# NVlabs/InstantSplat

Measured on AMD Instinct MI355X. Metric: train_iters_per_sec, higher is better.
Workload: dtype f32

## Files before the change

### include/mi355gs.h

```cpp
#ifndef MI355GS_H
#define MI355GS_H

#include <stddef.h>
#include <stdint.h>

#ifdef __cplusplus
extern "C" {
#endif

#define MI355GS_ABI_VERSION 10

#define MI355GS_OK 0
#define MI355GS_EINVAL (-1)
#define MI355GS_ELAUNCH (-2)
#define MI355GS_EOVERFLOW (-3)

int mi355gs_abi_version(void);
const char* mi355gs_error_string(int code);

size_t mi355gs_raster_geom_bytes(int P);
size_t mi355gs_raster_tiles_bytes(int W, int H);
size_t mi355gs_raster_binning_bytes(int64_t num_instances, int W, int H);

int mi355gs_raster_forward_preprocess(
    void* stream, int P, int D, int M, int W, int H,
    const float* means3D, const float* shs, const float* shs_rest, const float* colors_precomp, const float* opacities,
    const float* scales, float scale_modifier, const float* rotations, const float* cov3D_precomp,
    const float* viewmatrix, const float* projmatrix, const float* campos,
    float tanfovx, float tanfovy, int prefiltered,
    int32_t* radii, void* geom, void* tiles, int32_t* num_rendered, uint8_t* visible, void* grad_scratch, int debug);

int mi355gs_raster_forward_render(
    void* stream, int P, int W, int H, int64_t capacity, const float* bg,
    const void* geom, void* tiles, void* binning, float* out_color, int debug);

size_t mi355gs_raster_binning_bytes_render_only(int64_t num_instances, int W, int H);
int mi355gs_raster_forward_render_only(
    void* stream, int P, int W, int H, int64_t capacity, const float* bg,
    const void* geom, void* tiles, void* binning, float* out_color, int debug);

size_t mi355gs_raster_grad_scratch_bytes(int P);
size_t mi355gs_raster_grad_gate_offset(int P);
int mi355gs_raster_backward(
    void* stream, int P, int D, int M, int W, int H, const float* bg,
    const float* means3D, const float* shs, const float* shs_rest, const float* colors_precomp, const float* opacities,
    const float* scales, float scale_modifier, const float* rotations, const float* cov3D_precomp,
    const float* viewmatrix, const float* projmatrix, const float* campos,
    float tanfovx, float tanfovy,
    const void* geom, void* tiles, const void* binning, int64_t capacity, const int32_t* radii,
    const float* out_color, const float* dL_dpix, void* grad_scratch,
    float* dL_dmeans3D, float* dL_dmeans2D, float* dL_dshs, float* dL_dshs_rest, float* dL_dcolors, float* dL_dopacities,
    float* dL_dscales, float* dL_drotations, float* dL_dcov3D, int grad_scratch_is_clear, int debug);

int mi355gs_raster_mark_visible(void* stream, int P, const float* means3D, const float* viewmatrix,
                                const float* projmatrix, uint8_t* present);

int mi355gs_raster_frame_stats(void* stream, int W, int H, const void* tiles, int64_t* stats);

int mi355gs_tune_min_units(int min_units);

int mi355gs_tune_deterministic(int on);

int mi355gs_tune_scale_grad(int mode);

int mi355gs_profile_begin(void);
int mi355gs_profile_set_period(int every);
int mi355gs_profile_work_counters(void* counters);
int mi355gs_profile_read(int kind, double* total_ms, int* launches);
int mi355gs_profile_end(void);
int mi355gs_profile_ranges(int on);

size_t mi355gs_ssim_scratch_bytes(int B, int C, int H, int W);
int mi355gs_ssim_forward(void* stream, int B, int C, int H, int W, const float* img1, const float* img2,
                         float* dm_dmu1, float* dm_dsigma1_sq, float* dm_dsigma12,
                         void* scratch, float* ssim_mean, float* l1_mean, int padding_valid);
int mi355gs_ssim_backward(void* stream, int B, int C, int H, int W, const float* img1, const float* img2,
                          const float* dm_dmu1, const float* dm_dsigma1_sq, const float* dm_dsigma12,
                          const float* ssim_grad_scale, const float* l1_grad_scale, float* dL_dimg1, int padding_valid);
int mi355gs_l1_ssim_loss_fused(void* stream, int B, int C, int H, int W, const float* img1, const float* img2, void* scratch,
                               float lambda_dssim, float* ssim_mean, float* l1_mean, float* loss, float* dloss_dimg1);

size_t mi355gs_l1_scratch_bytes(int64_t n);
int mi355gs_l1_loss_forward(void* stream, int64_t n, const float* a, const float* b, void* scratch, float* mean_out);
int mi355gs_l1_loss_backward(void* stream, int64_t n, const float* a, const float* b, const float* grad_scale, float* d_a);
#define MI355GS_LOSS_PROGRAM_MAX 16
#define MI355GS_LOSS_OP_L1 0
#define MI355GS_LOSS_OP_SSIM 1
#define MI355GS_LOSS_OP_MULK 2
#define MI355GS_LOSS_OP_ADDK 3
#define MI355GS_LOSS_OP_RSUBK 4
#define MI355GS_LOSS_OP_DIVK 5
#define MI355GS_LOSS_OP_NEG 6
#define MI355GS_LOSS_OP_ADD 7
#define MI355GS_LOSS_OP_SUB 8
int mi355gs_l1_ssim_pair_forward(void* stream, int B, int C, int H, int W, const float* img1, const float* img2, void* scratch,
                                 float* dssim_dimg1);
int mi355gs_l1_ssim_pair_backward(void* stream, int64_t n, const float* img1, const float* img2, const float* dssim_dimg1,
                                  const float* g_l1, float c_l1, const float* g_ssim, float c_ssim, float* d_img1);
int mi355gs_loss_program_eval(void* stream, int n_ops, const int32_t* ops, const float* consts, int B, int C, int H, int W,
                              const void* scratch, float* ssim_mean, float* l1_mean, float* out, float* host_out, float ticket);
int mi355gs_loss_program_eval_grad(void* stream, int n_ops, const int32_t* ops, const float* consts, int B, int C, int H, int W,
                                   const void* scratch, float* ssim_mean, float* l1_mean, float* out, float* host_out, float ticket,
                                   const float* img1, const float* img2, const float* dssim_dimg1, float c_l1, float c_ssim, float* d_img1);

size_t mi355gs_knn_scratch_bytes(int N);
int mi355gs_knn_dist2(void* stream, int N, const float* points, float* mean_dist2, void* scratch);

int mi355gs_adam_step(void* stream, int64_t n, int row, float* param, const float* grad, float* exp_avg,
                      float* exp_avg_sq, const float* per_point_lr, const float* grad_sumsq,
                      float lr, float beta1, float beta2, float eps, int step);

int mi355gs_adam_multi_step(void* stream, int ntensors, const int64_t* numel, const int32_t* row, float* const* params,
                            const float* const* grads, float* const* exp_avg, float* const* exp_avg_sq,
                            const float* const* per_point_lr, const float* lr, float beta1, float beta2, float eps,
                            const int32_t* step, float* scratch, const float* gate, const int32_t* gate_index,
                            uint32_t* live, uint32_t seq);

int mi355gs_pose_forward(void* stream, int P, const float* xyz, const float* rot, const float* scaling,
                         const float* opacity_logit, const float* pose, float* means_cam, float* rot_cam, float* scales,
                         float* opac);
int mi355gs_pose_backward(void* stream, int P, const float* xyz, const float* rot, const float* scales, const float* opac,
                          const float* pose, const float* g_means, const float* g_rot, const float* g_scales,
                          const float* g_opac, float* d_xyz, float* d_rot, float* d_scaling, float* d_opacity_logit,
                          float* d_pose, float* scratch);

int mi355gs_posed_forward_preprocess(void* stream, int P, int D, int W, int H, const float* xyz, const float* f_dc,
                                     const float* f_rest, const float* opacity_logit, const float* log_scales, float scale_modifier,
                                     const float* rotation, const float* pose, const float* view_identity, const float* projmatrix,
                                     const float* origin, float tanfovx, float tanfovy, int32_t* radii, void* geom, void* tiles,
                                     int32_t* num_rendered, uint8_t* visible, void* grad_scratch, int debug);
int mi355gs_posed_backward(void* stream, int P, int D, int W, int H, const float* bg, const float* xyz, const float* f_dc,
                           const float* f_rest, const float* opacity_logit, const float* log_scales, float scale_modifier,
                           const float* rotation, const float* pose, const float* view_identity, const float* projmatrix,
                           const float* origin, float tanfovx, float tanfovy, const void* geom, void* tiles, const void* binning,
                           int64_t capacity, const int32_t* radii, const float* out_color, const float* dL_dpix,
                           void* grad_scratch, float* pose_scratch, float* d_xyz, float* d_means2D, float* d_f_dc, float* d_f_rest,
                           float* d_opacity_logit, float* d_log_scales, float* d_rotation, float* d_pose, int pose_rows, int pose_row,
                           int grad_scratch_is_clear, int debug);

size_t mi355gs_trainer_workspace_bytes(int P, int W, int H, int V, int64_t capacity);
void* mi355gs_trainer_create(int P, int W, int H, int V, int64_t capacity, float* xyz, float* f_dc, float* f_rest, float* opacity,
                             float* scaling, float* rotation, float* poses, float* const* exp_avg, float* const* exp_avg_sq,
                             const float* per_point_lr, void* workspace);
int mi355gs_trainer_step(void* trainer, void* stream, int view, int sh_degree, const float* gt_image, const float* projmatrix,
                         float tanfovx, float tanfovy, const float* bg, const float* lr, const int32_t* step, float beta1, float beta2, float eps,
                         float lambda_dssim, int do_optimizer_step, float* loss_out, int32_t* num_rendered_out);
int mi355gs_trainer_optimizer_step(void* trainer, void* stream, const float* lr, const int32_t* step, float beta1, float beta2,
                                   float eps, int commit_gate);
void mi355gs_trainer_destroy(void* trainer);
const float* mi355gs_trainer_grad(void* trainer, int k);

#define MI355GS_TRACKER_STATE_FLOATS 40
#define MI355GS_TRACKER_POSE 0
#define MI355GS_TRACKER_EXP_AVG 8
#define MI355GS_TRACKER_EXP_AVG_SQ 16
#define MI355GS_TRACKER_BEST 24
#define MI355GS_TRACKER_INITIAL 25
#define MI355GS_TRACKER_FLAG 26
#define MI355GS_TRACKER_COUNT 27
#define MI355GS_TRACKER_CAND 32
size_t mi355gs_tracker_workspace_bytes(int P, int W, int H, int64_t capacity);
void* mi355gs_tracker_create(int P, int M, int W, int H, int64_t capacity, const float* xyz, const float* f_dc, const float* f_rest,
                             const float* opacity, const float* scaling, const float* rotation, void* workspace);
int mi355gs_tracker_count(void* tracker, void* stream, int sh_degree, const float* projmatrix, float tanfovx, float tanfovy,
                          const float* pose, int32_t* count_out);
int mi355gs_tracker_run(void* tracker, void* stream, int sh_degree, const float* gt_image, const float* projmatrix, float tanfovx,
                        float tanfovy, const float* bg, const float* sched, int num_iter, int first_iter, int n_iters, float* state,
                        float* pose_trace, float* loss_trace, float* grad_trace);
void mi355gs_tracker_destroy(void* tracker);

int mi355gs_rgb8_from_planar(void* stream, int H, int W, const float* img, uint8_t* out);
size_t mi355gs_path_workspace_bytes(int P, int W, int H, int64_t capacity);
void* mi355gs_path_create(int P, int M, int W, int H, int64_t capacity, const float* xyz, const float* f_dc, const float* f_rest,
                          const float* opacity, const float* scaling, const float* rotation, void* workspace);
int mi355gs_path_render(void* path, void* stream, int sh_degree, const float* projmatrix, float tanfovx, float tanfovy,
                        const float* bg, const float* poses, int first, int n, uint8_t* frames, int32_t* counts);
void mi355gs_path_destroy(void* path);

#ifdef __cplusplus
}
#endif
#endif
```

### instantsplat_amd/_lib.py

```python
from __future__ import annotations

import ctypes
import os
from ctypes import c_float, c_int, c_int64, c_size_t, c_void_p

import torch

_HERE = os.path.dirname(os.path.abspath(__file__))
LIB_PATH = os.path.join(_HERE, "lib", "libmi355gs.so")
_LIB = None
_TEST_MODE = False

_P = c_void_p
_SIGNATURES = {
    "mi355gs_abi_version": (c_int, []),
    "mi355gs_error_string": (ctypes.c_char_p, [c_int]),
    "mi355gs_raster_geom_bytes": (c_size_t, [c_int]),
    "mi355gs_raster_tiles_bytes": (c_size_t, [c_int, c_int]),
    "mi355gs_raster_binning_bytes": (c_size_t, [c_int64, c_int, c_int]),
    "mi355gs_raster_grad_scratch_bytes": (c_size_t, [c_int]),
    "mi355gs_raster_grad_gate_offset": (c_size_t, [c_int]),
    "mi355gs_raster_forward_preprocess": (c_int, [_P, c_int, c_int, c_int, c_int, c_int, _P, _P, _P, _P, _P, _P, c_float, _P, _P,
                                                  _P, _P, _P, c_float, c_float, c_int, _P, _P, _P, _P, _P, _P, c_int]),
    "mi355gs_raster_forward_render": (c_int, [_P, c_int, c_int, c_int, c_int64, _P, _P, _P, _P, _P, c_int]),
    "mi355gs_raster_binning_bytes_render_only": (c_size_t, [c_int64, c_int, c_int]),
    "mi355gs_raster_forward_render_only": (c_int, [_P, c_int, c_int, c_int, c_int64, _P, _P, _P, _P, _P, c_int]),
    "mi355gs_raster_backward": (c_int, [_P, c_int, c_int, c_int, c_int, c_int, _P, _P, _P, _P, _P, _P, _P, c_float, _P, _P, _P, _P,
                                        _P, c_float, c_float, _P, _P, _P, c_int64, _P, _P, _P, _P, _P, _P, _P, _P, _P, _P, _P, _P, _P,
                                        c_int, c_int]),
    "mi355gs_raster_mark_visible": (c_int, [_P, c_int, _P, _P, _P, _P]),
    "mi355gs_raster_frame_stats": (c_int, [_P, c_int, c_int, _P, _P]),
    "mi355gs_tune_min_units": (c_int, [c_int]),
    "mi355gs_tune_scale_grad": (c_int, [c_int]),
    "mi355gs_tune_deterministic": (c_int, [c_int]),
    "mi355gs_profile_begin": (c_int, []),
    "mi355gs_profile_set_period": (c_int, [c_int]),
    "mi355gs_profile_work_counters": (c_int, [_P]),
    "mi355gs_profile_read": (c_int, [c_int, ctypes.POINTER(ctypes.c_double), ctypes.POINTER(c_int)]),
    "mi355gs_profile_end": (c_int, []),
    "mi355gs_profile_ranges": (c_int, [c_int]),
    "mi355gs_ssim_scratch_bytes": (c_size_t, [c_int, c_int, c_int, c_int]),
    "mi355gs_ssim_forward": (c_int, [_P, c_int, c_int, c_int, c_int, _P, _P, _P, _P, _P, _P, _P, _P, c_int]),
    "mi355gs_ssim_backward": (c_int, [_P, c_int, c_int, c_int, c_int, _P, _P, _P, _P, _P, _P, _P, _P, c_int]),
    "mi355gs_l1_ssim_loss_fused": (c_int, [_P, c_int, c_int, c_int, c_int, _P, _P, _P, c_float, _P, _P, _P, _P]),
    "mi355gs_l1_ssim_pair_forward": (c_int, [_P, c_int, c_int, c_int, c_int, _P, _P, _P, _P]),
    "mi355gs_l1_ssim_pair_backward": (c_int, [_P, c_int64, _P, _P, _P, _P, c_float, _P, c_float, _P]),
    "mi355gs_loss_program_eval": (c_int, [_P, c_int, _P, _P, c_int, c_int, c_int, c_int, _P, _P, _P, _P, _P, c_float]),
    "mi355gs_loss_program_eval_grad": (c_int, [_P, c_int, _P, _P, c_int, c_int, c_int, c_int, _P, _P, _P, _P, _P, c_float, _P, _P, _P, c_float,
                                               c_float, _P]),
    "mi355gs_knn_scratch_bytes": (c_size_t, [c_int]),
    "mi355gs_knn_dist2": (c_int, [_P, c_int, _P, _P, _P]),
    "mi355gs_adam_step": (c_int, [_P, c_int64, c_int, _P, _P, _P, _P, _P, _P, c_float, c_float, c_float, c_float, c_int]),
    "mi355gs_adam_multi_step": (c_int, [_P, c_int, _P, _P, _P, _P, _P, _P, _P, _P, c_float, c_float, c_float, _P, _P, _P, _P, _P,
                                        ctypes.c_uint32]),
    "mi355gs_pose_forward": (c_int, [_P, c_int, _P, _P, _P, _P, _P, _P, _P, _P, _P]),
    "mi355gs_pose_backward": (c_int, [_P, c_int, _P, _P, _P, _P, _P, _P, _P, _P, _P, _P, _P, _P, _P, _P, _P]),
    "mi355gs_posed_forward_preprocess": (c_int, [_P, c_int, c_int, c_int, c_int, _P, _P, _P, _P, _P, c_float, _P, _P, _P, _P, _P,
                                                 c_float, c_float, _P, _P, _P, _P, _P, _P, c_int]),
    "mi355gs_posed_backward": (c_int, [_P, c_int, c_int, c_int, c_int, _P, _P, _P, _P, _P, _P, c_float, _P, _P, _P, _P, _P, c_float,
                                       c_float, _P, _P, _P, c_int64, _P, _P, _P, _P, _P, _P, _P, _P, _P, _P, _P, _P, _P, c_int, c_int, c_int, c_int]),
    "mi355gs_l1_scratch_bytes": (c_size_t, [c_int64]),
    "mi355gs_l1_loss_forward": (c_int, [_P, c_int64, _P, _P, _P, _P]),
    "mi355gs_l1_loss_backward": (c_int, [_P, c_int64, _P, _P, _P, _P]),
    "mi355gs_trainer_workspace_bytes": (c_size_t, [c_int, c_int, c_int, c_int, c_int64]),
    "mi355gs_trainer_create": (c_void_p, [c_int, c_int, c_int, c_int, c_int64, _P, _P, _P, _P, _P, _P, _P, _P, _P, _P, _P]),
    "mi355gs_trainer_step": (c_int, [_P, _P, c_int, c_int, _P, _P, c_float, c_float, _P, _P, _P, c_float, c_float, c_float, c_float,
                                     c_int, _P, _P]),
    "mi355gs_trainer_optimizer_step": (c_int, [_P, _P, _P, _P, c_float, c_float, c_float, c_int]),
    "mi355gs_trainer_destroy": (None, [_P]),
    "mi355gs_trainer_grad": (_P, [_P, c_int]),
    "mi355gs_tracker_workspace_bytes": (c_size_t, [c_int, c_int, c_int, c_int64]),
    "mi355gs_tracker_create": (c_void_p, [c_int, c_int, c_int, c_int, c_int64, _P, _P, _P, _P, _P, _P, _P]),
    "mi355gs_tracker_count": (c_int, [_P, _P, c_int, _P, c_float, c_float, _P, _P]),
    "mi355gs_tracker_run": (c_int, [_P, _P, c_int, _P, _P, c_float, c_float, _P, _P, c_int, c_int, c_int, _P, _P, _P, _P]),
    "mi355gs_tracker_destroy": (None, [_P]),
    "mi355gs_rgb8_from_planar": (c_int, [_P, c_int, c_int, _P, _P]),
    "mi355gs_path_workspace_bytes": (c_size_t, [c_int, c_int, c_int, c_int64]),
    "mi355gs_path_create": (c_void_p, [c_int, c_int, c_int, c_int, c_int64, _P, _P, _P, _P, _P, _P, _P]),
    "mi355gs_path_render": (c_int, [_P, _P, c_int, _P, c_float, c_float, _P, _P, c_int, c_int, _P, _P]),
    "mi355gs_path_destroy": (None, [_P]),
}
EXPORTED_SYMBOLS = tuple(_SIGNATURES)


ABI_VERSION = 10


def _bind(path: str):
    lib = ctypes.CDLL(path)
    for name, (res, args) in _SIGNATURES.items():
        fn = getattr(lib, name)
        fn.restype, fn.argtypes = res, args
    got = lib.mi355gs_abi_version()
    if got != ABI_VERSION:
        raise RuntimeError(f"{path} implements ABI v{got}, this package binds v{ABI_VERSION}: rebuild it with "
                           "`python -c 'import __graft_entry__ as g; g.build()'`")
    return lib


def lib():
    global _LIB
    if _LIB is None:
        if not os.path.exists(LIB_PATH):
            raise RuntimeError(
                f"{LIB_PATH} is missing: build it with `python -c 'import __graft_entry__ as g; g.build()'` "
                "(hipcc --offload-arch=gfx950). instantsplat_amd has no CPU or PyTorch fallback.")
        _LIB = _bind(LIB_PATH)
        if os.environ.get("MI355GS_DETERMINISTIC", "0") == "1":
            _LIB.mi355gs_tune_deterministic(1)
    return _LIB


def _use_library_for_testing(path: str | None):
    global _LIB, _TEST_MODE, _EXT_BOUND_TO
    if path is None:
        _LIB, _TEST_MODE = None, False
    else:
        _LIB, _TEST_MODE = _bind(path), True
    _EXT_BOUND_TO = None


BINDING = os.environ.get("MI355GS_BINDING", "compiled")
EXT_PATH = os.path.join(_HERE, "lib", "_mi355gs_torch.so")
_EXT = None
_EXT_BOUND_TO = None


def compiled():
    global _EXT, _EXT_BOUND_TO
    if BINDING != "compiled":
        return None
    L = lib()
    if _EXT_BOUND_TO is L:
        return _EXT
    if _EXT is None:
        if not os.path.exists(EXT_PATH):
            raise RuntimeError(f"{EXT_PATH} is missing: build it with `python -c 'import __graft_entry__ as g; g.build()'` "
                               "(or set MI355GS_BINDING=ctypes to use the Python binding)")
        import importlib.util
        spec = importlib.util.spec_from_file_location("_mi355gs_torch", EXT_PATH)
        _EXT = importlib.util.module_from_spec(spec)
        spec.loader.exec_module(_EXT)
    _EXT.forget_gates()
    _EXT.bind({name: ctypes.cast(getattr(L, name), ctypes.c_void_p).value for name in _EXT.abi_symbols()}, _TEST_MODE)
    _EXT_BOUND_TO = L
    return _EXT


def check(code: int, what: str):
    if code != 0:
        raise RuntimeError(f"mi355gs: {what} failed: {lib().mi355gs_error_string(code).decode()} ({code})")


def ptr(t: torch.Tensor | None):
    return None if t is None else t.data_ptr()


_F32 = torch.float32


def f32c_on_one_device(*tensors):
    out, dev = [], None
    for t in tensors:
        if t.dtype is not _F32:
            raise RuntimeError(f"expected float32, got {t.dtype}")
        if not t.is_contiguous():
            t = t.contiguous()
        d = t.device
        if dev is None:
            if d.type != "cuda" and not _TEST_MODE:
                raise RuntimeError("instantsplat_amd operators run on the GPU only (got a CPU tensor; there is no CPU fallback)")
            dev = d
        elif d != dev:
            raise RuntimeError(f"tensors on different devices: {dev} vs {d}")
        out.append(t)
    return out, dev


def require_device(*tensors: torch.Tensor | None):
    dev = None
    for t in tensors:
        if t is None:
            continue
        if not t.is_cuda and not _TEST_MODE:
            raise RuntimeError("instantsplat_amd operators run on the GPU only (got a CPU tensor; there is no CPU fallback)")
        if not t.is_contiguous():
            raise RuntimeError("instantsplat_amd operators need contiguous tensors")
        if dev is None:
            dev = t.device
        elif t.device != dev:
            raise RuntimeError(f"tensors on different devices: {dev} vs {t.device}")
    return dev


class _NoGuard:
    def __enter__(self):
        return None

    def __exit__(self, *a):
        return False


_NO_GUARD = _NoGuard()


def on_device(device):
    if device is not None and device.type == "cuda" and device.index is not None and device.index != torch.cuda.current_device():
        return torch.cuda.device(device)
    return _NO_GUARD


def stream_ptr(device):
    if device is not None and device.type == "cuda":
        return torch.cuda.current_stream(device).cuda_stream
    return None


def f32c(t: torch.Tensor | None):
    if t is None:
        return None
    if t.dtype != torch.float32:
# ... 3 lines not shown
```

### instantsplat_amd/csrc/ssim.hip

```cpp
#include "common.h"

namespace {

constexpr int TS = 16;
constexpr int TSX = 32;
constexpr int HALO = 5;
constexpr int TH = TS + 2 * HALO;
constexpr int THX = TSX + 2 * HALO;
constexpr int SXP = 48;
constexpr int STAGE_ITERS = (TH * SXP + 255) / 256;
constexpr int ROW_ITEMS = TH * TS;
constexpr float C1 = 0.01f * 0.01f;
constexpr float C2 = 0.03f * 0.03f;

__device__ __forceinline__ float gw(int k) {
  constexpr float w[11] = {0.001028380123898387f, 0.0075987582094967365f, 0.036000773310661316f, 0.10936068743467331f,
                           0.21300552785396576f,  0.26601171493530273f,   0.21300552785396576f,  0.10936068743467331f,
                           0.036000773310661316f, 0.0075987582094967365f, 0.001028380123898387f};
  return w[k];
}

__device__ __forceinline__ bool ssim_equal_window(float mu1, float mu2, float exx, float eyy, float exy) {
  return mu1 == mu2 && exx == eyy && exx == exy && exx != 0.f;
}
// ... 64 lines not shown
    const gs_v2f A = mu1_sq + mu2_sq + c1, B = s1 + s2 + c2, Cc = two * mu12 + c1, Dd = two * s12 + c2;
    const gs_v2f invA = {ssim_rcp(A[0]), ssim_rcp(A[1])}, invB = {ssim_rcp(B[0]), ssim_rcp(B[1])};
    const gs_v2f invAB = invA * invB;
    const gs_v2f m = Cc * Dd * invAB;
    const gs_v2f t = mu1 * two * Cc * Dd * invAB;
    const gs_v2f d1 = (mu2 * two * Dd) * invAB - (mu2 * two * Cc) * invAB - t * invA + t * invB;
    const gs_v2f d2 = -m * invB;
    const gs_v2f d3 = two * Cc * invAB;
    const int gy = oy + ly;
#pragma unroll
    for (int half = 0; half < 2; ++half) {
      const int gx = ox + lx + half * TS;
      if (gx < W && gy < H) {
        const bool counted = gx >= crop && gx < W - crop && gy >= crop && gy < H - crop;
        const bool same = ssim_equal_window(mu1[half], mu2[half], exx[half], eyy[half], exy[half]);
        val += counted ? (same ? 1.f : m[half]) : 0.f;
        const size_t o = (size_t)plane * H * W + (size_t)gy * W + gx;
        if (dm_dmu1) {
          dm_dmu1[o] = counted ? (same ? 0.f : d1[half]) : 0.f;
          dm_dsigma1_sq[o] = counted ? (same ? -invB[half] : d2[half]) : 0.f;
          dm_dsigma12[o] = counted ? (same ? 2.f * invB[half] : d3[half]) : 0.f;
        }
        l1 += fabsf(s_x[ly + HALO][lx + half * TS + HALO] - s_y[ly + HALO][lx + half * TS + HALO]);
      }
    }
  }
  val = gs_wave_sum_row3(val);
  l1 = gs_wave_sum_row3(l1);
  const int wave = tid >> 6, lane = tid & 63;
  if (lane == 63) { s_red[0][wave] = val; s_red[1][wave] = l1; }
  __syncthreads();
  if (tid == 0) {
    const size_t b = ((size_t)blockIdx.z * gridDim.y + blockIdx.y) * gridDim.x + blockIdx.x;
    partial[2 * b] = (s_red[0][0] + s_red[0][1]) + (s_red[0][2] + s_red[0][3]);
    partial[2 * b + 1] = (s_red[1][0] + s_red[1][1]) + (s_red[1][2] + s_red[1][3]);
  }
}

__global__ __launch_bounds__(1024) void k_ssim_finish(int nblocks, double inv_n, const float* __restrict__ partial,
                                                       float* __restrict__ ssim_mean, float* __restrict__ l1_mean,
                                                       float* __restrict__ loss, float lambda_dssim) {
  __shared__ double s_a[16], s_b[16];
  double a = 0.0, b = 0.0;
  for (int i = threadIdx.x; i < nblocks; i += 1024) { a += (double)partial[2 * i]; b += (double)partial[2 * i + 1]; }
  a = gs_wave_sum_row3_f64(a); b = gs_wave_sum_row3_f64(b);
  const int wave = threadIdx.x >> 6, lane = threadIdx.x & 63;
  if (lane == 63) { s_a[wave] = a; s_b[wave] = b; }
  __syncthreads();
  if (threadIdx.x == 0) {
    double ta = 0.0, tb = 0.0;
    for (int w = 0; w < 16; ++w) { ta += s_a[w]; tb += s_b[w]; }
    const float sm = (float)(ta * inv_n), lm = (float)(tb * inv_n);
    if (ssim_mean) *ssim_mean = sm;
    if (l1_mean) *l1_mean = lm;
    if (loss) *loss = (1.0f - lambda_dssim) * lm + lambda_dssim * (1.0f - sm);
  }
}

__global__ __launch_bounds__(256) void k_ssim_bwd(int H, int W, float inv_n, const float* __restrict__ img1, const float* __restrict__ img2,
                                                   const float* __restrict__ dm_dmu1, const float* __restrict__ dm_dsigma1_sq,
                                                   const float* __restrict__ dm_dsigma12, const float* __restrict__ ssim_scale,
                                                   const float* __restrict__ l1_scale, float ssim_scale_host, float l1_scale_host,
                                                   float* __restrict__ dL_dimg1) {
  __shared__ float s_a[TH][SXP];
  __shared__ float s_b[TH][SXP];
  __shared__ float s_c[TH][SXP];
  __shared__ gs_v2f s_h[3][TH][TS];
  const int tid = threadIdx.y * TS + threadIdx.x;
  const int plane = blockIdx.z;
  const int ox = blockIdx.x * TSX, oy = blockIdx.y * TS;
  const size_t po = (size_t)plane * H * W;
  const float ks = (ssim_scale ? *ssim_scale : 1.f) * ssim_scale_host * inv_n;
  const float kl = (l1_scale ? *l1_scale : 1.f) * l1_scale_host * inv_n;
  float px[2], py[2];
#pragma unroll
  for (int half = 0; half < 2; ++half) {
    const size_t o = po + (size_t)min(oy + (int)threadIdx.y, H - 1) * W + min(ox + (int)threadIdx.x + half * TS, W - 1);
    px[half] = img1[o]; py[half] = img2[o];
  }
  if (ks != 0.f) {
    {
      float va[STAGE_ITERS], vb[STAGE_ITERS], vc[STAGE_ITERS];
#pragma unroll
      for (int j = 0; j < STAGE_ITERS; ++j) {
        const int i = tid + 256 * j, r = i / SXP, c = i - r * SXP;
        const size_t o = po + (size_t)min(max(oy + r - HALO, 0), H - 1) * W + min(max(ox + c - HALO, 0), W - 1);
        va[j] = dm_dmu1[o]; vb[j] = dm_dsigma1_sq[o]; vc[j] = dm_dsigma12[o];
      }
#pragma unroll
      for (int j = 0; j < STAGE_ITERS; ++j) {
        const int i = tid + 256 * j, r = i / SXP, c = i - r * SXP;
        const int gy = oy + r - HALO, gx = ox + c - HALO;
        const bool in = c < THX && gy >= 0 && gy < H && gx >= 0 && gx < W;
        if (i < TH * SXP) { s_a[r][c] = in ? va[j] : 0.f; s_b[r][c] = in ? vb[j] : 0.f; s_c[r][c] = in ? vc[j] : 0.f; }
      }
    }
    __syncthreads();
    for (int i = tid; i < ROW_ITEMS; i += 256) {
      const int r = i >> 4, c = i & 15;
      gs_v2f a = {0.f, 0.f}, b = a, cc = a;
#pragma unroll
      for (int k = 0; k < 11; ++k) {
        const gs_v2f w = {gw(k), gw(k)};
        a = gs_fma2(w, gs_v2f{s_a[r][c + k], s_a[r][c + TS + k]}, a);
        b = gs_fma2(w, gs_v2f{s_b[r][c + k], s_b[r][c + TS + k]}, b);
        cc = gs_fma2(w, gs_v2f{s_c[r][c + k], s_c[r][c + TS + k]}, cc);
      }
      s_h[0][r][c] = a; s_h[1][r][c] = b; s_h[2][r][c] = cc;
    }
    __syncthreads();
  }
  const int ly = threadIdx.y, lx = threadIdx.x;
  const int gy = oy + ly;
  if (gy >= H) return;
  gs_v2f a = {0.f, 0.f}, b = a, cc = a;
  if (ks != 0.f) {
#pragma unroll
    for (int k = 0; k < 11; ++k) {
      const gs_v2f w = {gw(k), gw(k)};
      a = gs_fma2(w, s_h[0][ly + k][lx], a); b = gs_fma2(w, s_h[1][ly + k][lx], b); cc = gs_fma2(w, s_h[2][ly + k][lx], cc);
    }
  }
#pragma unroll
  for (int half = 0; half < 2; ++half) {
    const int gx = ox + lx + half * TS;
    if (gx >= W) continue;
    const size_t o = po + (size_t)gy * W + gx;
    const float x = px[half], y = py[half];
    float g = 0.f;
    if (ks != 0.f) g = ks * ((x == y && cc[half] == -2.f * b[half]) ? a[half] : a[half] + 2.f * x * b[half] + y * cc[half]);
    if (kl != 0.f) {
      const float d = x - y;
      g += kl * (d > 0.f ? 1.f : (d < 0.f ? -1.f : 0.f));
    }
    dL_dimg1[o] = g;
  }
}


constexpr int FT = 32;
constexpr int FR1 = FT + 2 * HALO;
constexpr int FR2 = FT + 4 * HALO;
constexpr int FXP = 58;
constexpr int FHP = 43;
constexpr int FDP = 46;
constexpr int FEP = 33;
constexpr int FTHREADS = 512;
constexpr int F_STAGE_ITERS = (FR2 * FXP + FTHREADS - 1) / FTHREADS;
constexpr int FER = FT * FT / FTHREADS;
constexpr int FCR = 7, FC_GROUPS = (FR1 + FCR - 1) / FCR;
constexpr int FDR = 8, FD_GROUPS = FT / FDR;
static_assert(FC_GROUPS * FR1 <= FTHREADS && FD_GROUPS * FR1 <= FTHREADS && FT % FDR == 0 && FDR % 2 == 0, "one item per thread");

__global__ __launch_bounds__(FTHREADS) void k_l1_ssim_fused(int H, int W, const float* __restrict__ img1, const float* __restrict__ img2,
                                                        float ks , float kl ,
                                                        float* __restrict__ dL_dimg1, float* __restrict__ partial ) {
  __shared__ float s_xy[2][FR2][FXP];
  __shared__ float s_h[5][FR2][FHP];
  static_assert(3 * FR1 * FDP <= 2 * FR2 * FXP && 3 * FR1 * FEP <= 5 * FR2 * FHP, "aliased LDS buffers must fit");
  __shared__ float s_red[2][FTHREADS / 64];
  float (*s_d)[FR1][FDP] = reinterpret_cast<float (*)[FR1][FDP]>(&s_xy[0][0][0]);
  float (*s_e)[FR1][FEP] = reinterpret_cast<float (*)[FR1][FEP]>(&s_h[0][0][0]);
  const int tid = threadIdx.x;
  const int plane = blockIdx.z;
  const int ox = blockIdx.x * FT, oy = blockIdx.y * FT;
  const size_t po = (size_t)plane * H * W;
  const float* p1 = img1 + po;
  const float* p2 = img2 + po;
  const int ec = tid & 31, er0 = (tid >> 5) * FER;
  float ex[FER], ey[FER];
#pragma unroll
  for (int j = 0; j < FER; ++j) {
    const size_t o = (size_t)min(oy + er0 + j, H - 1) * W + min(ox + ec, W - 1);
    ex[j] = p1[o]; ey[j] = p2[o];
  }
  {
    float vx[F_STAGE_ITERS], vy[F_STAGE_ITERS];
#pragma unroll
    for (int j = 0; j < F_STAGE_ITERS; ++j) {
      const int i = tid + FTHREADS * j, r = i / FXP, c = i - r * FXP;
      const size_t o = (size_t)min(max(oy + r - 2 * HALO, 0), H - 1) * W + min(max(ox + c - 2 * HALO, 0), W - 1);
      vx[j] = p1[o]; vy[j] = p2[o];
    }
#pragma unroll
    for (int j = 0; j < F_STAGE_ITERS; ++j) {
      const int i = tid + FTHREADS * j, r = i / FXP, c = i - r * FXP;
      const int gy = oy + r - 2 * HALO, gx = ox + c - 2 * HALO;
      const bool in = gy >= 0 && gy < H && gx >= 0 && gx < W;
      if (i < FR2 * FXP) { s_xy[0][r][c] = in ? vx[j] : 0.f; s_xy[1][r][c] = in ? vy[j] : 0.f; }
    }
  }
  __syncthreads();
  for (int i = tid; i < FR2 * 7; i += FTHREADS) {
    const int r = i % FR2, c0 = (i / FR2) * 6;
    float x[16], y[16];
#pragma unroll
    for (int t = 0; t < 16; t += 2) {
      const float2 a = *reinterpret_cast<const float2*>(&s_xy[0][r][c0 + t]);
      const float2 b = *reinterpret_cast<const float2*>(&s_xy[1][r][c0 + t]);
      x[t] = a.x; x[t + 1] = a.y; y[t] = b.x; y[t + 1] = b.y;
    }
    float sx[6], sy[6], sxx[6], syy[6], sxy[6];
#pragma unroll
    for (int j = 0; j < 6; ++j) { sx[j] = sy[j] = sxx[j] = syy[j] = sxy[j] = 0.f; }
#pragma unroll
    for (int t = 0; t < 16; ++t) {
      const float xx = x[t] * x[t], yy = y[t] * y[t], xy = x[t] * y[t];
#pragma unroll
      for (int j = 0; j < 6; ++j) {
        const int k = t - j;
        if (k >= 0 && k < 11) {
          const float w = gw(k);
          sx[j] = fmaf(w, x[t], sx[j]); sy[j] = fmaf(w, y[t], sy[j]);
          sxx[j] = fmaf(w, xx, sxx[j]); syy[j] = fmaf(w, yy, syy[j]); sxy[j] = fmaf(w, xy, sxy[j]);
        }
      }
    }
#pragma unroll
    for (int j = 0; j < 6; ++j) {
      s_h[0][r][c0 + j] = sx[j]; s_h[1][r][c0 + j] = sy[j]; s_h[2][r][c0 + j] = sxx[j]; s_h[3][r][c0 + j] = syy[j];
      s_h[4][r][c0 + j] = sxy[j];
    }
  }
  __syncthreads();
  float val = 0.f;
  if (tid < FR1 * FC_GROUPS) {
    const int c = tid % FR1, r0 = (tid / FR1) * FCR;
    float mo[5][FCR];
#pragma unroll
    for (int m = 0; m < 5; ++m) {
      float v[FCR + 10];
#pragma unroll
      for (int t = 0; t < FCR + 10; ++t) v[t] = s_h[m][min(r0 + t, FR2 - 1)][c];
#pragma unroll
      for (int j = 0; j < FCR; ++j) {
        float a = 0.f;
#pragma unroll
        for (int k = 0; k < 11; ++k) a = fmaf(gw(k), v[j + k], a);
        mo[m][j] = a;
      }
    }
    const int gx = ox + c - HALO;
#pragma unroll
    for (int j = 0; j < FCR; ++j) {
      const int r = r0 + j, gy = oy + r - HALO;
      const float mu1 = mo[0][j], mu2 = mo[1][j];
      const float mu1_sq = mu1 * mu1, mu2_sq = mu2 * mu2, mu12 = mu1 * mu2;
      const float s1 = mo[2][j] - mu1_sq, s2 = mo[3][j] - mu2_sq, s12 = mo[4][j] - mu12;
      const float A = mu1_sq + mu2_sq + C1, B = s1 + s2 + C2, Cc = 2.f * mu12 + C1, Dd = 2.f * s12 + C2;
      const float invA = ssim_rcp(A), invB = ssim_rcp(B), invAB = invA * invB;
      const float m = Cc * Dd * invAB;
      const float t = mu1 * 2.f * Cc * Dd * invAB;
      const float d1 = (mu2 * 2.f * Dd) * invAB - (mu2 * 2.f * Cc) * invAB - t * invA + t * invB;
      const float d2 = -m * invB;
      const float d3 = 2.f * Cc * invAB;
      const bool in_img = gx >= 0 && gx < W && gy >= 0 && gy < H && r < FR1;
      const bool same = ssim_equal_window(mu1, mu2, mo[2][j], mo[3][j], mo[4][j]);
      mo[0][j] = in_img ? (same ? 0.f : d1) : 0.f; mo[1][j] = in_img ? (same ? -invB : d2) : 0.f; mo[2][j] = in_img ? (same ? 2.f * invB : d3) : 0.f;
      const bool in_tile = c >= HALO && c < HALO + FT && r >= HALO && r < HALO + FT;
      val += (in_img && in_tile) ? (same ? 1.f : m) : 0.f;
    }
#pragma unroll
    for (int j = 0; j < FCR; ++j)
      if (FR1 % FCR == 0 || r0 + j < FR1) { s_d[0][r0 + j][c] = mo[0][j]; s_d[1][r0 + j][c] = mo[1][j]; s_d[2][r0 + j][c] = mo[2][j]; }
  }
  __syncthreads();
  if (tid < FR1 * FD_GROUPS) {
    const int r = tid % FR1, c0 = (tid / FR1) * FDR;
#pragma unroll
    for (int m = 0; m < 3; ++m) {
      float v[FDR + 10];
#pragma unroll
      for (int t = 0; t < FDR + 10; t += 2) {
        const float2 a = *reinterpret_cast<const float2*>(&s_d[m][r][c0 + t]);
        v[t] = a.x; v[t + 1] = a.y;
      }
#pragma unroll
      for (int j = 0; j < FDR; ++j) {
        float a = 0.f;
#pragma unroll
        for (int k = 0; k < 11; ++k) a = fmaf(gw(k), v[j + k], a);
        s_e[m][r][c0 + j] = a;
      }
    }
  }
  __syncthreads();
  float l1 = 0.f;
  {
    float out[3][FER];
#pragma unroll
    for (int m = 0; m < 3; ++m) {
      float v[FER + 10];
#pragma unroll
      for (int t = 0; t < FER + 10; ++t) v[t] = s_e[m][er0 + t][ec];
#pragma unroll
      for (int j = 0; j < FER; ++j) {
        float a = 0.f;
#pragma unroll
        for (int k = 0; k < 11; ++k) a = fmaf(gw(k), v[j + k], a);
        out[m][j] = a;
      }
    }
    const int gx = ox + ec;
#pragma unroll
    for (int j = 0; j < FER; ++j) {
      const int gy = oy + er0 + j;
      if (gx < W && gy < H) {
        const float x = ex[j], y = ey[j], d = x - y;
        l1 += fabsf(d);
        const float gs = (d == 0.f && out[2][j] == -2.f * out[1][j]) ? out[0][j] : out[0][j] + 2.f * x * out[1][j] + y * out[2][j];
        const float g = ks * gs + kl * (d > 0.f ? 1.f : (d < 0.f ? -1.f : 0.f));
        dL_dimg1[po + (size_t)gy * W + gx] = g;
      }
    }
  }
  val = gs_wave_sum_row3(val);
  l1 = gs_wave_sum_row3(l1);
  const int wave = tid >> 6, lane = tid & 63;
  if (lane == 63) { s_red[0][wave] = val; s_red[1][wave] = l1; }
  __syncthreads();
  if (tid == 0) {
    const size_t b = ((size_t)blockIdx.z * gridDim.y + blockIdx.y) * gridDim.x + blockIdx.x;
    float ta = 0.f, tb = 0.f;
#pragma unroll
    for (int w = 0; w < FTHREADS / 64; ++w) { ta += s_red[0][w]; tb += s_red[1][w]; }
    partial[2 * b] = ta;
    partial[2 * b + 1] = tb;
  }
}

constexpr int L1_THREADS = 256, L1_PER_THREAD = 16;
__global__ __launch_bounds__(L1_THREADS) void k_l1_partial(long long n, const float* __restrict__ a, const float* __restrict__ b,
                                                           float* __restrict__ partial) {
  __shared__ float s_red[L1_THREADS / 64];
  const long long base = (long long)blockIdx.x * (L1_THREADS * L1_PER_THREAD);
  float acc = 0.f;
  const bool vec = ((((uintptr_t)a | (uintptr_t)b) & 15) == 0) && base + L1_THREADS * L1_PER_THREAD <= n;
  if (vec) {
#pragma unroll
    for (int r = 0; r < L1_PER_THREAD / 4; ++r) {
      const long long j = (base >> 2) + threadIdx.x + (long long)L1_THREADS * r;
      const float4 x = reinterpret_cast<const float4*>(a)[j], y = reinterpret_cast<const float4*>(b)[j];
      acc += (fabsf(x.x - y.x) + fabsf(x.y - y.y)) + (fabsf(x.z - y.z) + fabsf(x.w - y.w));
    }
  } else {
    for (int r = 0; r < L1_PER_THREAD; ++r) {
      const long long i = base + threadIdx.x + (long long)L1_THREADS * r;
      if (i < n) acc += fabsf(a[i] - b[i]);
    }
  }
  acc = gs_wave_sum_row3(acc);
  if ((threadIdx.x & 63) == 63) s_red[threadIdx.x >> 6] = acc;
  __syncthreads();
  if (threadIdx.x == 0) {
    partial[2 * blockIdx.x] = (s_red[0] + s_red[1]) + (s_red[2] + s_red[3]);
    partial[2 * blockIdx.x + 1] = 0.f;
  }
}

__global__ __launch_bounds__(256) void k_l1_bwd(long long n, const float* __restrict__ a, const float* __restrict__ b,
                                                const float* __restrict__ grad_scale, float n_as_float, float* __restrict__ d_a) {
  const float s = *grad_scale / n_as_float;
  const long long i0 = ((long long)blockIdx.x * 256 + threadIdx.x) * 4;
  if (((((uintptr_t)a | (uintptr_t)b | (uintptr_t)d_a) & 15) == 0) && i0 + 4 <= n) {
    const float4 x = reinterpret_cast<const float4*>(a)[i0 >> 2], y = reinterpret_cast<const float4*>(b)[i0 >> 2];
    auto sg = [&](float d) { return d > 0.f ? s : (d < 0.f ? -s : 0.f); };
    reinterpret_cast<float4*>(d_a)[i0 >> 2] = make_float4(sg(x.x - y.x), sg(x.y - y.y), sg(x.z - y.z), sg(x.w - y.w));
  } else {
    for (long long i = i0; i < min(n, i0 + 4); ++i) { const float d = a[i] - b[i]; d_a[i] = d > 0.f ? s : (d < 0.f ? -s : 0.f); }
  }
}

struct GsLossProgram {
  int n;
  signed char op[MI355GS_LOSS_PROGRAM_MAX];
  float k[MI355GS_LOSS_PROGRAM_MAX];
};

__device__ __forceinline__ void loss_program_body(const GsLossProgram& p, int nblocks, double inv_n, const float* __restrict__ partial,
                                                  float* __restrict__ ssim_mean, float* __restrict__ l1_mean, float* __restrict__ out,
                                                  float* __restrict__ host_out, float ticket) {
#pragma clang fp contract(off)
  __shared__ double s_a[16], s_b[16];
  double a = 0.0, b = 0.0;
  for (int i = threadIdx.x; i < nblocks; i += 1024) { a += (double)partial[2 * i]; b += (double)partial[2 * i + 1]; }
  a = gs_wave_sum_row3_f64(a); b = gs_wave_sum_row3_f64(b);
  const int wave = threadIdx.x >> 6, lane = threadIdx.x & 63;
  if (lane == 63) { s_a[wave] = a; s_b[wave] = b; }
  __syncthreads();
  if (threadIdx.x != 0) return;
  double ta = 0.0, tb = 0.0;
  for (int w = 0; w < 16; ++w) { ta += s_a[w]; tb += s_b[w]; }
  const float sm = (float)(ta * inv_n), lm = (float)(tb * inv_n);
  *ssim_mean = sm; *l1_mean = lm;
  float st[MI355GS_LOSS_PROGRAM_MAX];
  int sp = 0;
  for (int i = 0; i < p.n; ++i) {
    const float k = p.k[i];
    switch (p.op[i]) {
      case MI355GS_LOSS_OP_L1: st[sp++] = lm; break;
      case MI355GS_LOSS_OP_SSIM: st[sp++] = sm; break;
      case MI355GS_LOSS_OP_MULK: st[sp - 1] = st[sp - 1] * k; break;
      case MI355GS_LOSS_OP_ADDK: st[sp - 1] = st[sp - 1] + k; break;
      case MI355GS_LOSS_OP_RSUBK: st[sp - 1] = k - st[sp - 1]; break;
      case MI355GS_LOSS_OP_DIVK: st[sp - 1] = st[sp - 1] * (1.0f / k); break;
      case MI355GS_LOSS_OP_NEG: st[sp - 1] = -st[sp - 1]; break;
      case MI355GS_LOSS_OP_ADD: st[sp - 2] = st[sp - 2] + st[sp - 1]; --sp; break;
      case MI355GS_LOSS_OP_SUB: st[sp - 2] = st[sp - 2] - st[sp - 1]; --sp; break;
      default: break;
    }
  }
  const float value = sp > 0 ? st[sp - 1] : 0.f;
  *out = value;
  if (host_out) {
    typedef float v2f __attribute__((vector_size(8)));
    v2f both = {value, ticket};
    *reinterpret_cast<v2f*>(host_out) = both;
  }
}

__global__ __launch_bounds__(1024) void k_loss_program(GsLossProgram p, int nblocks, double inv_n, const float* __restrict__ partial,
                                                      float* __restrict__ ssim_mean, float* __restrict__ l1_mean, float* __restrict__ out,
                                                      float* __restrict__ host_out, float ticket) {
  loss_program_body(p, nblocks, inv_n, partial, ssim_mean, l1_mean, out, host_out, ticket);
}

__device__ __forceinline__ void loss_pair_bwd_four(long long n, long long i0, const float* __restrict__ a, const float* __restrict__ b,
                                                   const float* __restrict__ dssim, float sl, float ss, bool use_l1, bool use_ss,
                                                   float* __restrict__ d_a) {
#pragma clang fp contract(off)
  auto one = [&](float x, float y, float ds) {
    const float d = x - y;
    const float tl = use_l1 ? (d > 0.f ? sl : (d < 0.f ? -sl : 0.f)) : 0.f;
    return use_ss ? tl + ss * ds : tl;
  };
  const uintptr_t al = (uintptr_t)a | (uintptr_t)b | (uintptr_t)d_a | (uintptr_t)(use_ss ? dssim : a);
  if (((al & 15) == 0) && i0 + 4 <= n) {
    const float4 x = reinterpret_cast<const float4*>(a)[i0 >> 2], y = reinterpret_cast<const float4*>(b)[i0 >> 2];
    const float4 s = use_ss ? reinterpret_cast<const float4*>(dssim)[i0 >> 2] : make_float4(0.f, 0.f, 0.f, 0.f);
    reinterpret_cast<float4*>(d_a)[i0 >> 2] = make_float4(one(x.x, y.x, s.x), one(x.y, y.y, s.y), one(x.z, y.z, s.z), one(x.w, y.w, s.w));
  } else {
    for (long long i = i0; i < min(n, i0 + 4); ++i) d_a[i] = one(a[i], b[i], use_ss ? dssim[i] : 0.f);
  }
}

__global__ __launch_bounds__(256) void k_loss_pair_bwd(long long n, const float* __restrict__ a, const float* __restrict__ b,
                                                       const float* __restrict__ dssim, const float* __restrict__ g_l1, float c_l1,
                                                       const float* __restrict__ g_ssim, float c_ssim, float n_as_float,
                                                       float* __restrict__ d_a) {
#pragma clang fp contract(off)
  const float sl = ((g_l1 ? *g_l1 : 1.0f) * c_l1) / n_as_float;
  const float ss = (g_ssim ? *g_ssim : 1.0f) * c_ssim;
  const bool use_l1 = c_l1 != 0.0f, use_ss = c_ssim != 0.0f && dssim != nullptr;
  loss_pair_bwd_four(n, ((long long)blockIdx.x * 256 + threadIdx.x) * 4, a, b, dssim, sl, ss, use_l1, use_ss, d_a);
}

__global__ __launch_bounds__(1024) void k_loss_program_grad(GsLossProgram p, int nblocks, double inv_n, const float* __restrict__ partial,
                                                           float* __restrict__ ssim_mean, float* __restrict__ l1_mean, float* __restrict__ out,
                                                           float* __restrict__ host_out, float ticket, long long n,
                                                           const float* __restrict__ a, const float* __restrict__ b,
                                                           const float* __restrict__ dssim, float c_l1, float c_ssim, float n_as_float,
                                                           float* __restrict__ d_a) {
#pragma clang fp contract(off)
  if (blockIdx.x == 0) {
    loss_program_body(p, nblocks, inv_n, partial, ssim_mean, l1_mean, out, host_out, ticket);
    return;
  }
  const float sl = (1.0f * c_l1) / n_as_float;
  const float ss = 1.0f * c_ssim;
  const bool use_l1 = c_l1 != 0.0f, use_ss = c_ssim != 0.0f && dssim != nullptr;
  loss_pair_bwd_four(n, ((long long)(blockIdx.x - 1) * 1024 + threadIdx.x) * 4, a, b, dssim, sl, ss, use_l1, use_ss, d_a);
}

}

static inline int l1_nblocks(long long n) { return (int)((n + L1_THREADS * L1_PER_THREAD - 1) / (L1_THREADS * L1_PER_THREAD)); }

static inline int ssim_nblocks(int B, int C, int H, int W) { return B * C * ((H + TS - 1) / TS) * ((W + TSX - 1) / TSX); }

extern "C" {

size_t mi355gs_ssim_scratch_bytes(int B, int C, int H, int W) {
  if (B <= 0 || C <= 0 || H <= 0 || W <= 0) return 256;
  return gs_align((size_t)ssim_nblocks(B, C, H, W) * 2 * sizeof(float));
}

int mi355gs_ssim_forward(void* stream_, int B, int C, int H, int W, const float* img1, const float* img2, float* dm_dmu1,
                         float* dm_dsigma1_sq, float* dm_dsigma12, void* scratch, float* ssim_mean, float* l1_mean, int padding_valid) {
  GS_RANGE();
  hipStream_t stream = (hipStream_t)stream_;
  const int debug = 0;
  if (B <= 0 || C <= 0 || H <= 0 || W <= 0 || !img1 || !img2 || !scratch) return MI355GS_EINVAL;
  const int crop = padding_valid ? HALO : 0;
  if (padding_valid && (l1_mean || H <= 2 * HALO || W <= 2 * HALO)) return MI355GS_EINVAL;
  if ((dm_dmu1 == nullptr) != (dm_dsigma1_sq == nullptr) || (dm_dmu1 == nullptr) != (dm_dsigma12 == nullptr)) return MI355GS_EINVAL;
  if ((size_t)B * C > 65535) return MI355GS_EINVAL;
  const dim3 grid((W + TSX - 1) / TSX, (H + TS - 1) / TS, B * C);
  GS_KRANGE("ssim_fwd");
  hipLaunchKernelGGL(k_ssim_fwd, grid, dim3(TS, TS), 0, stream, H, W, img1, img2, dm_dmu1, dm_dsigma1_sq, dm_dsigma12, (float*)scratch, crop);
  GS_CHECK_LAUNCH("ssim_fwd");
  const double inv_n = 1.0 / ((double)B * C * (H - 2 * crop) * (W - 2 * crop));
  GS_KRANGE("ssim_finish");
  hipLaunchKernelGGL(k_ssim_finish, dim3(1), dim3(1024), 0, stream, ssim_nblocks(B, C, H, W), inv_n, (const float*)scratch, ssim_mean,
                     l1_mean, (float*)nullptr, 0.f);
  GS_CHECK_LAUNCH("ssim_finish");
  return MI355GS_OK;
}

int mi355gs_ssim_backward(void* stream_, int B, int C, int H, int W, const float* img1, const float* img2, const float* dm_dmu1,
                          const float* dm_dsigma1_sq, const float* dm_dsigma12, const float* ssim_grad_scale,
                          const float* l1_grad_scale, float* dL_dimg1, int padding_valid) {
  GS_RANGE();
  hipStream_t stream = (hipStream_t)stream_;
  const int debug = 0;
  if (B <= 0 || C <= 0 || H <= 0 || W <= 0 || !img1 || !img2 || !dL_dimg1) return MI355GS_EINVAL;
  if (ssim_grad_scale && (!dm_dmu1 || !dm_dsigma1_sq || !dm_dsigma12)) return MI355GS_EINVAL;
  if ((size_t)B * C > 65535) return MI355GS_EINVAL;
  const dim3 grid((W + TSX - 1) / TSX, (H + TS - 1) / TS, B * C);
  const int crop = padding_valid ? HALO : 0;
  if (padding_valid && (l1_grad_scale || H <= 2 * HALO || W <= 2 * HALO)) return MI355GS_EINVAL;
  const float inv_n = (float)(1.0 / ((double)B * C * (H - 2 * crop) * (W - 2 * crop)));
  GS_KRANGE("ssim_bwd");
  hipLaunchKernelGGL(k_ssim_bwd, grid, dim3(TS, TS), 0, stream, H, W, inv_n, img1, img2, dm_dmu1, dm_dsigma1_sq, dm_dsigma12,
                     ssim_grad_scale, l1_grad_scale, ssim_grad_scale ? 1.f : 0.f, l1_grad_scale ? 1.f : 0.f, dL_dimg1);
  GS_CHECK_LAUNCH("ssim_bwd");
  return MI355GS_OK;
}

size_t mi355gs_l1_scratch_bytes(int64_t n) { return gs_align((size_t)(n > 0 ? l1_nblocks(n) : 1) * 2 * sizeof(float)); }

int mi355gs_l1_loss_forward(void* stream_, int64_t n, const float* a, const float* b, void* scratch, float* mean_out) {
  GS_RANGE();
  hipStream_t stream = (hipStream_t)stream_;
  const int debug = 0;
  if (n <= 0 || n > (int64_t)1 << 40 || !a || !b || !scratch || !mean_out) return MI355GS_EINVAL;
  GS_KRANGE("l1_partial");
  hipLaunchKernelGGL(k_l1_partial, dim3(l1_nblocks(n)), dim3(L1_THREADS), 0, stream, (long long)n, a, b, (float*)scratch);
  GS_CHECK_LAUNCH("l1_partial");
  GS_KRANGE("l1_finish");
  hipLaunchKernelGGL(k_ssim_finish, dim3(1), dim3(1024), 0, stream, l1_nblocks(n), 1.0 / (double)n, (const float*)scratch, mean_out,
                     (float*)nullptr, (float*)nullptr, 0.f);
  GS_CHECK_LAUNCH("l1_finish");
  return MI355GS_OK;
}

int mi355gs_l1_loss_backward(void* stream_, int64_t n, const float* a, const float* b, const float* grad_scale, float* d_a) {
  GS_RANGE();
  hipStream_t stream = (hipStream_t)stream_;
  const int debug = 0;
  if (n <= 0 || n > (int64_t)1 << 40 || !a || !b || !grad_scale || !d_a) return MI355GS_EINVAL;
  GS_KRANGE("l1_bwd");
  hipLaunchKernelGGL(k_l1_bwd, dim3((unsigned)((n + 1023) / 1024)), dim3(256), 0, stream, (long long)n, a, b, grad_scale, (float)n, d_a);
  GS_CHECK_LAUNCH("l1_bwd");
  return MI355GS_OK;
}

static inline int fused_nblocks(int B, int C, int H, int W) { return B * C * ((H + FT - 1) / FT) * ((W + FT - 1) / FT); }

int mi355gs_l1_ssim_loss_fused(void* stream_, int B, int C, int H, int W, const float* img1, const float* img2, void* scratch,
                               float lambda_dssim, float* ssim_mean, float* l1_mean, float* loss, float* dloss_dimg1) {
  GS_RANGE();
  hipStream_t stream = (hipStream_t)stream_;
  const int debug = 0;
  if (B <= 0 || C <= 0 || H <= 0 || W <= 0 || !img1 || !img2 || !scratch || !loss || !dloss_dimg1) return MI355GS_EINVAL;
  if ((size_t)B * C > 65535) return MI355GS_EINVAL;
  const double inv_n = 1.0 / ((double)B * C * H * W);
  const dim3 grid((W + FT - 1) / FT, (H + FT - 1) / FT, B * C);
  {
    GsProfScope prof(3, stream);
    GS_KRANGE("l1_ssim_fused");
    hipLaunchKernelGGL(k_l1_ssim_fused, grid, dim3(FTHREADS), 0, stream, H, W, img1, img2, (float)(-(double)lambda_dssim * inv_n),
                       (float)((1.0 - (double)lambda_dssim) * inv_n), dloss_dimg1, (float*)scratch);
  }
  GS_CHECK_LAUNCH("l1_ssim_fused");
  GS_KRANGE("ssim_finish");
  hipLaunchKernelGGL(k_ssim_finish, dim3(1), dim3(1024), 0, stream, fused_nblocks(B, C, H, W), inv_n, (const float*)scratch, ssim_mean,
                     l1_mean, loss, lambda_dssim);
  GS_CHECK_LAUNCH("ssim_finish");
  return MI355GS_OK;
}

int mi355gs_l1_ssim_pair_forward(void* stream_, int B, int C, int H, int W, const float* img1, const float* img2, void* scratch,
                                 float* dssim_dimg1) {
  GS_RANGE();
  hipStream_t stream = (hipStream_t)stream_;
  const int debug = 0;
  if (B <= 0 || C <= 0 || H <= 0 || W <= 0 || !img1 || !img2 || !scratch || !dssim_dimg1) return MI355GS_EINVAL;
  if ((size_t)B * C > 65535) return MI355GS_EINVAL;
  const double inv_n = 1.0 / ((double)B * C * H * W);
  const dim3 grid((W + FT - 1) / FT, (H + FT - 1) / FT, B * C);
  {
    GsProfScope prof(3, stream);
    GS_KRANGE("l1_ssim_pair");
    hipLaunchKernelGGL(k_l1_ssim_fused, grid, dim3(FTHREADS), 0, stream, H, W, img1, img2, (float)inv_n, 0.0f, dssim_dimg1, (float*)scratch);
  }
  GS_CHECK_LAUNCH("l1_ssim_pair");
  return MI355GS_OK;
}

int mi355gs_l1_ssim_pair_backward(void* stream_, int64_t n, const float* img1, const float* img2, const float* dssim_dimg1,
                                  const float* g_l1, float c_l1, const float* g_ssim, float c_ssim, float* d_img1) {
  GS_RANGE();
  hipStream_t stream = (hipStream_t)stream_;
  const int debug = 0;
  if (n <= 0 || n > (int64_t)1 << 40 || !img1 || !img2 || !d_img1) return MI355GS_EINVAL;
  if (c_ssim != 0.0f && !dssim_dimg1) return MI355GS_EINVAL;
  GS_KRANGE("loss_pair_bwd");
  hipLaunchKernelGGL(k_loss_pair_bwd, dim3((unsigned)((n + 1023) / 1024)), dim3(256), 0, stream, (long long)n, img1, img2, dssim_dimg1, g_l1,
                     c_l1, g_ssim, c_ssim, (float)n, d_img1);
  GS_CHECK_LAUNCH("loss_pair_bwd");
  return MI355GS_OK;
}

static int build_loss_program(int n_ops, const int32_t* ops, const float* consts, GsLossProgram& p) {
  if (n_ops <= 0 || n_ops > MI355GS_LOSS_PROGRAM_MAX || !ops || !consts) return MI355GS_EINVAL;
  p.n = n_ops;
  int depth = 0;
  for (int i = 0; i < MI355GS_LOSS_PROGRAM_MAX; ++i) {
    p.op[i] = 0; p.k[i] = 0.f;
    if (i >= n_ops) continue;
    const int op = ops[i];
    if (op == MI355GS_LOSS_OP_L1 || op == MI355GS_LOSS_OP_SSIM) ++depth;
    else if (op == MI355GS_LOSS_OP_ADD || op == MI355GS_LOSS_OP_SUB) { if (depth < 2) return MI355GS_EINVAL; --depth; }
    else if (op >= MI355GS_LOSS_OP_MULK && op <= MI355GS_LOSS_OP_NEG) { if (depth < 1) return MI355GS_EINVAL; }
    else return MI355GS_EINVAL;
    p.op[i] = (signed char)op; p.k[i] = consts[i];
  }
  return depth == 1 ? MI355GS_OK : MI355GS_EINVAL;
}

int mi355gs_loss_program_eval(void* stream_, int n_ops, const int32_t* ops, const float* consts, int B, int C, int H, int W,
                              const void* scratch, float* ssim_mean, float* l1_mean, float* out, float* host_out, float ticket) {
  GS_RANGE();
  hipStream_t stream = (hipStream_t)stream_;
  const int debug = 0;
  if (!scratch || !l1_mean || !ssim_mean || !out) return MI355GS_EINVAL;
  if (B <= 0 || C <= 0 || H <= 0 || W <= 0 || ((uintptr_t)host_out & 7) != 0) return MI355GS_EINVAL;
  GsLossProgram p;
  if (build_loss_program(n_ops, ops, consts, p) != MI355GS_OK) return MI355GS_EINVAL;
  GS_KRANGE("loss_program");
  hipLaunchKernelGGL(k_loss_program, dim3(1), dim3(1024), 0, stream, p, fused_nblocks(B, C, H, W), 1.0 / ((double)B * C * H * W),
                     (const float*)scratch, ssim_mean, l1_mean, out, host_out, ticket);
  GS_CHECK_LAUNCH("loss_program");
  return MI355GS_OK;
}

int mi355gs_loss_program_eval_grad(void* stream_, int n_ops, const int32_t* ops, const float* consts, int B, int C, int H, int W,
                                   const void* scratch, float* ssim_mean, float* l1_mean, float* out, float* host_out, float ticket,
                                   const float* img1, const float* img2, const float* dssim_dimg1, float c_l1, float c_ssim, float* d_img1) {
  GS_RANGE();
  hipStream_t stream = (hipStream_t)stream_;
  const int debug = 0;
  if (!scratch || !l1_mean || !ssim_mean || !out || !img1 || !img2 || !d_img1) return MI355GS_EINVAL;
  if (B <= 0 || C <= 0 || H <= 0 || W <= 0 || ((uintptr_t)host_out & 7) != 0) return MI355GS_EINVAL;
  if (c_ssim != 0.0f && !dssim_dimg1) return MI355GS_EINVAL;
  GsLossProgram p;
  if (build_loss_program(n_ops, ops, consts, p) != MI355GS_OK) return MI355GS_EINVAL;
  const long long n = (long long)B * C * H * W;
  GS_KRANGE("loss_program_grad");
  hipLaunchKernelGGL(k_loss_program_grad, dim3(1u + (unsigned)((n + 4095) / 4096)), dim3(1024), 0, stream, p, fused_nblocks(B, C, H, W),
                     1.0 / (double)n, (const float*)scratch, ssim_mean, l1_mean, out, host_out, ticket, n, img1, img2, dssim_dimg1, c_l1, c_ssim,
                     (float)n, d_img1);
  GS_CHECK_LAUNCH("loss_program_grad");
  return MI355GS_OK;
}

}

int gs_loss_fused(hipStream_t stream, int C, int H, int W, const float* img1, const float* img2, float lambda_dssim, float* dL_dimg1,
                  void* scratch) {
  const int debug = 0;
  const double inv_n = 1.0 / ((double)C * H * W);
  const dim3 grid((W + FT - 1) / FT, (H + FT - 1) / FT, C);
  {
    GsProfScope prof(3, stream);
    GS_KRANGE("l1_ssim_fused");
    hipLaunchKernelGGL(k_l1_ssim_fused, grid, dim3(FTHREADS), 0, stream, H, W, img1, img2, (float)(-(double)lambda_dssim * inv_n),
                       (float)((1.0 - (double)lambda_dssim) * inv_n), dL_dimg1, (float*)scratch);
  }
  GS_CHECK_LAUNCH("l1_ssim_fused");
  return MI355GS_OK;
}
int gs_loss_fused_nblocks(int C, int H, int W) { return fused_nblocks(1, C, H, W); }
```

### instantsplat_amd/csrc/trainer.hip

```cpp
#include <stdlib.h>
#include <string.h>
#include "common.h"

int gs_loss_fused(hipStream_t, int, int, int, const float*, const float*, float, float*, void*);
int gs_loss_fused_nblocks(int, int, int);
int gs_launch_pose_finish_partials(hipStream_t, const float*, const float*, int, float*, float*, const float*, int, double, float, float*, int,
                                   int);

namespace {

struct Trainer {
  int P, W, H, V;
  int64_t capacity;
  float *xyz, *f_dc, *f_rest, *opacity, *scaling, *rotation, *poses;
  float* m[7];
  float* v[7];
  const float* pplr;
  char *geom, *tiles, *binning, *grad_scratch, *ssim_scratch;
  float *image, *dL_dimg;
  int32_t* radii;
  float *g_means2D, *g_colors;
  float *g_xyz, *g_rot, *g_scaling, *g_opacity, *g_fdc, *g_frest, *g_poses;
  float *pose_scratch, *pose_partial, *adam_scratch, *consts;
  uint32_t* adam_live;
  uint32_t adam_seq;
  bool consts_ready;
  int det;
  int min_units;
};

size_t carve(Trainer& t, void* workspace) {
  GsCarver c{(char*)workspace};
  const size_t P = (size_t)(t.P > 0 ? t.P : 1), npix = (size_t)t.W * t.H;
  t.geom = c.take<char>(mi355gs_raster_geom_bytes(t.P));
  t.tiles = c.take<char>(mi355gs_raster_tiles_bytes(t.W, t.H));
  t.binning = c.take<char>(mi355gs_raster_binning_bytes(t.capacity, t.W, t.H));
  t.grad_scratch = c.take<char>(mi355gs_raster_grad_scratch_bytes(t.P));
  t.ssim_scratch = c.take<char>(mi355gs_ssim_scratch_bytes(1, 3, t.H, t.W));
  t.image = c.take<float>(3 * npix); t.dL_dimg = c.take<float>(3 * npix);
  t.radii = c.take<int32_t>(P);
  t.g_means2D = c.take<float>(3 * P); t.g_colors = c.take<float>(3 * P);
  t.g_xyz = c.take<float>(3 * P); t.g_rot = c.take<float>(4 * P); t.g_scaling = c.take<float>(3 * P); t.g_opacity = c.take<float>(P);
  t.g_fdc = c.take<float>(3 * P); t.g_frest = c.take<float>(45 * P); t.g_poses = c.take<float>(7 * (size_t)t.V);
  t.pose_scratch = c.take<float>(32); t.pose_partial = c.take<float>(16 * ((P + 255) / 256)); t.adam_scratch = c.take<float>(8); t.consts = c.take<float>(32);
  t.adam_live = c.take<uint32_t>(16);
  return c.off;
}

int trainer_adam(Trainer* t, hipStream_t stream, const float* lr, const int32_t* step, float beta1, float beta2, float eps,
                 bool commit_gate) {
  const int P = t->P;
  const int64_t numel[7] = {3LL * P, 3LL * P, 45LL * P, (int64_t)P, 3LL * P, 4LL * P, 7LL * t->V};
  const int32_t row[7] = {3, 1, 1, 1, 1, 1, 1};
  float* params[7] = {t->xyz, t->f_dc, t->f_rest, t->opacity, t->scaling, t->rotation, t->poses};
  const float* grads[7] = {t->g_xyz, t->g_fdc, t->g_frest, t->g_opacity, t->g_scaling, t->g_rot, t->g_poses};
  const float* pplr[7] = {t->pplr, nullptr, nullptr, nullptr, nullptr, nullptr, nullptr};
  if (++t->adam_seq == 0u) t->adam_seq = 1u;
  g_fused.adam_live = t->adam_live; g_fused.adam_seq = t->adam_seq;
  if (commit_gate) {
    const TilesLayout tl(t->W, t->H);
    g_fused.commit_count = (const uint32_t*)(t->tiles + tl.start) + tl.T;
    g_fused.commit_capacity = (unsigned long long)t->capacity;
    g_fused.commit_poison = t->adam_live + 15;
  }
  return mi355gs_adam_multi_step(stream, 7, numel, row, params, grads, t->m, t->v, pplr, lr, beta1, beta2, eps, step, t->adam_scratch, nullptr, nullptr, nullptr, 0u);
}

}

extern "C" {

int mi355gs_posed_forward_preprocess(void* stream, int P, int D, int W, int H, const float* xyz, const float* f_dc,
                                     const float* f_rest, const float* opacity_logit, const float* log_scales, float scale_modifier,
                                     const float* rotation, const float* pose, const float* view_identity, const float* projmatrix,
                                     const float* origin, float tanfovx, float tanfovy, int32_t* radii, void* geom, void* tiles,
                                     int32_t* num_rendered, uint8_t* visible, void* grad_scratch, int debug) {
  GS_RANGE();
  if (!pose || D < 0 || D > 3 || (D > 0 && !f_rest)) return MI355GS_EINVAL;
  struct Scope { ~Scope() { g_fused = GsFusedStepHooks(); } } scope;
  g_fused.posed.pose = pose;
  return mi355gs_raster_forward_preprocess(stream, P, D, D == 0 ? 1 : 16, W, H, xyz, f_dc, D == 0 ? nullptr : f_rest, nullptr,
                                           opacity_logit, log_scales, scale_modifier, rotation, nullptr, view_identity, projmatrix,
                                           origin, tanfovx, tanfovy, 0, radii, geom, tiles, num_rendered, visible, grad_scratch, debug);
}

int mi355gs_posed_backward(void* stream_, int P, int D, int W, int H, const float* bg, const float* xyz, const float* f_dc,
                           const float* f_rest, const float* opacity_logit, const float* log_scales, float scale_modifier,
                           const float* rotation, const float* pose, const float* view_identity, const float* projmatrix,
                           const float* origin, float tanfovx, float tanfovy, const void* geom, void* tiles, const void* binning,
                           int64_t capacity, const int32_t* radii, const float* out_color, const float* dL_dpix,
                           void* grad_scratch, float* pose_scratch, float* d_xyz, float* d_means2D, float* d_f_dc, float* d_f_rest,
                           float* d_opacity_logit, float* d_log_scales, float* d_rotation, float* d_pose, int pose_rows, int pose_row,
                           int grad_scratch_is_clear, int debug) {
  GS_RANGE();
  hipStream_t stream = (hipStream_t)stream_;
  if (!pose || !pose_scratch || !d_pose || D < 0 || D > 3 || (D > 0 && (!f_rest || !d_f_rest))) return MI355GS_EINVAL;
  if (pose_rows < 0 || (pose_rows > 0 && (pose_row < 0 || pose_row >= pose_rows))) return MI355GS_EINVAL;
  if (P <= 0)
    return hipMemsetAsync(d_pose, 0, (size_t)(pose_rows > 0 ? pose_rows : 1) * 7 * sizeof(float), stream) == hipSuccess ? MI355GS_OK : MI355GS_ELAUNCH;
  const int rows = (P + 255) / 256;
  float* gate = (float*)((char*)grad_scratch + mi355gs_raster_grad_gate_offset(P));
  int rc;
  {
    struct Scope { ~Scope() { g_fused = GsFusedStepHooks(); } } scope;
    g_fused.posed.pose = pose;
    g_fused.posed.acc = pose_scratch + (size_t)16 * rows;
    g_fused.posed.partial = pose_scratch;
    g_fused.gate = gate; g_fused.gate_tail = true;
    g_fused.gate_xyz = 0; g_fused.gate_sh = 1; g_fused.gate_sh_rest = 2; g_fused.gate_opacity = 3; g_fused.gate_scaling = 4; g_fused.gate_rot = 5;
    rc = mi355gs_raster_backward(stream, P, D, D == 0 ? 1 : 16, W, H, bg, xyz, f_dc, D == 0 ? nullptr : f_rest, nullptr, opacity_logit,
                                 log_scales, scale_modifier, rotation, nullptr, view_identity, projmatrix, origin, tanfovx, tanfovy,
                                 geom, tiles, binning, capacity, radii, out_color, dL_dpix, grad_scratch, d_xyz, d_means2D, d_f_dc,
                                 D == 0 ? nullptr : d_f_rest, nullptr, d_opacity_logit, d_log_scales, d_rotation, nullptr,
                                 grad_scratch_is_clear, debug);
  }
  if (rc) return rc;
  GS_KRANGE("pose_finish");
  gs_launch_pose_finish_partials(stream, pose, pose_scratch, rows, d_pose, gate + 6, nullptr, 0, 0.0, 0.f, nullptr, pose_rows, pose_row);
  GS_CHECK_LAUNCH("pose_finish");
  return MI355GS_OK;
}

size_t mi355gs_trainer_workspace_bytes(int P, int W, int H, int V, int64_t capacity) {
  if (P < 0 || W <= 0 || H <= 0 || V <= 0 || capacity < 0) return 0;
  Trainer t;
  memset(&t, 0, sizeof(t));
  t.P = P; t.W = W; t.H = H; t.V = V; t.capacity = capacity;
  return carve(t, nullptr);
}

void* mi355gs_trainer_create(int P, int W, int H, int V, int64_t capacity, float* xyz, float* f_dc, float* f_rest, float* opacity,
                             float* scaling, float* rotation, float* poses, float* const* exp_avg, float* const* exp_avg_sq,
                             const float* per_point_lr, void* workspace) {
  if (P <= 0 || W <= 0 || H <= 0 || V <= 0 || capacity <= 0 || !workspace || !exp_avg || !exp_avg_sq) return nullptr;
  if (!xyz || !f_dc || !f_rest || !opacity || !scaling || !rotation || !poses) return nullptr;
  Trainer* t = (Trainer*)calloc(1, sizeof(Trainer));
  if (!t) return nullptr;
  t->P = P; t->W = W; t->H = H; t->V = V; t->capacity = capacity;
  t->xyz = xyz; t->f_dc = f_dc; t->f_rest = f_rest; t->opacity = opacity; t->scaling = scaling; t->rotation = rotation; t->poses = poses;
  for (int k = 0; k < 7; ++k) {
    if (!exp_avg[k] || !exp_avg_sq[k]) { free(t); return nullptr; }
    t->m[k] = exp_avg[k]; t->v[k] = exp_avg_sq[k];
  }
  t->pplr = per_point_lr;
  t->min_units = gs_min_units();
  t->det = gs_deterministic();
  carve(*t, workspace);
  t->consts_ready = false;
  return t;
}

void mi355gs_trainer_destroy(void* handle) { free(handle); }

const float* mi355gs_trainer_grad(void* handle, int k) {
  Trainer* t = (Trainer*)handle;
  if (!t || k < 0 || k > 6) return nullptr;
  const float* g[7] = {t->g_xyz, t->g_fdc, t->g_frest, t->g_opacity, t->g_scaling, t->g_rot, t->g_poses};
  return g[k];
}

int mi355gs_trainer_step(void* handle, void* stream_, int view, int sh_degree, const float* gt_image, const float* projmatrix,
                         float tanfovx, float tanfovy, const float* bg, const float* lr, const int32_t* step, float beta1, float beta2, float eps,
                         float lambda_dssim, int do_optimizer_step, float* loss_out, int32_t* num_rendered_out) {
  GS_RANGE();
  Trainer* t = (Trainer*)handle;
  hipStream_t stream = (hipStream_t)stream_;
  const int debug = 0;
  if (!t || view < 0 || view >= t->V || sh_degree < 0 || sh_degree > 3 || !gt_image || !projmatrix || !bg || !lr || !step || !loss_out || !num_rendered_out)
    return MI355GS_EINVAL;
  const int P = t->P, W = t->W, H = t->H;
  if (!t->consts_ready) {
    GS_KRANGE("trainer_consts");
    gs_launch_view_consts(stream, t->consts);
    GS_CHECK_LAUNCH("trainer_consts");
    if (hipMemsetAsync(t->g_frest, 0, (size_t)P * 45 * sizeof(float), stream) != hipSuccess) return MI355GS_ELAUNCH;
    if (hipMemsetAsync(t->adam_live, 0, 16 * sizeof(uint32_t), stream) != hipSuccess) return MI355GS_ELAUNCH;
    t->consts_ready = true;
  }
  struct HookScope {
    HookScope(float* gate, const GsPrologue& pro, const GsPosed& posed, int min_units, int det) {
      gs_pin_min_units(min_units);
      gs_pin_deterministic(det);
      g_fused.skip_memsets = true; g_fused.gate = gate; g_fused.prologue = pro; g_fused.posed = posed;
      g_fused.gate_xyz = 0; g_fused.gate_sh = 1; g_fused.gate_sh_rest = 2; g_fused.gate_opacity = 3; g_fused.gate_scaling = 4; g_fused.gate_rot = 5; g_fused.gate_pose = 6;
    }
    ~HookScope() { g_fused = GsFusedStepHooks(); gs_pin_min_units(0); gs_pin_deterministic(-1); }
  };
  GsPrologue pro;
  {
    const TilesLayout tl(W, H);
    pro.grad_records = (float4*)t->grad_scratch; pro.n_vec = (size_t)P * 3;
    pro.tile_counters = (uint32_t*)(t->tiles + tl.count); pro.n_counters = (int)((tl.start - tl.count) / 4);
    pro.g_poses = t->g_poses; pro.n_pose = 7 * t->V; pro.pose_scratch = t->pose_scratch; pro.adam_scratch = t->adam_scratch;
  }
  GsPosed posed;
  posed.pose = t->poses + 7 * (size_t)view; posed.acc = t->pose_scratch; posed.partial = t->pose_partial;
  HookScope hook_scope(t->adam_scratch, pro, posed, t->min_units, t->det);
  const float* view_m = t->consts;
  const float* campos = t->consts + 16;
  const float* pose = t->poses + 7 * (size_t)view;
  int rc;
  const int D = sh_degree, M = D == 0 ? 1 : 16;
  const float* rest = D == 0 ? nullptr : t->f_rest;
  float* g_rest = D == 0 ? nullptr : t->g_frest;
  if ((rc = mi355gs_raster_forward_preprocess(stream, P, D, M, W, H, t->xyz, t->f_dc, rest, nullptr, t->opacity, t->scaling, 1.0f,
                                              t->rotation, nullptr, view_m, projmatrix, campos, tanfovx, tanfovy, 0, t->radii,
                                              t->geom, t->tiles, num_rendered_out, nullptr, nullptr, 0)))
    return rc;
  if ((rc = mi355gs_raster_forward_render(stream, P, W, H, t->capacity, bg, t->geom, t->tiles, t->binning, t->image, 0))) return rc;
  if ((rc = gs_loss_fused(stream, 3, H, W, t->image, gt_image, lambda_dssim, t->dL_dimg, t->ssim_scratch))) return rc;
  if ((rc = mi355gs_raster_backward(stream, P, D, M, W, H, bg, t->xyz, t->f_dc, rest, nullptr, t->opacity, t->scaling, 1.0f, t->rotation,
                                    nullptr, view_m, projmatrix, campos, tanfovx, tanfovy, t->geom, t->tiles, t->binning,
                                    t->capacity, t->radii, t->image, t->dL_dimg, t->grad_scratch, t->g_xyz, t->g_means2D, t->g_fdc,
                                    g_rest, t->g_colors, t->g_opacity, t->g_scaling, t->g_rot, nullptr, 0, 0)))
    return rc;
  GS_KRANGE("pose_finish");
  gs_launch_pose_finish_partials(stream, pose, t->pose_partial, (P + 255) / 256, t->g_poses + 7 * (size_t)view, t->adam_scratch + 6,
                                 (const float*)t->ssim_scratch, gs_loss_fused_nblocks(3, H, W), 1.0 / (3.0 * H * W), lambda_dssim, loss_out, 0, 0);
  GS_CHECK_LAUNCH("pose_finish");
  if (do_optimizer_step) return trainer_adam(t, stream, lr, step, beta1, beta2, eps, true);
  return MI355GS_OK;
}

int mi355gs_trainer_optimizer_step(void* handle, void* stream_, const float* lr, const int32_t* step, float beta1, float beta2,
                                   float eps, int commit_gate) {
  GS_RANGE();
  Trainer* t = (Trainer*)handle;
  if (!t || !lr || !step || !t->consts_ready) return MI355GS_EINVAL;
  g_fused.gate = t->adam_scratch;
  const int rc = trainer_adam(t, (hipStream_t)stream_, lr, step, beta1, beta2, eps, commit_gate != 0);
  g_fused = GsFusedStepHooks();
  return rc;
}

}
```

### instantsplat_amd/csrc_torch/binding.cpp

```cpp
#include <torch/extension.h>
#include <ATen/hip/impl/HIPGuardImplMasqueradingAsCUDA.h>
#include <c10/hip/HIPStream.h>

#include <chrono>
#include <optional>
#include <map>
#include <mutex>

#include "../../include/mi355gs.h"

namespace {

using torch::Tensor;
using torch::autograd::AutogradContext;
using torch::autograd::variable_list;

#define GS_ABI_LIST(X)                                                 \
  X(geom_bytes, mi355gs_raster_geom_bytes)                             \
  X(tiles_bytes, mi355gs_raster_tiles_bytes)                           \
  X(binning_bytes, mi355gs_raster_binning_bytes)                       \
  X(grad_scratch_bytes, mi355gs_raster_grad_scratch_bytes)             \
  X(grad_gate_offset, mi355gs_raster_grad_gate_offset)                 \
  X(posed_forward_preprocess, mi355gs_posed_forward_preprocess)        \
  X(forward_preprocess, mi355gs_raster_forward_preprocess)             \
  X(raster_backward, mi355gs_raster_backward)                          \
  X(forward_render, mi355gs_raster_forward_render)                     \
  X(binning_bytes_render_only, mi355gs_raster_binning_bytes_render_only) \
  X(forward_render_only, mi355gs_raster_forward_render_only)           \
  X(posed_backward, mi355gs_posed_backward)                            \
  X(ssim_scratch_bytes, mi355gs_ssim_scratch_bytes)                    \
  X(l1_ssim_loss_fused, mi355gs_l1_ssim_loss_fused)                    \
  X(l1_scratch_bytes, mi355gs_l1_scratch_bytes)                        \
  X(l1_loss_forward, mi355gs_l1_loss_forward)                          \
  X(l1_loss_backward, mi355gs_l1_loss_backward)                        \
  X(pair_forward, mi355gs_l1_ssim_pair_forward)                        \
  X(pair_backward, mi355gs_l1_ssim_pair_backward)                      \
  X(program_eval, mi355gs_loss_program_eval)                           \
  X(program_eval_grad, mi355gs_loss_program_eval_grad)                 \
  X(ssim_forward, mi355gs_ssim_forward)                                \
  X(ssim_backward, mi355gs_ssim_backward)                              \
  X(adam_multi_step, mi355gs_adam_multi_step)                          \
  X(error_string, mi355gs_error_string)

struct Abi {
#define GS_MEMBER(field, name) decltype(&name) field = nullptr;
  GS_ABI_LIST(GS_MEMBER)
#undef GS_MEMBER
  bool bound = false;
  bool allow_cpu = false;
} g_abi;

std::vector<std::string> abi_symbols() {
#define GS_NAME(field, name) #name,
  return {GS_ABI_LIST(GS_NAME)};
#undef GS_NAME
}

void bind_abi(const std::map<std::string, uintptr_t>& sym, bool allow_cpu_tensors) {
  g_abi.allow_cpu = allow_cpu_tensors;
  auto get = [&](const char* name) {
    auto it = sym.find(name);
    TORCH_CHECK(it != sym.end() && it->second, "mi355gs torch binding: entry point ", name, " was not provided");
    return it->second;
  };
#define GS_BIND(field, name) g_abi.field = reinterpret_cast<decltype(&name)>(get(#name));
  GS_ABI_LIST(GS_BIND)
#undef GS_BIND
  g_abi.bound = true;
}

void check(int code, const char* what) {
  TORCH_CHECK(code == 0, "mi355gs: ", what, " failed: ", g_abi.error_string ? g_abi.error_string(code) : "?", " (", code, ")");
}

struct DeviceScope {
  c10::hip::OptionalHIPGuardMasqueradingAsCUDA guard;
  void* stream = nullptr;
  explicit DeviceScope(const Tensor& t) {
    if (t.is_cuda()) {
      guard.set_device(t.device());
      stream = (void*)c10::hip::getCurrentHIPStream(t.device().index()).stream();
    }
  }
  void synchronize(const Tensor& t) const {
    if (t.is_cuda()) c10::hip::getCurrentHIPStream(t.device().index()).synchronize();
  }
};

void wait_for_count(const int32_t* count, const DeviceScope& dev, const Tensor& t) {
  if (!t.is_cuda()) return;
  std::optional<py::gil_scoped_release> nogil;
  if (PyGILState_Check()) nogil.emplace();
  const auto t0 = std::chrono::steady_clock::now();
  for (unsigned spin = 0;; ++spin) {
    if (*reinterpret_cast<const volatile int32_t*>(count) >= 0) return;
    if ((spin & 1023u) == 1023u && std::chrono::steady_clock::now() - t0 > std::chrono::milliseconds(2)) break;
  }
  dev.synchronize(t);
  TORCH_CHECK(*reinterpret_cast<const volatile int32_t*>(count) >= 0, "mi355gs: the forward did not report its instance count");
}

void wait_for_words(Tensor words, int64_t sentinel, Tensor like, int64_t timeout_us) {
  TORCH_CHECK(words.scalar_type() == at::kInt && !words.is_cuda() && words.is_contiguous(), "wait_for_words: an int32 host tensor");
  const volatile int32_t* w = words.data_ptr<int32_t>();
  const int64_t n = words.numel();
  auto all_there = [&]() {
    for (int64_t i = 0; i < n; ++i)
      if (w[i] == (int32_t)sentinel) return false;
    return true;
  };
  if (all_there()) return;
  {
    std::optional<py::gil_scoped_release> nogil;
    if (PyGILState_Check()) nogil.emplace();
    const auto t0 = std::chrono::steady_clock::now();
    for (unsigned spin = 0;; ++spin) {
      if (all_there()) return;
      if ((spin & 1023u) == 1023u && std::chrono::steady_clock::now() - t0 > std::chrono::microseconds(timeout_us)) break;
    }
    if (like.is_cuda()) {
      const DeviceScope dev(like);
      dev.synchronize(like);
    }
  }
  TORCH_CHECK(all_there(), "mi355gs: the step did not report its results");
}

Tensor f32c(const Tensor& t, const char* name, const Tensor& like) {
  TORCH_CHECK(t.is_cuda() || g_abi.allow_cpu, "instantsplat_amd operators run on the GPU only (got a CPU tensor; there is no CPU fallback)");
  TORCH_CHECK(t.scalar_type() == at::kFloat, "expected float32, got ", t.scalar_type(), " (", name, ")");
  TORCH_CHECK(t.device() == like.device(), "tensors on different devices: ", like.device(), " vs ", t.device(), " (", name, ")");
  return t.is_contiguous() ? t : t.contiguous();
}
float* fp(const Tensor& t) { return t.defined() && t.numel() ? t.data_ptr<float>() : nullptr; }

Tensor empty_bytes(size_t n, const Tensor& like) {
  return at::empty({(int64_t)(n > 0 ? n : 1)}, like.options().dtype(at::kByte));
}

struct HostClock {
  std::chrono::steady_clock::time_point t0 = std::chrono::steady_clock::now();
  double* acc;
  explicit HostClock(double* a) : acc(a) {}
  ~HostClock() { *acc += std::chrono::duration<double, std::micro>(std::chrono::steady_clock::now() - t0).count(); }
};
double g_host_us[6] = {0, 0, 0, 0, 0, 0};

struct GateRecord {
  Tensor scratch;
  const float* gate = nullptr;
  std::vector<c10::weak_intrusive_ptr<c10::StorageImpl>> storage;
  int64_t numel[7] = {0, 0, 0, 0, 0, 0, 0};
  int64_t version[7] = {0, 0, 0, 0, 0, 0, 0};
  bool valid = false;
};
std::mutex g_gate_mutex;
GateRecord g_gates;

template <class... T> bool any_requires_grad(const T&... t) {
  if (!at::GradMode::is_enabled()) return false;
  bool any = false;
  ((any = any || (t.defined() && t.requires_grad())), ...);
  return any;
}
thread_local bool t_backward_follows = false;
struct BackwardFollows {
  explicit BackwardFollows(bool v) { t_backward_follows = v; }
  ~BackwardFollows() { t_backward_follows = false; }
};

struct ZeroGrad { Tensor buf; uint32_t version = 0; };
std::mutex g_zero_mutex;
std::map<std::string, ZeroGrad> g_zero_pool;
bool g_share_zero_grad = true;
Tensor zero_grad_like(const Tensor& like) {
  if (!g_share_zero_grad) return at::zeros_like(like);
  std::ostringstream key;
  key << like.device() << ":" << like.sizes() << "@" << like.data_ptr();
  std::lock_guard<std::mutex> lock(g_zero_mutex);
  if (g_zero_pool.size() > 8 && !g_zero_pool.count(key.str())) g_zero_pool.clear();
  ZeroGrad& z = g_zero_pool[key.str()];
  if (!z.buf.defined()) {
    z.buf = at::zeros_like(like, like.options().requires_grad(false), at::MemoryFormat::Contiguous);
    z.version = z.buf._version();
  } else if (z.buf._version() != z.version) {
    z.buf.zero_();
    z.version = z.buf._version();
  }
// ... 172 lines not shown
    ctx->mark_non_differentiable({f.radii, visible});
    ctx->set_materialize_grads(false);
    return {f.color, f.radii, visible};
  }

  static variable_list backward(AutogradContext* ctx, variable_list grad_out) {
    HostClock clock(&g_host_us[1]);
    const auto saved = ctx->get_saved_variables();
    const Tensor &xyz = saved[0], &rot = saved[1], &scaling = saved[2], &opl = saved[3], &f_dc = saved[4], &f_rest = saved[5],
                 &pose = saved[6], &radii = saved[7], &geom = saved[8], &tiles = saved[9], &binning = saved[10], &bg = saved[11],
                 &view = saved[12], &proj = saved[13], &origin = saved[14], &color = saved[15];
    const auto dims = ctx->saved_data["dims"].toIntVector();
    const auto sc = ctx->saved_data["scalars"].toDoubleVector();
    const int P = (int)dims[0], D = (int)dims[1], W = (int)dims[2], H = (int)dims[3];
    const int64_t R = dims[4];
    if (!grad_out[0].defined()) return variable_list(21);
    const Tensor g = f32c(grad_out[0], "grad_color", xyz);
    const DeviceScope dev(xyz);
    Tensor d_xyz = at::empty_like(xyz), d_rot = at::empty_like(rot), d_scaling = at::empty_like(scaling), d_opl = at::empty_like(opl),
           d_fdc = at::empty_like(f_dc), d_m2d = at::empty_like(xyz);
    Tensor d_frest = D == 0 ? zero_grad_like(f_rest) : at::empty_like(f_rest);
    const auto pose_table = ctx->saved_data["pose_table"].toIntVector();
    const int64_t pose_rows = pose_table[0], pose_index = pose_table[1];
    Tensor d_pose_store = at::empty({pose_rows > 0 ? pose_rows * 7 : 7}, xyz.options());
    Tensor d_pose = d_pose_store;
    if (pose_rows > 0) {
      d_pose = at::empty({0}, xyz.options());
      d_pose.set_(d_pose_store.storage(), 7 * pose_index, {7}, {1});
    }
    const auto [scratch, scratch_is_clear] = backward_scratch(ctx, saved[16], xyz, binning, R, P, W, H);
    Tensor pose_scratch = at::empty({16 * (((int64_t)P + 255) / 256) + 32}, xyz.options());
    check(g_abi.posed_backward(dev.stream, P, D, W, H, fp(bg), fp(xyz), fp(f_dc), fp(f_rest), fp(opl), fp(scaling), (float)sc[2], fp(rot),
                               fp(pose), fp(view), fp(proj), fp(origin), (float)sc[0], (float)sc[1], geom.data_ptr(), tiles.data_ptr(),
                               binning.data_ptr(), R, radii.data_ptr<int32_t>(), fp(color), fp(g), scratch.data_ptr(), fp(pose_scratch),
                               fp(d_xyz), fp(d_m2d), fp(d_fdc), D ? fp(d_frest) : nullptr, fp(d_opl), fp(d_scaling), fp(d_rot),
                               fp(d_pose_store), (int)pose_rows, (int)pose_index, scratch_is_clear, 0),
          "posed_backward");
    {
      std::lock_guard<std::mutex> lock(g_gate_mutex);
      g_pose_table.valid = pose_rows > 0;
      if (pose_rows > 0) {
        g_pose_table.storage = d_pose_store.storage().getWeakStorageImpl();
        g_pose_table.rows = pose_rows; g_pose_table.index = pose_index;
      }
      const Tensor* outs[7] = {&d_xyz, &d_fdc, &d_frest, &d_opl, &d_scaling, &d_rot, &d_pose};
      g_gates.storage.clear();
      for (int k = 0; k < 7; ++k) {
        g_gates.storage.push_back(outs[k]->storage().getWeakStorageImpl());
        g_gates.numel[k] = outs[k]->numel();
        g_gates.version[k] = (int64_t)outs[k]->_version();
      }
      g_gates.scratch = scratch;
      g_gates.gate = reinterpret_cast<const float*>(static_cast<const char*>(scratch.data_ptr()) + g_abi.grad_gate_offset(P));
      g_gates.valid = true;
    }
    Tensor none;
    return {d_xyz, d_rot, d_scaling, d_opl, d_fdc, d_frest, d_pose, d_m2d, none, none, none, none,
            none, none, none, none, none, none, none, none, none};
  }
};

std::vector<Tensor> render_posed(Tensor xyz, Tensor rot, Tensor scaling, Tensor opl, Tensor f_dc, Tensor f_rest, Tensor pose,
                                 Tensor means2D, Tensor bg, Tensor view, Tensor proj, Tensor origin, int64_t H, int64_t W,
                                 double tanfovx, double tanfovy, double scale_modifier, int64_t D, int64_t capacity, int64_t count_hint,
                                 Tensor count_slot) {
  const BackwardFollows scope(any_requires_grad(xyz, rot, scaling, opl, f_dc, f_rest, pose, means2D));
  return RenderPosedFn::apply(xyz, rot, scaling, opl, f_dc, f_rest, pose, means2D, bg, view, proj, origin, H, W, tanfovx, tanfovy,
                              scale_modifier, D, capacity, count_hint, count_slot);
}

struct RasterizeFn : public torch::autograd::Function<RasterizeFn> {
  using OptTensor = c10::optional<Tensor>;
  static variable_list forward(AutogradContext* ctx, Tensor means3D_, Tensor means2D, OptTensor sh_, OptTensor colors_, Tensor opac_,
                               OptTensor scales_, OptTensor rot_, OptTensor cov_, OptTensor sh_rest_, Tensor bg_, Tensor view_, Tensor proj_,
                               Tensor campos_,
                               int64_t H, int64_t W, double tanfovx, double tanfovy, double scale_modifier, int64_t D, bool prefiltered,
                               int64_t capacity, int64_t count_hint, Tensor count_slot) {
    TORCH_CHECK(g_abi.bound, "mi355gs torch binding: bind() has not been called");
    HostClock clock(&g_host_us[0]);
    (void)means2D;
    auto opt = [&](const OptTensor& t, const char* name, const Tensor& like) {
      return (t.has_value() && t->defined() && t->numel()) ? f32c(*t, name, like) : Tensor();
    };
    const Tensor means3D = f32c(means3D_, "means3D", means3D_), opac = f32c(opac_, "opacities", means3D);
    const Tensor sh = opt(sh_, "sh", means3D), colors = opt(colors_, "colors_precomp", means3D), scales = opt(scales_, "scales", means3D),
                 rot = opt(rot_, "rotations", means3D), cov = opt(cov_, "cov3Ds_precomp", means3D), sh_rest = opt(sh_rest_, "sh_rest", means3D);
    const Tensor bg = f32c(bg_, "bg", means3D), view = f32c(view_, "viewmatrix", means3D), proj = f32c(proj_, "projmatrix", means3D),
                 campos = f32c(campos_, "campos", means3D);
    TORCH_CHECK(means3D.dim() == 2 && means3D.size(1) == 3, "means3D must have dimensions (num_points, 3)");
    const int P = (int)means3D.size(0);
    const int M = sh.defined() ? (int)(sh.size(1) + (sh_rest.defined() ? sh_rest.size(1) : 0)) : 0;
    const DeviceScope dev(means3D);
    FrameForward f(means3D, P, count_slot);
    f.run(dev, means3D, P, (int)W, (int)H, bg, capacity, count_hint, [&](const FrameForward& frame) {
      check(g_abi.forward_preprocess(dev.stream, P, (int)D, M, (int)W, (int)H, fp(means3D), fp(sh), fp(sh_rest), fp(colors), fp(opac), fp(scales),
                                     (float)scale_modifier, fp(rot), fp(cov), fp(view), fp(proj), fp(campos), (float)tanfovx, (float)tanfovy,
                                     prefiltered ? 1 : 0, frame.radii.data_ptr<int32_t>(), frame.geom.data_ptr(), frame.tiles.data_ptr(), frame.count, nullptr,
                                     frame.scratch.defined() ? frame.scratch.data_ptr() : nullptr, 0),
            "raster_forward_preprocess");
    });
    ctx->saved_data["dims"] = std::vector<int64_t>{P, D, M, W, H, f.R};
    ctx->saved_data["scalars"] = std::vector<double>{tanfovx, tanfovy, scale_modifier};
    ctx->saved_data["opacity_shape"] = opac_.sizes().vec();
    ctx->saved_data["scratch_is_clear"] = f.scratch.defined();
    ctx->save_for_backward({means3D, sh, colors, opac, scales, rot, cov, sh_rest, f.radii, f.geom, f.tiles, f.binning, bg, view, proj, campos,
                            f.color, f.scratch});
    ctx->mark_non_differentiable({f.radii});
    ctx->set_materialize_grads(false);
    return {f.color, f.radii};
  }

  static variable_list backward(AutogradContext* ctx, variable_list grad_out) {
    if (!grad_out[0].defined()) return variable_list(23);
    const auto saved = ctx->get_saved_variables();
    const Tensor &means3D = saved[0], &sh = saved[1], &colors = saved[2], &opac = saved[3], &scales = saved[4], &rot = saved[5], &cov = saved[6],
                 &sh_rest = saved[7], &radii = saved[8], &geom = saved[9], &tiles = saved[10], &binning = saved[11], &bg = saved[12],
                 &view = saved[13], &proj = saved[14], &campos = saved[15], &color = saved[16];
    const auto dims = ctx->saved_data["dims"].toIntVector();
    const auto sc = ctx->saved_data["scalars"].toDoubleVector();
    const int P = (int)dims[0], D = (int)dims[1], M = (int)dims[2], W = (int)dims[3], H = (int)dims[4];
    const int64_t R = dims[5];
    const Tensor g = f32c(grad_out[0], "grad_color", means3D);
    const DeviceScope dev(means3D);
    const auto o = means3D.options();
    Tensor d_means3D = at::empty({P, 3}, o), d_means2D = at::empty({P, 3}, o), d_opac = at::empty({P}, o), d_col = at::empty({P, 3}, o);
    Tensor d_sh, d_shr, d_scales, d_rot, d_cov;
    if (sh.defined()) d_sh = at::empty({P, sh_rest.defined() ? 1 : M, 3}, o);
    if (sh_rest.defined()) d_shr = at::empty({P, M - 1, 3}, o);
    if (cov.defined()) d_cov = at::empty({P, 6}, o); else { d_scales = at::empty({P, 3}, o); d_rot = at::empty({P, 4}, o); }
    const auto [scratch, scratch_is_clear] = backward_scratch(ctx, saved[17], means3D, binning, R, P, W, H);
    check(g_abi.raster_backward(dev.stream, P, D, M, W, H, fp(bg), fp(means3D), fp(sh), fp(sh_rest), fp(colors), fp(opac), fp(scales), (float)sc[2],
                                fp(rot), fp(cov), fp(view), fp(proj), fp(campos), (float)sc[0], (float)sc[1], geom.data_ptr(), tiles.data_ptr(),
                                binning.data_ptr(), R, radii.data_ptr<int32_t>(), fp(color), fp(g), scratch.data_ptr(), fp(d_means3D), fp(d_means2D),
                                fp(d_sh), fp(d_shr), fp(d_col), fp(d_opac), fp(d_scales), fp(d_rot), fp(d_cov), scratch_is_clear, 0),
          "raster_backward");
    Tensor none;
    const auto shape = ctx->saved_data["opacity_shape"].toIntVector();
    return {d_means3D, d_means2D, d_sh, sh.defined() ? none : d_col, d_opac.reshape(shape), d_scales, d_rot, d_cov, d_shr,
            none, none, none, none, none, none, none, none, none, none, none, none, none, none};
  }
};

std::vector<Tensor> rasterize(Tensor means3D, Tensor means2D, c10::optional<Tensor> sh, c10::optional<Tensor> colors, Tensor opac,
                              c10::optional<Tensor> scales, c10::optional<Tensor> rot, c10::optional<Tensor> cov, c10::optional<Tensor> sh_rest,
                              Tensor bg, Tensor view, Tensor proj, Tensor campos, int64_t H, int64_t W, double tanfovx, double tanfovy,
                              double scale_modifier, int64_t D, bool prefiltered, int64_t capacity, int64_t count_hint, Tensor count_slot) {
  const Tensor none;
  auto val = [&](const c10::optional<Tensor>& t) -> const Tensor& { return t.has_value() ? *t : none; };
  const BackwardFollows scope(any_requires_grad(means3D, means2D, opac, val(sh), val(colors), val(scales), val(rot), val(cov), val(sh_rest)));
  return RasterizeFn::apply(means3D, means2D, sh, colors, opac, scales, rot, cov, sh_rest, bg, view, proj, campos, H, W,
                            tanfovx, tanfovy, scale_modifier, D, prefiltered, capacity, count_hint, count_slot);
}

struct L1SsimLossFn : public torch::autograd::Function<L1SsimLossFn> {
  static variable_list forward(AutogradContext* ctx, Tensor img1, Tensor img2, double lambda_dssim) {
    TORCH_CHECK(g_abi.bound, "mi355gs torch binding: bind() has not been called");
    HostClock clock(&g_host_us[2]);
    const Tensor a = f32c(img1, "img1", img1), b = f32c(img2, "img2", a);
    TORCH_CHECK(a.dim() == 4 && a.sizes() == b.sizes(), "fused_ssim expects two [B,C,H,W] tensors of equal shape");
    const int B = (int)a.size(0), C = (int)a.size(1), H = (int)a.size(2), W = (int)a.size(3);
    const DeviceScope dev(a);
    Tensor scratch = empty_bytes(g_abi.ssim_scratch_bytes(B, C, H, W), a);
    Tensor out = at::empty({2}, a.options());
    Tensor loss = at::empty({}, a.options());
    Tensor grad = at::empty_like(a);
    check(g_abi.l1_ssim_loss_fused(dev.stream, B, C, H, W, fp(a), fp(b), scratch.data_ptr(), (float)lambda_dssim, fp(out), fp(out) + 1,
                                   fp(loss), fp(grad)),
          "l1_ssim_loss_fused");
    ctx->save_for_backward({grad});
    ctx->mark_non_differentiable({out});
    ctx->set_materialize_grads(false);
    return {loss, out};
  }
  static variable_list backward(AutogradContext* ctx, variable_list grad_out) {
    HostClock clock(&g_host_us[3]);
    Tensor none;
    if (!grad_out[0].defined()) return {none, none, none};
    const auto saved = ctx->get_saved_variables();
    return {saved[0] * grad_out[0], none, none};
  }
};

std::vector<Tensor> l1_ssim_loss(Tensor img1, Tensor img2, double lambda_dssim) { return L1SsimLossFn::apply(img1, img2, lambda_dssim); }

struct L1LossFn : public torch::autograd::Function<L1LossFn> {
  static Tensor forward(AutogradContext* ctx, Tensor a_, Tensor b_) {
    TORCH_CHECK(g_abi.bound, "mi355gs torch binding: bind() has not been called");
    const Tensor a = f32c(a_, "network_output", a_), b = f32c(b_, "gt", a);
    TORCH_CHECK(a.sizes() == b.sizes() && a.numel() > 0, "l1_loss expects two non-empty tensors of equal shape");
    const DeviceScope dev(a);
    Tensor scratch = empty_bytes(g_abi.l1_scratch_bytes(a.numel()), a);
    Tensor out = at::empty({}, a.options());
    check(g_abi.l1_loss_forward(dev.stream, a.numel(), fp(a), fp(b), scratch.data_ptr(), fp(out)), "l1_loss_forward");
    ctx->save_for_backward({a, b});
    return out;
  }
  static variable_list backward(AutogradContext* ctx, variable_list grad_out) {
    const auto saved = ctx->get_saved_variables();
    const Tensor &a = saved[0], &b = saved[1];
    const Tensor g = f32c(grad_out[0], "grad", a);
    const DeviceScope dev(a);
    Tensor d = at::empty_like(a);
    check(g_abi.l1_loss_backward(dev.stream, a.numel(), fp(a), fp(b), fp(g), fp(d)), "l1_loss_backward");
    return {d, Tensor()};
  }
};

Tensor l1_loss(Tensor a, Tensor b) { return L1LossFn::apply(a, b); }

std::vector<Tensor> loss_pair_forward(Tensor img1, Tensor img2) {
  TORCH_CHECK(g_abi.bound, "mi355gs torch binding: bind() has not been called");
  HostClock clock(&g_host_us[2]);
  const Tensor a = f32c(img1, "img1", img1), b = f32c(img2, "img2", a);
  TORCH_CHECK((a.dim() == 3 || a.dim() == 4) && a.sizes() == b.sizes() && a.numel() > 0, "the loss pair expects two [C,H,W] or [B,C,H,W] tensors of equal shape");
  const int64_t o = a.dim() == 4 ? 1 : 0;
  const int B = o ? (int)a.size(0) : 1, C = (int)a.size(o), H = (int)a.size(o + 1), W = (int)a.size(o + 2);
  const DeviceScope dev(a);
  Tensor scratch = empty_bytes(g_abi.ssim_scratch_bytes(B, C, H, W), a);
  Tensor means = at::empty({2}, a.options());
  Tensor dmap = at::empty_like(a);
  check(g_abi.pair_forward(dev.stream, B, C, H, W, fp(a), fp(b), scratch.data_ptr(), fp(dmap)), "l1_ssim_pair_forward");
  return {means, scratch, dmap, a, b};
}

struct LossAffineFn : public torch::autograd::Function<LossAffineFn> {
  static Tensor forward(AutogradContext* ctx, Tensor image, Tensor a, Tensor b, Tensor dmap, Tensor means, Tensor scratch,
                        std::vector<int64_t> ops, std::vector<double> consts, double c_l1, double c_ssim, Tensor host_slot, double ticket,
                        c10::optional<Tensor> unit_grad_) {
    const Tensor unit_grad = unit_grad_.has_value() ? *unit_grad_ : Tensor();
    TORCH_CHECK(g_abi.bound, "mi355gs torch binding: bind() has not been called");
    TORCH_CHECK(ops.size() == consts.size() && !ops.empty() && ops.size() <= MI355GS_LOSS_PROGRAM_MAX, "loss_affine: 1..16 operations");
    TORCH_CHECK(image.numel() == a.numel() && means.numel() == 2, "loss_affine: image and its contiguous copy differ in size");
    const int64_t o = a.dim() == 4 ? 1 : 0;
    const int B = o ? (int)a.size(0) : 1, C = (int)a.size(o), H = (int)a.size(o + 1), W = (int)a.size(o + 2);
    const DeviceScope dev(a);
    int32_t op32[MI355GS_LOSS_PROGRAM_MAX]; float k32[MI355GS_LOSS_PROGRAM_MAX];
    for (size_t i = 0; i < ops.size(); ++i) { op32[i] = (int32_t)ops[i]; k32[i] = (float)consts[i]; }
    Tensor out = at::empty({}, a.options());
    float* host_out = nullptr;
    if (host_slot.defined() && host_slot.numel() >= 2) {
      TORCH_CHECK(host_slot.scalar_type() == at::kFloat && !host_slot.is_cuda() && host_slot.is_contiguous(), "loss_affine: the host slot is float32[2] host memory");
      host_out = host_slot.data_ptr<float>();
    }
    Tensor d;
    const bool with_grad = unit_grad.defined() && unit_grad.numel() == 1;
    if (with_grad) {
      d = at::empty_like(a);
      check(g_abi.program_eval_grad(dev.stream, (int)ops.size(), op32, k32, B, C, H, W, scratch.data_ptr(), fp(means) + 1, fp(means), fp(out), host_out,
                                    (float)ticket, fp(a), fp(b), fp(dmap), (float)c_l1, (float)c_ssim, fp(d)),
            "loss_program_eval_grad");
    } else {
      check(g_abi.program_eval(dev.stream, (int)ops.size(), op32, k32, B, C, H, W, scratch.data_ptr(), fp(means) + 1, fp(means), fp(out), host_out,
                               (float)ticket),
            "loss_program_eval");
    }
    ctx->save_for_backward({a, b, dmap, with_grad ? d : Tensor()});
    ctx->saved_data["c"] = std::vector<double>{c_l1, c_ssim};
    ctx->saved_data["shape"] = image.sizes().vec();
    ctx->saved_data["unit_grad_ptr"] = with_grad ? (int64_t)(uintptr_t)unit_grad.data_ptr() : (int64_t)0;
    return out;
  }
  static variable_list backward(AutogradContext* ctx, variable_list grad_out) {
    HostClock clock(&g_host_us[3]);
    const auto saved = ctx->get_saved_variables();
    const Tensor &a = saved[0], &b = saved[1], &dmap = saved[2];
    const auto c = ctx->saved_data["c"].toDoubleVector();
    Tensor none;
    const int64_t unit_ptr = ctx->saved_data["unit_grad_ptr"].toInt();
    if (unit_ptr != 0 && saved.size() > 3 && saved[3].defined() && (int64_t)(uintptr_t)grad_out[0].data_ptr() == unit_ptr) {
      return {saved[3].view(ctx->saved_data["shape"].toIntVector()), none, none, none, none, none, none, none, none, none, none, none, none};
    }
    const Tensor g = f32c(grad_out[0].reshape({1}), "grad", a);
    const DeviceScope dev(a);
    Tensor d = at::empty_like(a);
    check(g_abi.pair_backward(dev.stream, a.numel(), fp(a), fp(b), fp(dmap), fp(g), (float)c[0], fp(g), (float)c[1], fp(d)), "l1_ssim_pair_backward");
    return {d.view(ctx->saved_data["shape"].toIntVector()), none, none, none, none, none, none, none, none, none, none, none, none};
  }
};

Tensor loss_affine(Tensor image, Tensor a, Tensor b, Tensor dmap, Tensor means, Tensor scratch, std::vector<int64_t> ops,
                   std::vector<double> consts, double c_l1, double c_ssim, Tensor host_slot, double ticket) {
  return LossAffineFn::apply(image, a, b, dmap, means, scratch, ops, consts, c_l1, c_ssim, host_slot, ticket, c10::optional<Tensor>());
}

py::object wait_for_loss(Tensor host_slot, double ticket, int64_t timeout_us) {
  TORCH_CHECK(host_slot.scalar_type() == at::kFloat && !host_slot.is_cuda() && host_slot.numel() >= 2, "wait_for_loss: float32[2] host memory");
  const volatile float* w = host_slot.data_ptr<float>();
  const float want = (float)ticket;
  auto taken_over = [want](float have) {
    if (have == 0.f || have == want) return false;
    float ahead = have - want;
    if (ahead < 0.f) ahead += 16000000.f;
    return ahead < 8000000.f;
  };
  bool there = w[1] == want;
  if (!there && !taken_over(w[1])) {
    py::gil_scoped_release nogil;
    const auto t0 = std::chrono::steady_clock::now();
    for (unsigned spin = 0;; ++spin) {
      const float have = w[1];
      if (have == want) { there = true; break; }
      if (taken_over(have)) break;
      if ((spin & 1023u) == 1023u && std::chrono::steady_clock::now() - t0 > std::chrono::microseconds(timeout_us)) break;
    }
  }
  if (!there) return py::none();
  const float v = w[0];
  if (w[1] != want) return py::none();
  return py::float_((double)v);
}

Tensor loss_affine_backward(Tensor image, Tensor a, Tensor b, Tensor dmap, Tensor means, Tensor scratch, std::vector<int64_t> ops,
                            std::vector<double> consts, double c_l1, double c_ssim, Tensor host_slot, double ticket) {
  static std::mutex mu;
  static std::map<std::string, std::pair<Tensor, uint32_t>> ones;
  Tensor one;
  {
    std::lock_guard<std::mutex> lock(mu);
    std::ostringstream key;
    key << a.device();
    auto& slot = ones[key.str()];
    if (!slot.first.defined() || slot.first._version() != slot.second) {
      slot.first = at::ones({}, a.options().requires_grad(false));
      slot.second = slot.first._version();
    }
    one = slot.first;
  }
  const bool will_run = at::GradMode::is_enabled() && image.requires_grad();
  Tensor out = LossAffineFn::apply(image, a, b, dmap, means, scratch, ops, consts, c_l1, c_ssim, host_slot, ticket, will_run ? c10::optional<Tensor>(one) : c10::optional<Tensor>());
  if (!out.requires_grad()) return out;
  py::gil_scoped_release nogil;
  torch::autograd::backward({out}, {one}, false, false);
  return out;
}

struct SsimFn : public torch::autograd::Function<SsimFn> {
  static Tensor forward(AutogradContext* ctx, Tensor img1, Tensor img2, bool train, bool valid) {
    TORCH_CHECK(g_abi.bound, "mi355gs torch binding: bind() has not been called");
    const Tensor a = f32c(img1, "img1", img1), b = f32c(img2, "img2", a);
    TORCH_CHECK(a.dim() == 4 && a.sizes() == b.sizes(), "fused_ssim expects two [B,C,H,W] tensors of equal shape");
    const int B = (int)a.size(0), C = (int)a.size(1), H = (int)a.size(2), W = (int)a.size(3);
    TORCH_CHECK(!valid || (H > 10 && W > 10), "fused_ssim(padding=\"valid\") needs images larger than the 11x11 window");
    const DeviceScope dev(a);
    Tensor dm1, dm2, dm3;
    if (train) { dm1 = at::empty_like(a); dm2 = at::empty_like(a); dm3 = at::empty_like(a); }
    Tensor scratch = empty_bytes(g_abi.ssim_scratch_bytes(B, C, H, W), a);
    Tensor out = at::empty({2}, a.options());
    check(g_abi.ssim_forward(dev.stream, B, C, H, W, fp(a), fp(b), fp(dm1), fp(dm2), fp(dm3), scratch.data_ptr(), fp(out),
                             valid ? nullptr : fp(out) + 1, valid ? 1 : 0),
          "ssim_forward");
    if (train) ctx->save_for_backward({a, b, dm1, dm2, dm3});
    ctx->saved_data["flags"] = std::vector<int64_t>{train ? 1 : 0, valid ? 1 : 0};
    return out.select(0, 0).clone();
  }
  static variable_list backward(AutogradContext* ctx, variable_list grad_out) {
    const auto flags = ctx->saved_data["flags"].toIntVector();
    TORCH_CHECK(flags[0] == 1, "fused_ssim was called with train=False; no gradient is available");
    const auto saved = ctx->get_saved_variables();
    const Tensor &a = saved[0], &b = saved[1];
    const int B = (int)a.size(0), C = (int)a.size(1), H = (int)a.size(2), W = (int)a.size(3);
    const DeviceScope dev(a);
    const Tensor scale = f32c(grad_out[0].reshape({1}), "grad", a);
    Tensor grad = at::empty_like(a);
    check(g_abi.ssim_backward(dev.stream, B, C, H, W, fp(a), fp(b), fp(saved[2]), fp(saved[3]), fp(saved[4]), fp(scale), nullptr, fp(grad),
                              (int)flags[1]),
          "ssim_backward");
    Tensor none;
    return {grad, none, none, none};
  }
};

Tensor fused_ssim(Tensor img1, Tensor img2, bool train, bool valid) { return SsimFn::apply(img1, img2, train, valid); }

struct AdamPlan {
  std::vector<Tensor> params, exp_avg, exp_avg_sq, pplr;
  std::vector<int64_t> numel;
  std::vector<int32_t> row;
  double beta1, beta2, eps;
  int64_t last_used_gates = 0;
  std::string last_gate_note;
  Tensor live;
  uint32_t seq = 0;
  std::vector<int64_t> moment_version;
  std::vector<Tensor> owners;

  AdamPlan(std::vector<Tensor> p, std::vector<Tensor> m, std::vector<Tensor> v, std::vector<c10::optional<Tensor>> pp, double b1, double b2,
           double e)
      : params(std::move(p)), exp_avg(std::move(m)), exp_avg_sq(std::move(v)), beta1(b1), beta2(b2), eps(e) {
    const size_t n = params.size();
    TORCH_CHECK(n >= 1 && n <= 8 && exp_avg.size() == n && exp_avg_sq.size() == n && pp.size() == n, "AdamPlan: 1..8 tensors, equal-length lists");
    for (size_t t = 0; t < n; ++t) {
      const Tensor& q = params[t];
      TORCH_CHECK(q.is_cuda() || g_abi.allow_cpu, "instantsplat_amd operators run on the GPU only (got a CPU tensor; there is no CPU fallback)");
      TORCH_CHECK(q.scalar_type() == at::kFloat && q.is_contiguous(), "AdamPlan: parameters must be contiguous float32");
      for (const Tensor* s : {&exp_avg[t], &exp_avg_sq[t]})
        TORCH_CHECK(s->scalar_type() == at::kFloat && s->is_contiguous() && s->device() == q.device() && s->numel() == q.numel(),
                    "AdamPlan: moments must match their parameter");
      numel.push_back(q.numel());
      if (pp[t].has_value() && pp[t]->defined()) {
        const Tensor& l = *pp[t];
        TORCH_CHECK(l.scalar_type() == at::kFloat && l.is_contiguous() && l.device() == q.device() && q.dim() >= 1 && q.size(0) > 0 &&
                        l.numel() == q.size(0),
                    "AdamPlan: per_point_lr must hold one contiguous float32 per point");
        pplr.push_back(l);
        row.push_back((int32_t)(q.numel() / q.size(0)));
      } else {
        pplr.emplace_back();
        row.push_back(1);
      }
    }
  }

  void set_owners(std::vector<Tensor> o) {
    TORCH_CHECK(o.size() == params.size(), "AdamPlan.set_owners: one Parameter per tensor");
    owners = std::move(o);
  }
  bool step_owned(const std::vector<double>& lr, const std::vector<int64_t>& step_counts) {
    const size_t n = params.size();
    if (owners.size() != n) return false;
    std::vector<Tensor> grads(n);
    for (size_t t = 0; t < n; ++t) {
      const Tensor& g = owners[t].grad();
      if (!g.defined() || g.is_sparse() || owners[t].data_ptr() != params[t].data_ptr() || g.numel() != numel[t]) return false;
      grads[t] = g;
    }
    this->step(grads, lr, step_counts);
    return true;
  }
  void zero_owned() {
    for (Tensor& o : owners) o.mutable_grad().reset();
  }

  void step(const std::vector<Tensor>& grads, const std::vector<double>& lr, const std::vector<int64_t>& step) {
    const size_t n = params.size();
    TORCH_CHECK(grads.size() == n && lr.size() == n && step.size() == n, "AdamPlan.step: list lengths");
    HostClock clock(&g_host_us[4]);
    const DeviceScope dev(params[0]);
    int64_t nm[8]; int32_t rw[8], st[8], gidx[8];
    float* pp[8]; const float* gg[8]; float* mm[8]; float* vv[8]; const float* ll[8]; float lrs[8];
    std::vector<Tensor> keep;
    int64_t n_flagged = 0;
    GateRecord rec;
    {
      std::lock_guard<std::mutex> lock(g_gate_mutex);
      rec = g_gates;
    }
    for (size_t t = 0; t < n; ++t) {
      Tensor g = grads[t];
      TORCH_CHECK(g.defined() && g.numel() == numel[t] && g.device() == params[t].device(), "AdamPlan.step: gradient ", t, " does not match its parameter");
      bool mine = false;
      if (rec.valid && g.scalar_type() == at::kFloat && g.is_contiguous() && g.storage_offset() == 0) {
        const c10::StorageImpl* impl = g.storage().unsafeGetStorageImpl();
        for (int k = 0; k < (int)rec.storage.size() && !mine; ++k) {
          auto strong = rec.storage[k].lock();
          if (strong && strong.get() == impl && rec.numel[k] == g.numel() && rec.version[k] == (int64_t)g._version()) { gidx[t] = k; mine = true; }
        }
      }
      if (!mine) {
        std::ostringstream why;
        why << "tensor " << t << ": record " << (rec.valid ? "valid" : "absent") << ", offset " << g.storage_offset() << ", version " << g._version()
            << ", storage " << (const void*)g.storage().unsafeGetStorageImpl() << ", numel " << g.numel();
        last_gate_note = why.str();
      }
      if (!mine) gidx[t] = -1;
      n_flagged += mine ? 1 : 0;
      if (g.scalar_type() != at::kFloat || !g.is_contiguous()) { g = g.to(at::kFloat).contiguous(); keep.push_back(g); }
      nm[t] = numel[t]; rw[t] = row[t]; st[t] = (int32_t)step[t]; lrs[t] = (float)lr[t];
      pp[t] = params[t].data_ptr<float>(); gg[t] = g.data_ptr<float>(); mm[t] = exp_avg[t].data_ptr<float>();
      vv[t] = exp_avg_sq[t].data_ptr<float>(); ll[t] = pplr[t].defined() ? pplr[t].data_ptr<float>() : nullptr;
    }
    const bool gated = n_flagged > 0;
    Tensor scratch;
    if (n_flagged < (int64_t)n) scratch = at::empty({8}, params[0].options());
    last_used_gates = n_flagged;
    bool moments_touched = !live.defined();
    if (moment_version.size() != 2 * n) moment_version.assign(2 * n, -1);
    for (size_t t = 0; t < n; ++t) {
      const int64_t v0 = (int64_t)exp_avg[t]._version(), v1 = (int64_t)exp_avg_sq[t]._version();
      moments_touched = moments_touched || v0 != moment_version[2 * t] || v1 != moment_version[2 * t + 1];
      moment_version[2 * t] = v0; moment_version[2 * t + 1] = v1;
    }
    if (!live.defined()) live = at::zeros({16}, params[0].options().dtype(at::kInt));
    else if (moments_touched) live.zero_();
    if (++seq == 0u) seq = 1u;
    check(g_abi.adam_multi_step(dev.stream, (int)n, nm, rw, pp, gg, mm, vv, ll, lrs, (float)beta1, (float)beta2, (float)eps, st,
                                scratch.defined() ? scratch.data_ptr<float>() : nullptr, gated ? rec.gate : nullptr, gated ? gidx : nullptr,
                                reinterpret_cast<uint32_t*>(live.data_ptr<int32_t>()), seq),
          "adam_multi_step");
  }
};

}

PYBIND11_MODULE(TORCH_EXTENSION_NAME, m) {
  m.doc() = "compiled PyTorch binding of libmi355gs.so's drop-in operators (no compute of its own)";
  m.def("abi_symbols", &abi_symbols, "the C symbols bind() must be given, in the order of the list they are generated from");
  m.def("bind", &bind_abi, "hand over the C-ABI entry points (name -> address) of the loaded libmi355gs build; allow_cpu_tensors: test tier only");
  m.def("l1_loss", &l1_loss, "utils/loss_utils.py::l1_loss as one node (the library's l1_loss forward / backward pair)");
  m.def("render_posed", &render_posed);
  m.def("wait_for_words", &wait_for_words, "spin (GIL released) until no element of an int32 pinned host tensor holds the sentinel; stream wait after timeout_us");
  m.def("pose_row", &pose_row, "GaussianModel.get_RT: row `index` of the [views, 7] pose table as a node the render node's backward cooperates with");
  m.def("rasterize", &rasterize);
  m.def("l1_ssim_loss", &l1_ssim_loss);
  m.def("loss_pair_forward", &loss_pair_forward, "-> [means (l1, ssim: filled by the first loss_affine), partial sums, d(ssim_mean)/dimg1, img1, img2 (contiguous)]: one launch, no autograd node");
  m.def("wait_for_loss", &wait_for_loss, "the value the program kernel stored to a pinned host slot under this ticket, or None (timeout / slot taken over)");
  m.def("loss_affine_backward", &loss_affine_backward, "loss_affine + the engine run of loss.backward() in one call (root gradient: a cached 1)");
  m.def("loss_affine", &loss_affine, "the recorded scalar expression over (l1_mean, ssim_mean) as ONE node on `image`");
  m.def("fused_ssim", &fused_ssim);
  m.def("host_times_us", [](bool reset) {
    std::vector<double> v(g_host_us, g_host_us + 6);
    if (reset) for (double& x : g_host_us) x = 0;
    return v;
  }, "accumulated host microseconds: render fwd (incl. the count wait), render bwd, loss fwd, loss bwd, adam step, count wait");
  m.def("forget_gates", []() { std::lock_guard<std::mutex> lock(g_gate_mutex); g_gates = GateRecord(); });
  m.def("shared_zero_grad", [](bool on) {
    std::lock_guard<std::mutex> lock(g_zero_mutex);
    const bool old = g_share_zero_grad;
    g_share_zero_grad = on;
    if (!on) g_zero_pool.clear();
    return old;
  }, "f_rest's all-zero gradient below its SH degree: true (default) = aliases of one persistent zero buffer, false = a fresh zeros tensor per backward");
  py::class_<AdamPlan>(m, "AdamPlan")
      .def(py::init<std::vector<Tensor>, std::vector<Tensor>, std::vector<Tensor>, std::vector<c10::optional<Tensor>>, double, double, double>())
      .def("step", &AdamPlan::step)
      .def("set_owners", &AdamPlan::set_owners)
      .def("step_owned", &AdamPlan::step_owned)
      .def("zero_owned", &AdamPlan::zero_owned)
      .def_readonly("last_used_gates", &AdamPlan::last_used_gates)
      .def_readonly("last_gate_note", &AdamPlan::last_gate_note);
}
```

### instantsplat_amd/fused_ssim/__init__.py

```python
from __future__ import annotations

import torch

from .. import _lib
from .. import lazy_loss


def _run_forward(img1, img2, train, valid=False):
    L = _lib.lib()
    a, b = _lib.f32c(img1), _lib.f32c(img2)
    if a.dim() != 4 or a.shape != b.shape:
        raise RuntimeError("fused_ssim expects two [B,C,H,W] tensors of equal shape")
    dev = _lib.require_device(a, b)
    B, C, H, W = a.shape
    new = lambda: torch.empty_like(a)
    dm1, dm2, dm3 = (new(), new(), new()) if train else (None, None, None)
    scratch = torch.empty(int(L.mi355gs_ssim_scratch_bytes(B, C, H, W)), dtype=torch.uint8, device=dev)
    if valid and (H <= 10 or W <= 10):
        raise RuntimeError('fused_ssim(padding="valid") needs images larger than the 11x11 window')
    out = torch.empty(2, dtype=torch.float32, device=dev)
    with _lib.on_device(dev):
        _lib.check(L.mi355gs_ssim_forward(_lib.stream_ptr(dev), B, C, H, W, _lib.ptr(a), _lib.ptr(b), _lib.ptr(dm1), _lib.ptr(dm2),
                                          _lib.ptr(dm3), _lib.ptr(scratch), _lib.ptr(out[0:1]), None if valid else _lib.ptr(out[1:2]),
                                          1 if valid else 0), "ssim_forward")
    return a, b, dm1, dm2, dm3, out


def _run_backward(a, b, dm1, dm2, dm3, ssim_scale, l1_scale, valid=False):
    L = _lib.lib()
    dev = a.device
    B, C, H, W = a.shape
    grad = torch.empty_like(a)
    with _lib.on_device(dev):
        _lib.check(L.mi355gs_ssim_backward(_lib.stream_ptr(dev), B, C, H, W, _lib.ptr(a), _lib.ptr(b), _lib.ptr(dm1), _lib.ptr(dm2),
                                           _lib.ptr(dm3), _lib.ptr(ssim_scale), _lib.ptr(l1_scale), _lib.ptr(grad), 1 if valid else 0),
                   "ssim_backward")
    return grad


class _FusedSSIM(torch.autograd.Function):
    @staticmethod
    def forward(ctx, img1, img2, train, valid=False):
        a, b, dm1, dm2, dm3, out = _run_forward(img1, img2, train, valid)
        if train:
            ctx.save_for_backward(a, b, dm1, dm2, dm3)
        ctx.train, ctx.valid = train, valid
        return out[0].clone()

    @staticmethod
    def backward(ctx, g):
        if not ctx.train:
            raise RuntimeError("fused_ssim was called with train=False; no gradient is available")
        a, b, dm1, dm2, dm3 = ctx.saved_tensors
        scale = _lib.f32c(g.reshape(1))
        return _run_backward(a, b, dm1, dm2, dm3, scale, None, ctx.valid), None, None, None


def fused_ssim(img1, img2, padding="same", train=True):
    if padding not in ("same", "valid"):
        raise ValueError(f'padding must be "same" or "valid", got {padding!r}')
    if train and padding == "same" and lazy_loss._LAST[0] is not None and isinstance(img1, torch.Tensor) and isinstance(img2, torch.Tensor):
        half = lazy_loss.ssim_of_pair(img1, img2)
        if half is not None:
            return half
    ext = _lib.compiled()
    if ext is not None:
        return ext.fused_ssim(img1, img2, bool(train), padding == "valid")
    return _FusedSSIM.apply(img1, img2, train, padding == "valid")


_SCRATCH_BYTES = {}


def _scratch_bytes(L, B, C, H, W):
    key = (B, C, H, W)
    n = _SCRATCH_BYTES.get(key)
    if n is None:
        if len(_SCRATCH_BYTES) > 64:
            _SCRATCH_BYTES.clear()
        n = _SCRATCH_BYTES[key] = int(L.mi355gs_ssim_scratch_bytes(B, C, H, W))
    return n


class _FusedL1SSIM(torch.autograd.Function):

    @staticmethod
    def forward(ctx, img1, img2, lambda_dssim):
        L = _lib.lib()
        (a, b), dev = _lib.f32c_on_one_device(img1, img2)
        if a.dim() != 4 or a.shape != b.shape:
            raise RuntimeError("fused_ssim expects two [B,C,H,W] tensors of equal shape")
        B, C, H, W = a.shape
        scratch = torch.empty(_scratch_bytes(L, B, C, H, W), dtype=torch.uint8, device=dev)
        out = torch.empty(2, dtype=torch.float32, device=dev)
        loss = torch.empty((), dtype=torch.float32, device=dev)
        grad = torch.empty_like(a)
        p0 = out.data_ptr()
        with _lib.on_device(dev):
            _lib.check(L.mi355gs_l1_ssim_loss_fused(_lib.stream_ptr(dev), B, C, H, W, _lib.ptr(a), _lib.ptr(b), _lib.ptr(scratch),
                                                    float(lambda_dssim), p0, p0 + 4, _lib.ptr(loss), _lib.ptr(grad)),
                       "l1_ssim_loss_fused")
        ctx.save_for_backward(grad)
        ctx.mark_non_differentiable(out)
        return loss, out

    @staticmethod
    def backward(ctx, g, _):
        (grad,) = ctx.saved_tensors
        return grad * g, None, None


def fused_l1_ssim_loss(img1, img2, lambda_dssim=0.2):
    ext = _lib.compiled()
    if ext is not None:
        return ext.l1_ssim_loss(img1, img2, float(lambda_dssim))
    return _FusedL1SSIM.apply(img1, img2, lambda_dssim)
```

### instantsplat_amd/lazy_loss.py

```python
from __future__ import annotations

import os
import time
import warnings

import numpy as np
import torch

from . import _lib

ENABLED = os.environ.get("MI355GS_LAZY_LOSS", "1") != "0"

OP_L1, OP_SSIM, OP_MULK, OP_ADDK, OP_RSUBK, OP_DIVK, OP_NEG, OP_ADD, OP_SUB = range(9)
PROGRAM_MAX = 16

_PLACEHOLDER = {}


def _placeholder(dev):
    t = _PLACEHOLDER.get(dev)
    if t is None:
        t = _PLACEHOLDER[dev] = torch.full((), float("nan"), dtype=torch.float32, device=dev)
    return t


def _tensor_key(t):
    return (t.data_ptr(), t._version, t.numel(), tuple(t.shape[-3:]))


class Pair:
    __slots__ = ("image", "gt", "image_key", "gt_key", "a", "b", "dmap", "means", "scratch", "dev")

    def __init__(self, image, gt):
        ext = _lib.compiled()
        if ext is not None:
            self.means, self.scratch, self.dmap, self.a, self.b = ext.loss_pair_forward(image, gt)
        else:
            self.means, self.scratch, self.dmap, self.a, self.b = _pair_forward_ctypes(image, gt)
        self.image, self.gt = image, gt
        self.image_key, self.gt_key = _tensor_key(image), _tensor_key(gt)
        self.dev = self.a.device

    @property
    def l1(self):
        return self.means[0]

    @property
    def ssim(self):
        return self.means[1]

    def matches(self, img1, img2):
        return (_tensor_key(img1) == self.image_key and _tensor_key(img2) == self.gt_key and img1.is_contiguous() and img2.is_contiguous()
                and img1.dtype is torch.float32 and img2.dtype is torch.float32 and not img2.requires_grad)


_LAST = [None]


def eligible(network_output, gt):
    return (ENABLED and torch.is_grad_enabled() and network_output.requires_grad and not gt.requires_grad
            and network_output.dim() in (3, 4) and network_output.dtype is torch.float32 and gt.dtype is torch.float32
            and network_output.shape == gt.shape and network_output.numel() > 0 and network_output.device == gt.device
            and (network_output.is_cuda or _lib._TEST_MODE) and network_output.is_contiguous() and gt.is_contiguous()
            and network_output.shape[-3] * (network_output.shape[0] if network_output.dim() == 4 else 1) <= 65535)


def l1_of_pair(network_output, gt):
    rec = _LAST[0] = Pair(network_output, gt)
    return _new(rec, ((OP_L1, 0.0),))


def ssim_of_pair(img1, img2):
    rec = _LAST[0]
    if rec is None or not ENABLED or not torch.is_grad_enabled() or not rec.matches(img1, img2):
        return None
    return _new(rec, ((OP_SSIM, 0.0),))


def forget():
    _LAST[0] = None


def _new(rec, prog):
    t = torch.Tensor._make_subclass(LazyScalar, _placeholder(rec.dev), False)
    t._rec, t._prog, t._real, t._slot = rec, prog, None, None
    return t


def _is_number(k):
    return isinstance(k, (int, float)) and not isinstance(k, bool)


def _is_lazy(x):
    return type(x) is LazyScalar


EARLY_ITEM = os.environ.get("MI355GS_EARLY_ITEM", "1") != "0"
_NO_SLOT = torch.empty(0)
_SLOTS = {}
_N_SLOTS = 64
_TICKET = [0]


def _host_slot(dev):
    ring = _SLOTS.get(dev)
    if ring is None:
        words = torch.zeros(_N_SLOTS, 2, dtype=torch.float32, pin_memory=(dev.type == "cuda"))
        ring = _SLOTS[dev] = [words, [words[i] for i in range(_N_SLOTS)], 0]
    k = ring[2]
    ring[2] = (k + 1) % _N_SLOTS
    t = _TICKET[0] = _TICKET[0] % 16000000 + 1
    return ring[1][k], float(t)


_PARTIALS = {}


def partials(prog):
    c = _PARTIALS.get(prog)
    if c is not None:
        return c
    f = np.float32
    st = []
    for op, k in prog:
        k = f(k)
        if op == OP_L1:
            st.append((f(1), f(0)))
        elif op == OP_SSIM:
            st.append((f(0), f(1)))
        elif op == OP_MULK:
            a = st[-1]
            st[-1] = (a[0] * k, a[1] * k)
        elif op == OP_DIVK:
            a, r = st[-1], f(1) / k
            st[-1] = (a[0] * r, a[1] * r)
        elif op in (OP_RSUBK, OP_NEG):
            a = st[-1]
            st[-1] = (-a[0], -a[1])
        elif op == OP_ADD:
            b, a = st.pop(), st.pop()
            st.append((a[0] + b[0], a[1] + b[1]))
        elif op == OP_SUB:
            b, a = st.pop(), st.pop()
            st.append((a[0] - b[0], a[1] - b[1]))
        elif op != OP_ADDK:
            raise ValueError(f"unknown loss-program operation {op}")
    assert len(st) == 1, prog
    if len(_PARTIALS) > 256:
        _PARTIALS.clear()
    c = _PARTIALS[prog] = (float(st[0][0]), float(st[0][1]))
    return c


def materialize(x):
    rec = x._rec
    need_grad = torch.is_grad_enabled() and rec.image.requires_grad
    real = x._real
    if real is not None and (real.requires_grad or not need_grad):
        return real
    c_l1, c_ssim = partials(x._prog)
    ops, consts = [p[0] for p in x._prog], [float(p[1]) for p in x._prog]
    ext = _lib.compiled()
    if ext is not None:
        slot, ticket = _host_slot(rec.dev) if EARLY_ITEM else (None, 0.0)
        real = ext.loss_affine(rec.image, rec.a, rec.b, rec.dmap, rec.means, rec.scratch, ops, consts, c_l1, c_ssim, _NO_SLOT if slot is None else slot, ticket)
        x._slot = (slot, ticket) if slot is not None else None
    else:
        real = _LossAffine.apply(rec.image, rec, ops, consts, c_l1, c_ssim)
        x._slot = None
    x._real = real
    return real


def _unary(x, op, k=0.0):
    if len(x._prog) >= PROGRAM_MAX:
        return NotImplemented
    return _new(x._rec, x._prog + ((op, float(k)),))


def _binary(a, b, op):
    if a._rec is not b._rec or len(a._prog) + len(b._prog) >= PROGRAM_MAX:
        return NotImplemented
    return _new(a._rec, a._prog + b._prog + ((op, 0.0),))


def _h_mul(a, b):
    if _is_lazy(a) and _is_number(b):
        return _unary(a, OP_MULK, b)
    if _is_lazy(b) and _is_number(a):
        return _unary(b, OP_MULK, a)
    return NotImplemented


def _h_add(a, b, alpha=1):
    if alpha != 1:
        return NotImplemented
    if _is_lazy(a) and _is_lazy(b):
        return _binary(a, b, OP_ADD)
    if _is_lazy(a) and _is_number(b):
        return _unary(a, OP_ADDK, b)
    if _is_lazy(b) and _is_number(a):
        return _unary(b, OP_ADDK, a)
    return NotImplemented


def _h_sub(a, b, alpha=1):
    if alpha != 1:
        return NotImplemented
    if _is_lazy(a) and _is_lazy(b):
        return _binary(a, b, OP_SUB)
    if _is_lazy(a) and _is_number(b):
        return _unary(a, OP_ADDK, -b)
    if _is_lazy(b) and _is_number(a):
        return _unary(b, OP_RSUBK, a)
    return NotImplemented


def _h_rsub(a, b, alpha=1):
    return _h_sub(b, a, alpha)


def _h_div(a, b, rounding_mode=None):
    if rounding_mode is None and _is_lazy(a) and _is_number(b) and b != 0:
        return _unary(a, OP_DIVK, b)
    return NotImplemented


def _h_neg(a):
    return _unary(a, OP_NEG) if _is_lazy(a) else NotImplemented


_T = torch.Tensor
_HANDLERS = {}
for _fns, _h in (((_T.__mul__, _T.__rmul__, _T.mul, torch.mul, _T.multiply, torch.multiply), _h_mul),
                 ((_T.__add__, _T.__radd__, _T.add, torch.add), _h_add),
                 ((_T.__sub__, _T.sub, torch.sub, _T.subtract, torch.subtract), _h_sub),
                 ((_T.__rsub__, torch.rsub), _h_rsub),
                 ((_T.__truediv__, _T.div, torch.div, _T.true_divide, torch.true_divide, _T.divide, torch.divide), _h_div),
                 ((_T.__neg__, _T.neg, torch.neg, _T.negative, torch.negative), _h_neg)):
    for _f in _fns:
        _HANDLERS[_f] = _h


def _real_args(x):
    if _is_lazy(x):
        return materialize(x)
    if isinstance(x, (list, tuple)):
        return type(x)(_real_args(v) for v in x)
    if isinstance(x, dict):
        return {k: _real_args(v) for k, v in x.items()}
    return x


class LazyScalar(torch.Tensor):

    def __mul__(self, k):
        return _unary(self, OP_MULK, k) if _is_number(k) and len(self._prog) < PROGRAM_MAX else _T.__mul__(self, k)

    __rmul__ = __mul__

    def __add__(self, k):
        if type(k) is LazyScalar:
            out = _binary(self, k, OP_ADD)
            return out if out is not NotImplemented else _T.__add__(self, k)
        return _unary(self, OP_ADDK, k) if _is_number(k) and len(self._prog) < PROGRAM_MAX else _T.__add__(self, k)

    __radd__ = __add__

    def __sub__(self, k):
        if type(k) is LazyScalar:
            out = _binary(self, k, OP_SUB)
            return out if out is not NotImplemented else _T.__sub__(self, k)
        return _unary(self, OP_ADDK, -k) if _is_number(k) and len(self._prog) < PROGRAM_MAX else _T.__sub__(self, k)

    def __rsub__(self, k):
        return _unary(self, OP_RSUBK, k) if _is_number(k) and len(self._prog) < PROGRAM_MAX else _T.__rsub__(self, k)

    def __truediv__(self, k):
        return _unary(self, OP_DIVK, k) if _is_number(k) and k != 0 and len(self._prog) < PROGRAM_MAX else _T.__truediv__(self, k)

    def __neg__(self):
        return _unary(self, OP_NEG) if len(self._prog) < PROGRAM_MAX else _T.__neg__(self)

    def backward(self, gradient=None, retain_graph=None, create_graph=False, inputs=None):
        if gradient is None and not retain_graph and not create_graph and inputs is None and torch.is_grad_enabled():
            real = self._real
            if real is None or not real.requires_grad:
                ext = _lib.compiled()
                rec = self._rec
                if ext is not None and rec.image.requires_grad:
                    c_l1, c_ssim = partials(self._prog)
                    prog = self._prog
                    slot, ticket = _host_slot(rec.dev) if EARLY_ITEM else (None, 0.0)
                    self._real = ext.loss_affine_backward(rec.image, rec.a, rec.b, rec.dmap, rec.means, rec.scratch, [p[0] for p in prog],
                                                          [p[1] for p in prog], c_l1, c_ssim, _NO_SLOT if slot is None else slot, ticket)
                    self._slot = (slot, ticket) if slot is not None else None
                    return None
        return materialize(self).backward(gradient, retain_graph, create_graph, inputs)

    def item(self):
        real = materialize(self)
        slot = self._slot
        if slot is not None:
            ext = _lib.compiled()
            if ext is not None:
                t0 = time.perf_counter()
                v = ext.wait_for_loss(slot[0], slot[1], 200_000)
                if v is not None:
                    return v
                if time.perf_counter() - t0 > 0.1:
                    global EARLY_ITEM
                    EARLY_ITEM = False
                    warnings.warn("instantsplat_amd.lazy_loss: the pinned loss slot did not receive the value within 200 ms; "
                                  "loss.item() falls back to an ordinary read for the rest of the process (MI355GS_EARLY_ITEM=0)")
        return real.item()

    def __float__(self):
        return float(materialize(self).detach())

    def detach(self):
        return materialize(self).detach()

    @classmethod
    def __torch_function__(cls, func, types, args=(), kwargs=None):
        kwargs = kwargs or {}
        h = _HANDLERS.get(func)
        if h is not None:
            try:
                out = h(*args, **kwargs)
            except TypeError:
                out = NotImplemented
            if out is not NotImplemented:
                return out
        args, kwargs = _real_args(args), _real_args(kwargs)
        with torch._C.DisableTorchFunctionSubclass():
            return func(*args, **kwargs)


def _pair_forward_ctypes(img1, img2):
    L = _lib.lib()
    (a, b), dev = _lib.f32c_on_one_device(img1, img2)
    if a.dim() not in (3, 4) or a.shape != b.shape or a.numel() == 0:
        raise RuntimeError("the loss pair expects two [C,H,W] or [B,C,H,W] tensors of equal shape")
    B = a.shape[0] if a.dim() == 4 else 1
    C, H, W = a.shape[-3:]
    scratch = torch.empty(int(L.mi355gs_ssim_scratch_bytes(B, C, H, W)), dtype=torch.uint8, device=dev)
    means = torch.empty(2, dtype=torch.float32, device=dev)
    dmap = torch.empty_like(a)
    with _lib.on_device(dev):
        _lib.check(L.mi355gs_l1_ssim_pair_forward(_lib.stream_ptr(dev), B, C, H, W, _lib.ptr(a), _lib.ptr(b), _lib.ptr(scratch),
                                                  _lib.ptr(dmap)), "l1_ssim_pair_forward")
    return means, scratch, dmap, a, b


class _LossAffine(torch.autograd.Function):
    @staticmethod
    def forward(ctx, image, rec, ops, consts, c_l1, c_ssim):
        import ctypes
        L = _lib.lib()
        dev = rec.dev
        out = torch.empty((), dtype=torch.float32, device=dev)
        n = len(ops)
        a = rec.a
        B = a.shape[0] if a.dim() == 4 else 1
        C, H, W = a.shape[-3:]
        with _lib.on_device(dev):
            _lib.check(L.mi355gs_loss_program_eval(_lib.stream_ptr(dev), n, (ctypes.c_int32 * n)(*ops), (ctypes.c_float * n)(*consts), B, C, H, W,
                                                   _lib.ptr(rec.scratch), rec.means.data_ptr() + 4, rec.means.data_ptr(), _lib.ptr(out), None, 0.0),
                       "loss_program_eval")
        ctx.save_for_backward(rec.a, rec.b, rec.dmap)
        ctx.c, ctx.shape = (c_l1, c_ssim), image.shape
        return out

    @staticmethod
    def backward(ctx, g):
        a, b, dmap = ctx.saved_tensors
        L = _lib.lib()
        g = _lib.f32c(g.reshape(1))
        d = torch.empty_like(a)
        with _lib.on_device(a.device):
            _lib.check(L.mi355gs_l1_ssim_pair_backward(_lib.stream_ptr(a.device), a.numel(), _lib.ptr(a), _lib.ptr(b), _lib.ptr(dmap),
                                                       _lib.ptr(g), ctx.c[0], _lib.ptr(g), ctx.c[1], _lib.ptr(d)), "l1_ssim_pair_backward")
        return d.view(ctx.shape), None, None, None, None, None
```

### instantsplat_amd/train.py

```python
from __future__ import annotations

import ctypes
import gc
import math
import random
import time
from dataclasses import dataclass, field
from typing import List, Optional

import torch

from . import _lib
from .arguments import ModelParams, OptimizationParams, PipelineParams
from .optim import PerPointAdam
from .fused_ssim import fused_l1_ssim_loss, fused_ssim
from .diff_gaussian_rasterization import BinningPolicy, binning_hint
from .gaussian_renderer import render
from .pose_utils import quadmultiply
from .scene import GaussianModel, confidence_to_lr_modifiers
from .synthetic import PointmapScene


from .loss_utils import l1_loss
from .lazy_loss import LazyScalar
# ... 154 lines not shown


WAIT_WITH_EVENT = False
_WAIT = {"timeout_us": 50_000, "ema_us": None}
_NOT_YET = -2


def _wait_for_words(words: torch.Tensor, dev):
    ext = _lib.compiled()
    if ext is not None:
        t0 = time.perf_counter()
        ext.wait_for_words(words, _NOT_YET, _device_token(dev), _WAIT["timeout_us"])
        dt_us = 1e6 * (time.perf_counter() - t0)
        _WAIT["ema_us"] = dt_us if _WAIT["ema_us"] is None else 0.9 * _WAIT["ema_us"] + 0.1 * dt_us
        _WAIT["timeout_us"] = int(min(max(50_000, 8 * _WAIT["ema_us"]), 5_000_000))
        return
    for spin in range(200_000):
        if int(words[0]) != _NOT_YET and int(words[1]) != _NOT_YET:
            return
    torch.cuda.current_stream(dev).synchronize()
    if int(words[0]) == _NOT_YET or int(words[1]) == _NOT_YET:
        raise RuntimeError("mi355gs: the step did not report its results")


_DEVICE_TOKEN = {}


def _device_token(dev):
    t = _DEVICE_TOKEN.get(dev)
    if t is None:
        t = _DEVICE_TOKEN[dev] = torch.empty(1, device=dev)
    return t


def _fused_synced_iteration(st: TrainState):
    tr = getattr(st, "_trainer", None)
    if tr is None:
        st._prepared = None
        with torch.no_grad():
            for cam in st.cameras:
                with binning_hint(hint_key(st, cam)):
                    render(cam, st.gaussians, st.pipe, st.background, camera_pose=st.gaussians.get_RT(cam.uid))
        need = max(BinningPolicy.known[hint_key(st, c)] for c in st.cameras)
        tr = st._trainer = FusedTrainer(st, int(BinningPolicy.slack * need) + BinningPolicy.pad)
        st._host_words = torch.zeros(4, dtype=torch.int32, pin_memory=(tr.dev.type == "cuda"))
        st._loss_slots = [st._host_words[0:1].view(torch.float32), st._host_words[2:3].view(torch.float32)]
        st._count_slots = [st._host_words[1:2], st._host_words[3:4]]
    cuda = tr.dev.type == "cuda"

    def enqueue_forward_backward(slot):
        saved = _host_state(st, tr)
        args = tr.prepare()
        st._host_words[2 * slot: 2 * slot + 2] = _NOT_YET
        cam = tr.launch(args, st._loss_slots[slot], st._count_slots[slot], defer_optimizer=True)
        ev = None
        if cuda and WAIT_WITH_EVENT:
            ev = torch.cuda.Event()
            ev.record(torch.cuda.current_stream(tr.dev))
        return saved, args, slot, ev, cam

    pre = getattr(st, "_prepared", None)
    st._prepared = None
    saved, args, slot, ev, cam = pre if pre is not None else enqueue_forward_backward(0)
    tr.apply_optimizer(gated=True)
    nxt = None
    if args["it"] < st.opt.iterations:
        nxt = enqueue_forward_backward(slot ^ 1)
    if ev is not None:
        ev.synchronize()
    elif cuda:
        _wait_for_words(st._host_words[2 * slot: 2 * slot + 2], tr.dev)
    loss, r = float(st._loss_slots[slot][0]), int(st._count_slots[slot][0])
    BinningPolicy.known[hint_key(st, cam)] = int(r)
    if r > tr.capacity:
        _restore_host_state(st, tr, saved)
        tr.close()
        st._trainer = None
        return None
    st._prepared = nxt
    if r * 1.2 + 1024 > tr.capacity:
        cancel_prepared(st)
        tr.close()
        st._trainer = None
    return loss


def train_iteration(st: TrainState, fused_loss: bool = True, sync_loss: bool = True, fused_step: bool = False):
    if fused_step and sync_loss and fused_loss is True and FusedTrainer.supported(st):
        out = _fused_synced_iteration(st)
        if out is not None:
            st.last_loss = out
            return out
    cancel_prepared(st)
    loss = _forward_backward_step(st, fused_loss)
    out = loss.item() if sync_loss else loss
    _optimizer_step(st)
    st.last_loss = out
    return out


class FusedTrainer:

    ORDER = ("_xyz", "_features_dc", "_features_rest", "_opacity", "_scaling", "_rotation", "P")

    @staticmethod
    def supported(st: TrainState) -> bool:
        g, o, p = st.gaussians, st.opt, st.pipe
        if g.max_sh_degree != 3 or not o.optim_pose or p.debug or p.compute_cov3D_python or p.convert_SHs_python:
            return False
        if not isinstance(g.optimizer, PerPointAdam) or len(g.optimizer.param_groups) != 7:
            return False
        grp = g.optimizer.param_groups
        if any(x["weight_decay"] != 0 or x["betas"] != grp[0]["betas"] or x["eps"] != grp[0]["eps"] for x in grp):
            return False
        if [x["name"] for x in grp] != ["xyz", "f_dc", "f_rest", "opacity", "scaling", "rotation", "pose"]:
            return False
        dev = g._xyz.device
        W, H = int(st.cameras[0].image_width), int(st.cameras[0].image_height)
        ok = lambda t, shape: (isinstance(t, torch.Tensor) and t.dtype == torch.float32 and t.is_contiguous() and t.device == dev
                               and tuple(t.shape) == shape)
        for cam in st.cameras:
            if int(cam.image_width) != W or int(cam.image_height) != H or not ok(cam.projection_matrix, (4, 4)):
                return False
            if cam.uid >= len(st.gt_images) or not ok(st.gt_images[cam.uid], (3, H, W)):
                return False
        return ok(st.background, (3,))

    def __init__(self, st: TrainState, capacity: int):
        self.st, self.capacity = st, int(capacity)
        g = st.gaussians
        L = _lib.lib()
        self.params = [getattr(g, n) for n in self.ORDER]
        dev = _lib.require_device(*[p.data for p in self.params])
        self.dev = dev
        for p in self.params:
            s = g.optimizer.state[p]
            if len(s) == 0:
                s["step"], s["exp_avg"], s["exp_avg_sq"] = 0, torch.zeros_like(p), torch.zeros_like(p)
        P, V = g._xyz.shape[0], g.P.shape[0]
        cam = st.cameras[0]
        self.W, self.H = int(cam.image_width), int(cam.image_height)
        nbytes = L.mi355gs_trainer_workspace_bytes(P, self.W, self.H, V, self.capacity)
        self.workspace = torch.empty(int(nbytes), dtype=torch.uint8, device=dev)
        PTR = ctypes.c_void_p * 7
        m = PTR(*[g.optimizer.state[p]["exp_avg"].data_ptr() for p in self.params])
        v = PTR(*[g.optimizer.state[p]["exp_avg_sq"].data_ptr() for p in self.params])
        pplr = g.optimizer.param_groups[0].get("per_point_lr")
        self._keep = (m, v, pplr)
        self.handle = L.mi355gs_trainer_create(P, self.W, self.H, V, self.capacity, *[_lib.ptr(p.data) for p in self.params], m, v,
                                               _lib.ptr(pplr), _lib.ptr(self.workspace))
        if not self.handle:
            raise RuntimeError("mi355gs_trainer_create failed")
        self.num_rendered = torch.zeros(1, dtype=torch.int32, device=dev)
        self._count_ring = torch.zeros(self.COUNT_RING, dtype=torch.int32, pin_memory=(dev.type == "cuda"))
        self._count_next = 0

    def close(self):
        handle, self.handle = getattr(self, "handle", None), None
        if handle:
            try:
                _lib.lib().mi355gs_trainer_destroy(ctypes.c_void_p(handle))
            except Exception:
                pass

    def gradients(self) -> dict:
        L, base, out = _lib.lib(), self.workspace.data_ptr(), {}
        for k, (name, p) in enumerate(zip(self.ORDER, self.params)):
            addr = L.mi355gs_trainer_grad(ctypes.c_void_p(self.handle), k)
            off, nbytes = int(addr) - base, 4 * p.numel()
            assert addr and 0 <= off and off + nbytes <= self.workspace.numel(), (name, off)
            out[name] = self.workspace[off:off + nbytes].view(torch.float32).view(p.shape).clone()
        return out

    __del__ = close

    COUNT_RING = 256

    def prepare(self):
        st = self.st
        st.iteration += 1
        it, g, opt = st.iteration, st.gaussians, st.opt
        g.update_learning_rate(it)
        if it % 1000 == 0:
            g.oneupSHdegree()
        cam = _pick_camera(st)
        bg = torch.rand(3, device=self.dev) if opt.random_background else st.background
        do_opt = it < opt.iterations
        grp = g.optimizer.param_groups
        steps = []
        for p in self.params:
            s = g.optimizer.state[p]
            if do_opt:
                s["step"] += 1
            steps.append(max(s["step"], 1))
        b1, b2 = grp[0]["betas"]
        F7, I7 = ctypes.c_float * 7, ctypes.c_int32 * 7
        return dict(it=it, cam=cam, bg=bg, do_opt=do_opt, sh=int(g.active_sh_degree), lr=F7(*[float(x["lr"]) for x in grp]), steps=I7(*steps),
                    b1=float(b1), b2=float(b2), eps=float(grp[0]["eps"]), lam=float(opt.lambda_dssim))

    def launch(self, a, loss_slot: torch.Tensor, count_out: torch.Tensor, defer_optimizer: bool = False):
        cam = a["cam"]
        with _lib.on_device(self.dev):
            _lib.check(_lib.lib().mi355gs_trainer_step(
                ctypes.c_void_p(self.handle), _lib.stream_ptr(self.dev), int(cam.uid), a["sh"], _lib.ptr(self.st.gt_images[cam.uid]),
                _lib.ptr(cam.projection_matrix), math.tan(cam.FoVx * 0.5), math.tan(cam.FoVy * 0.5), _lib.ptr(a["bg"]),
                a["lr"], a["steps"], a["b1"], a["b2"], a["eps"], a["lam"],
                1 if (a["do_opt"] and not defer_optimizer) else 0, _lib.ptr(loss_slot), _lib.ptr(count_out)), "trainer_step")
        self._pending_opt = (a["lr"], a["steps"], a["b1"], a["b2"], a["eps"]) if a["do_opt"] else None
        return cam

    def step(self, loss_slot: torch.Tensor, defer_optimizer: bool = False, verify_async: bool = True, record_event: bool = True,
             count_out: torch.Tensor | None = None):
        a = self.prepare()
        if verify_async:
            if len(BinningPolicy.pending) >= self.COUNT_RING:
                raise RuntimeError("more unverified frames than count slots: call BinningPolicy.poll() at least every "
                                   f"{self.COUNT_RING} steps")
            k = self._count_next
            self._count_next = (k + 1) % self.COUNT_RING
            count_out = self._count_ring[k:k + 1]
        elif count_out is None:
            count_out = self.num_rendered
        cam = self.launch(a, loss_slot, count_out, defer_optimizer)
        if not verify_async:
            return cam
        with binning_hint(hint_key(self.st, cam), tag=a["it"]):
            BinningPolicy.defer(count_out, self.capacity, self.dev, event=record_event)
        return cam

    def apply_optimizer(self, gated: bool = False):
        if self._pending_opt is not None:
            lr, steps, b1, b2, eps = self._pending_opt
            with _lib.on_device(self.dev):
                _lib.check(_lib.lib().mi355gs_trainer_optimizer_step(ctypes.c_void_p(self.handle), _lib.stream_ptr(self.dev), lr, steps,
                                                                     b1, b2, eps, 1 if gated else 0), "trainer_optimizer_step")
            self._pending_opt = None


class RunAhead:

    def __init__(self, st: TrainState, window: int = 10, fused_loss: bool = True, fused_step: bool = True):
        self.st, self.window, self.fused = st, window, fused_loss
        self.fused_step, self.trainer = fused_step, None
        cancel_prepared(st)
        dev = st.background.device
        self.ring = torch.zeros(window, dtype=torch.float32, device=dev)
        self.ema = 0.0
        self.n_in_window = 0
        self.replays = 0
        self.partial_replays = 0
        BinningPolicy.reset("bounded")
        self.snap, self._host_hist = None, []
        if fused_step and FusedTrainer.supported(st):
            self._make_trainer()
        if self.trainer is None:
            self._snapshot()

    def _make_trainer(self):
        st = self.st
        with torch.no_grad():
            for cam in st.cameras:
                if hint_key(st, cam) not in BinningPolicy.known:
                    mode, BinningPolicy.mode = BinningPolicy.mode, "exact"
                    with binning_hint(hint_key(st, cam)):
                        render(cam, st.gaussians, st.pipe, st.background, camera_pose=st.gaussians.get_RT(cam.uid))
                    BinningPolicy.mode = mode
        need = max(BinningPolicy.known[hint_key(st, c)] for c in st.cameras)
        if self.trainer is not None:
            self.trainer.close()
        self.trainer = FusedTrainer(st, int(BinningPolicy.slack * need) + BinningPolicy.pad)

    def _tensors(self):
        g = self.st.gaussians
        return [g._xyz, g._features_dc, g._features_rest, g._opacity, g._scaling, g._rotation, g.P]

    def _snapshot(self):
        st, g = self.st, self.st.gaussians
        opt_state = []
        for p in self._tensors():
            s = g.optimizer.state.get(p, {})
            opt_state.append(None if not s else (s["step"], s["exp_avg"].clone(), s["exp_avg_sq"].clone()))
        self.snap = dict(params=[p.detach().clone() for p in self._tensors()], opt=opt_state, iteration=st.iteration,
                         stack=list(st.viewpoint_stack), rng=st.rng.getstate(), sh=g.active_sh_degree, ema=self.ema,
                         lrs=[grp["lr"] for grp in g.optimizer.param_groups])

    def _restore(self):
        st, g, sn = self.st, self.st.gaussians, self.snap
        with torch.no_grad():
            for p, v, o in zip(self._tensors(), sn["params"], sn["opt"]):
                p.copy_(v)
                p.grad = None
                if o is None:
                    g.optimizer.state.pop(p, None)
                else:
                    s = g.optimizer.state[p]
                    s["step"] = o[0]
                    s["exp_avg"].copy_(o[1])
                    s["exp_avg_sq"].copy_(o[2])
        st.iteration, st.viewpoint_stack, g.active_sh_degree, self.ema = sn["iteration"], list(sn["stack"]), sn["sh"], sn["ema"]
        st.rng.setstate(sn["rng"])
        for grp, lr in zip(g.optimizer.param_groups, sn["lrs"]):
            grp["lr"] = lr

    def step(self):
        if self.trainer is not None and FusedTrainer.supported(self.st):
            if self.snap is not None and self.n_in_window == 0:
                self.snap = None
            self._host_hist.append(_host_state(self.st, self.trainer))
            self.trainer.step(self.ring[self.n_in_window:self.n_in_window + 1], record_event=False)
        else:
            if self.snap is None:
                self.flush()
                self._snapshot()
            loss = _forward_backward_step(self.st, self.fused)
            self.ring[self.n_in_window] = loss.detach()
            _optimizer_step(self.st)
        self.n_in_window += 1
        if self.n_in_window == self.window:
            return self.flush()
        return None

    def flush(self):
        n = self.n_in_window
        if n == 0:
            return self.ema
        losses = self.ring[:n].tolist()
        overflowed = BinningPolicy.poll(block=True)
        if overflowed:
            self.replays += 1
            first = 0
            if len(self._host_hist) == n:
                its = [h[0] + 1 for h in self._host_hist]
                first = min(its.index(t) for t in overflowed if t in its) if any(t in its for t in overflowed) else 0
                _restore_host_state(self.st, self.trainer, self._host_hist[first])
                losses = losses[:first]
                self.partial_replays += first > 0
            else:
                self._restore()
                losses = []
            BinningPolicy.mode = "exact"
            for _ in range(n - first):
                l = _forward_backward_step(self.st, self.fused)
                losses.append(float(l.item()))
                _optimizer_step(self.st)
            BinningPolicy.mode = "bounded"
            if self.trainer is not None:
                self._make_trainer()
        for l in losses:
            self.ema = 0.4 * l + 0.6 * self.ema
        self.st.last_loss = losses[-1]
        self.n_in_window = 0
        self._host_hist = []
        if self.trainer is not None:
            need = max(BinningPolicy.known.get(hint_key(self.st, c), 0) for c in self.st.cameras)
            if need * 1.2 + 1024 > self.trainer.capacity:
                self._make_trainer()
        if self.trainer is None:
# ... 151 lines not shown
```

Before: 3534.

## Precompute and cache per-view SSIM target statistics to skip target blurs

Adds a kernel that computes the Gaussian-blurred mean and second moment of each ground-truth image. The trainer precomputes these maps once per view, and the Python loss paths cache them keyed on tensor identity and version. The fused L1+SSIM kernel gains a cached variant that runs only three of the five separable-blur channels and reads mu2 and E[y^2] from global memory instead. This cuts arithmetic and LDS traffic per iteration, at the cost of extra global reads, memory held for the stats maps, and invalidation logic for when the ground truth changes.

After: 3578, median of 6. 1.01x the previous value.

```diff
diff --git a/include/mi355gs.h b/include/mi355gs.h
--- a/include/mi355gs.h
+++ b/include/mi355gs.h
@@ -79,6 +79,11 @@
                           const float* ssim_grad_scale, const float* l1_grad_scale, float* dL_dimg1, int padding_valid);
 int mi355gs_l1_ssim_loss_fused(void* stream, int B, int C, int H, int W, const float* img1, const float* img2, void* scratch,
                                float lambda_dssim, float* ssim_mean, float* l1_mean, float* loss, float* dloss_dimg1);
+size_t mi355gs_ssim_target_stats_bytes(int B, int C, int H, int W);
+int mi355gs_ssim_target_stats(void* stream, int B, int C, int H, int W, const float* img2, void* stats);
+int mi355gs_l1_ssim_loss_fused_cached(void* stream, int B, int C, int H, int W, const float* img1, const float* img2, void* scratch,
+                                      float lambda_dssim, float* ssim_mean, float* l1_mean, float* loss, float* dloss_dimg1,
+                                      const void* target_stats);
 
 size_t mi355gs_l1_scratch_bytes(int64_t n);
 int mi355gs_l1_loss_forward(void* stream, int64_t n, const float* a, const float* b, void* scratch, float* mean_out);
@@ -95,6 +100,8 @@
 #define MI355GS_LOSS_OP_SUB 8
 int mi355gs_l1_ssim_pair_forward(void* stream, int B, int C, int H, int W, const float* img1, const float* img2, void* scratch,
                                  float* dssim_dimg1);
+int mi355gs_l1_ssim_pair_forward_cached(void* stream, int B, int C, int H, int W, const float* img1, const float* img2, void* scratch,
+                                        float* dssim_dimg1, const void* target_stats);
 int mi355gs_l1_ssim_pair_backward(void* stream, int64_t n, const float* img1, const float* img2, const float* dssim_dimg1,
                                   const float* g_l1, float c_l1, const float* g_ssim, float c_ssim, float* d_img1);
 int mi355gs_loss_program_eval(void* stream, int n_ops, const int32_t* ops, const float* consts, int B, int C, int H, int W,
@@ -147,6 +154,7 @@
                          float lambda_dssim, int do_optimizer_step, float* loss_out, int32_t* num_rendered_out);
 int mi355gs_trainer_optimizer_step(void* trainer, void* stream, const float* lr, const int32_t* step, float beta1, float beta2,
                                    float eps, int commit_gate);
+int mi355gs_trainer_set_target_stats(void* trainer, int view, const void* stats);
 void mi355gs_trainer_destroy(void* trainer);
 const float* mi355gs_trainer_grad(void* trainer, int k);
 
diff --git a/instantsplat_amd/_lib.py b/instantsplat_amd/_lib.py
--- a/instantsplat_amd/_lib.py
+++ b/instantsplat_amd/_lib.py
@@ -43,7 +43,11 @@
     "mi355gs_ssim_forward": (c_int, [_P, c_int, c_int, c_int, c_int, _P, _P, _P, _P, _P, _P, _P, _P, c_int]),
     "mi355gs_ssim_backward": (c_int, [_P, c_int, c_int, c_int, c_int, _P, _P, _P, _P, _P, _P, _P, _P, c_int]),
     "mi355gs_l1_ssim_loss_fused": (c_int, [_P, c_int, c_int, c_int, c_int, _P, _P, _P, c_float, _P, _P, _P, _P]),
+    "mi355gs_ssim_target_stats_bytes": (c_size_t, [c_int, c_int, c_int, c_int]),
+    "mi355gs_ssim_target_stats": (c_int, [_P, c_int, c_int, c_int, c_int, _P, _P]),
+    "mi355gs_l1_ssim_loss_fused_cached": (c_int, [_P, c_int, c_int, c_int, c_int, _P, _P, _P, c_float, _P, _P, _P, _P, _P]),
     "mi355gs_l1_ssim_pair_forward": (c_int, [_P, c_int, c_int, c_int, c_int, _P, _P, _P, _P]),
+    "mi355gs_l1_ssim_pair_forward_cached": (c_int, [_P, c_int, c_int, c_int, c_int, _P, _P, _P, _P, _P]),
     "mi355gs_l1_ssim_pair_backward": (c_int, [_P, c_int64, _P, _P, _P, _P, c_float, _P, c_float, _P]),
     "mi355gs_loss_program_eval": (c_int, [_P, c_int, _P, _P, c_int, c_int, c_int, c_int, _P, _P, _P, _P, _P, c_float]),
     "mi355gs_loss_program_eval_grad": (c_int, [_P, c_int, _P, _P, c_int, c_int, c_int, c_int, _P, _P, _P, _P, _P, c_float, _P, _P, _P, c_float,
@@ -67,6 +71,7 @@
     "mi355gs_trainer_step": (c_int, [_P, _P, c_int, c_int, _P, _P, c_float, c_float, _P, _P, _P, c_float, c_float, c_float, c_float,
                                      c_int, _P, _P]),
     "mi355gs_trainer_optimizer_step": (c_int, [_P, _P, _P, _P, c_float, c_float, c_float, c_int]),
+    "mi355gs_trainer_set_target_stats": (c_int, [_P, c_int, _P]),
     "mi355gs_trainer_destroy": (None, [_P]),
     "mi355gs_trainer_grad": (_P, [_P, c_int]),
     "mi355gs_tracker_workspace_bytes": (c_size_t, [c_int, c_int, c_int, c_int64]),
diff --git a/instantsplat_amd/csrc/ssim.hip b/instantsplat_amd/csrc/ssim.hip
--- a/instantsplat_amd/csrc/ssim.hip
+++ b/instantsplat_amd/csrc/ssim.hip
@@ -240,12 +240,17 @@
 constexpr int FDR = 8, FD_GROUPS = FT / FDR;
 static_assert(FC_GROUPS * FR1 <= FTHREADS && FD_GROUPS * FR1 <= FTHREADS && FT % FDR == 0 && FDR % 2 == 0, "one item per thread");
 
-__global__ __launch_bounds__(FTHREADS) void k_l1_ssim_fused(int H, int W, const float* __restrict__ img1, const float* __restrict__ img2,
-                                                        float ks , float kl ,
-                                                        float* __restrict__ dL_dimg1, float* __restrict__ partial ) {
+template <bool CACHED>
+__global__ __launch_bounds__(FTHREADS)
+void k_l1_ssim_fused(int H, int W, const float* __restrict__ img1, const float* __restrict__ img2,
+                     const float* __restrict__ mu2_map , const float* __restrict__ eyy_map,
+                     float ks , float kl ,
+                     float* __restrict__ dL_dimg1, float* __restrict__ partial ) {
+  constexpr int NM = CACHED ? 3 : 5;
+  constexpr int PX = 0, PY = 1, PXX = CACHED ? 1 : 2, PYY = 3, PXY = CACHED ? 2 : 4;
   __shared__ float s_xy[2][FR2][FXP];
-  __shared__ float s_h[5][FR2][FHP];
-  static_assert(3 * FR1 * FDP <= 2 * FR2 * FXP && 3 * FR1 * FEP <= 5 * FR2 * FHP, "aliased LDS buffers must fit");
+  __shared__ float s_h[NM][FR2][FHP];
+  static_assert(3 * FR1 * FDP <= 2 * FR2 * FXP && 3 * FR1 * FEP <= NM * FR2 * FHP, "aliased LDS buffers must fit");
   __shared__ float s_red[2][FTHREADS / 64];
   float (*s_d)[FR1][FDP] = reinterpret_cast<float (*)[FR1][FDP]>(&s_xy[0][0][0]);
   float (*s_e)[FR1][FEP] = reinterpret_cast<float (*)[FR1][FEP]>(&s_h[0][0][0]);
@@ -257,10 +262,12 @@
   const float* p2 = img2 + po;
   const int ec = tid & 31, er0 = (tid >> 5) * FER;
   float ex[FER], ey[FER];
-#pragma unroll
-  for (int j = 0; j < FER; ++j) {
-    const size_t o = (size_t)min(oy + er0 + j, H - 1) * W + min(ox + ec, W - 1);
-    ex[j] = p1[o]; ey[j] = p2[o];
+  if constexpr (!CACHED) {
+#pragma unroll
+    for (int j = 0; j < FER; ++j) {
+      const size_t o = (size_t)min(oy + er0 + j, H - 1) * W + min(ox + ec, W - 1);
+      ex[j] = p1[o]; ey[j] = p2[o];
+    }
   }
   {
     float vx[F_STAGE_ITERS], vy[F_STAGE_ITERS];
@@ -299,15 +306,23 @@
         const int k = t - j;
         if (k >= 0 && k < 11) {
           const float w = gw(k);
-          sx[j] = fmaf(w, x[t], sx[j]); sy[j] = fmaf(w, y[t], sy[j]);
-          sxx[j] = fmaf(w, xx, sxx[j]); syy[j] = fmaf(w, yy, syy[j]); sxy[j] = fmaf(w, xy, sxy[j]);
+          if constexpr (CACHED) {
+            sx[j] = fmaf(w, x[t], sx[j]); sxx[j] = fmaf(w, xx, sxx[j]); sxy[j] = fmaf(w, xy, sxy[j]);
+          } else {
+            sx[j] = fmaf(w, x[t], sx[j]); sy[j] = fmaf(w, y[t], sy[j]);
+            sxx[j] = fmaf(w, xx, sxx[j]); syy[j] = fmaf(w, yy, syy[j]); sxy[j] = fmaf(w, xy, sxy[j]);
+          }
         }
       }
     }
 #pragma unroll
     for (int j = 0; j < 6; ++j) {
-      s_h[0][r][c0 + j] = sx[j]; s_h[1][r][c0 + j] = sy[j]; s_h[2][r][c0 + j] = sxx[j]; s_h[3][r][c0 + j] = syy[j];
-      s_h[4][r][c0 + j] = sxy[j];
+      if constexpr (CACHED) {
+        s_h[PX][r][c0 + j] = sx[j]; s_h[PXX][r][c0 + j] = sxx[j]; s_h[PXY][r][c0 + j] = sxy[j];
+      } else {
+        s_h[PX][r][c0 + j] = sx[j]; s_h[PY][r][c0 + j] = sy[j]; s_h[PXX][r][c0 + j] = sxx[j]; s_h[PYY][r][c0 + j] = syy[j];
+        s_h[PXY][r][c0 + j] = sxy[j];
+      }
     }
   }
   __syncthreads();
@@ -315,11 +330,21 @@
   if (tid < FR1 * FC_GROUPS) {
     const int c = tid % FR1, r0 = (tid / FR1) * FCR;
     float mo[5][FCR];
+    if constexpr (CACHED) {
+      const int gx = ox + c - HALO;
+#pragma unroll
+      for (int j = 0; j < FCR; ++j) {
+        const size_t o = po + (size_t)min(max(oy + r0 + j - HALO, 0), H - 1) * W + min(max(gx, 0), W - 1);
+        mo[1][j] = mu2_map[o]; mo[3][j] = eyy_map[o];
+      }
+    }
 #pragma unroll
     for (int m = 0; m < 5; ++m) {
+      if (CACHED && (m == PY || m == PYY)) continue;
+      const int mp = CACHED ? m / 2 : m;
       float v[FCR + 10];
 #pragma unroll
-      for (int t = 0; t < FCR + 10; ++t) v[t] = s_h[m][min(r0 + t, FR2 - 1)][c];
+      for (int t = 0; t < FCR + 10; ++t) v[t] = s_h[mp][min(r0 + t, FR2 - 1)][c];
 #pragma unroll
       for (int j = 0; j < FCR; ++j) {
         float a = 0.f;
@@ -352,6 +377,13 @@
     for (int j = 0; j < FCR; ++j)
       if (FR1 % FCR == 0 || r0 + j < FR1) { s_d[0][r0 + j][c] = mo[0][j]; s_d[1][r0 + j][c] = mo[1][j]; s_d[2][r0 + j][c] = mo[2][j]; }
   }
+  if constexpr (CACHED) {
+#pragma unroll
+    for (int j = 0; j < FER; ++j) {
+      const size_t o = (size_t)min(oy + er0 + j, H - 1) * W + min(ox + ec, W - 1);
+      ex[j] = p1[o]; ey[j] = p2[o];
+    }
+  }
   __syncthreads();
   if (tid < FR1 * FD_GROUPS) {
     const int r = tid % FR1, c0 = (tid / FR1) * FDR;
@@ -414,6 +446,39 @@
     for (int w = 0; w < FTHREADS / 64; ++w) { ta += s_red[0][w]; tb += s_red[1][w]; }
     partial[2 * b] = ta;
     partial[2 * b + 1] = tb;
+  }
+}
+
+constexpr int ST = 16, STH = ST + 2 * HALO;
+__global__ __launch_bounds__(ST * ST) void k_ssim_target_stats(int H, int W, const float* __restrict__ img2, float* __restrict__ mu2_map,
+                                                               float* __restrict__ eyy_map) {
+  __shared__ float s_y[STH][STH + 1];
+  __shared__ float s_r[2][STH][ST + 1];
+  const int tid = threadIdx.x;
+  const int ox = blockIdx.x * ST, oy = blockIdx.y * ST;
+  const size_t po = (size_t)blockIdx.z * H * W;
+  for (int i = tid; i < STH * STH; i += ST * ST) {
+    const int r = i / STH, c = i - r * STH;
+    const int gy = oy + r - HALO, gx = ox + c - HALO;
+    s_y[r][c] = (gy >= 0 && gy < H && gx >= 0 && gx < W) ? img2[po + (size_t)gy * W + gx] : 0.f;
+  }
+  __syncthreads();
+  for (int i = tid; i < STH * ST; i += ST * ST) {
+    const int r = i / ST, c = i - r * ST;
+    float sy = 0.f, syy = 0.f;
+    for (int k = 0; k < 11; ++k) {
+      const float y = s_y[r][c + k], yy = y * y;
+      sy = fmaf(gw(k), y, sy); syy = fmaf(gw(k), yy, syy);
+    }
+    s_r[0][r][c] = sy; s_r[1][r][c] = syy;
+  }
+  __syncthreads();
+  const int lx = tid % ST, ly = tid / ST;
+  float mu2 = 0.f, eyy = 0.f;
+  for (int k = 0; k < 11; ++k) { mu2 = fmaf(gw(k), s_r[0][ly + k][lx], mu2); eyy = fmaf(gw(k), s_r[1][ly + k][lx], eyy); }
+  if (ox + lx < W && oy + ly < H) {
+    const size_t o = po + (size_t)(oy + ly) * W + ox + lx;
+    mu2_map[o] = mu2; eyy_map[o] = eyy;
   }
 }
 
@@ -645,20 +710,58 @@
 
 static inline int fused_nblocks(int B, int C, int H, int W) { return B * C * ((H + FT - 1) / FT) * ((W + FT - 1) / FT); }
 
-int mi355gs_l1_ssim_loss_fused(void* stream_, int B, int C, int H, int W, const float* img1, const float* img2, void* scratch,
+static inline size_t stats_map_bytes(int planes, int H, int W) { return gs_align((size_t)planes * H * W * sizeof(float)); }
+
+static void launch_l1_ssim_fused(hipStream_t stream, int planes, int H, int W, const float* img1, const float* img2, const void* stats,
+                                 float ks, float kl, float* d_img1, float* partial) {
+  const dim3 grid((W + FT - 1) / FT, (H + FT - 1) / FT, planes);
+  if (stats) {
+    const float* mu2_map = (const float*)stats;
+    const float* eyy_map = (const float*)((const char*)stats + stats_map_bytes(planes, H, W));
+    hipLaunchKernelGGL(k_l1_ssim_fused<true>, grid, dim3(FTHREADS), 0, stream, H, W, img1, img2, mu2_map, eyy_map, ks, kl, d_img1, partial);
+  } else {
+    hipLaunchKernelGGL(k_l1_ssim_fused<false>, grid, dim3(FTHREADS), 0, stream, H, W, img1, img2, (const float*)nullptr, (const float*)nullptr,
+                       ks, kl, d_img1, partial);
+  }
+}
+
+size_t mi355gs_ssim_target_stats_bytes(int B, int C, int H, int W) {
+  if (B <= 0 || C <= 0 || H <= 0 || W <= 0) return 256;
+  return 2 * stats_map_bytes(B * C, H, W);
+}
+
+int mi355gs_ssim_target_stats(void* stream_, int B, int C, int H, int W, const float* img2, void* stats) {
+  GS_RANGE();
+  hipStream_t stream = (hipStream_t)stream_;
+  const int debug = 0;
+  if (B <= 0 || C <= 0 || H <= 0 || W <= 0 || !img2 || !stats) return MI355GS_EINVAL;
+  if ((size_t)B * C > 65535) return MI355GS_EINVAL;
+  GS_KRANGE("ssim_target_stats");
+  hipLaunchKernelGGL(k_ssim_target_stats, dim3((W + ST - 1) / ST, (H + ST - 1) / ST, B * C), dim3(ST * ST), 0, stream, H, W, img2,
+                     (float*)stats, (float*)((char*)stats + stats_map_bytes(B * C, H, W)));
+  GS_CHECK_LAUNCH("ssim_target_stats");
+  return MI355GS_OK;
+}
+
+int mi355gs_l1_ssim_loss_fused(void* stream, int B, int C, int H, int W, const float* img1, const float* img2, void* scratch,
                                float lambda_dssim, float* ssim_mean, float* l1_mean, float* loss, float* dloss_dimg1) {
+  return mi355gs_l1_ssim_loss_fused_cached(stream, B, C, H, W, img1, img2, scratch, lambda_dssim, ssim_mean, l1_mean, loss, dloss_dimg1, nullptr);
+}
+
+int mi355gs_l1_ssim_loss_fused_cached(void* stream_, int B, int C, int H, int W, const float* img1, const float* img2, void* scratch,
+                                      float lambda_dssim, float* ssim_mean, float* l1_mean, float* loss, float* dloss_dimg1,
+                                      const void* target_stats) {
   GS_RANGE();
   hipStream_t stream = (hipStream_t)stream_;
   const int debug = 0;
   if (B <= 0 || C <= 0 || H <= 0 || W <= 0 || !img1 || !img2 || !scratch || !loss || !dloss_dimg1) return MI355GS_EINVAL;
   if ((size_t)B * C > 65535) return MI355GS_EINVAL;
   const double inv_n = 1.0 / ((double)B * C * H * W);
-  const dim3 grid((W + FT - 1) / FT, (H + FT - 1) / FT, B * C);
   {
     GsProfScope prof(3, stream);
     GS_KRANGE("l1_ssim_fused");
-    hipLaunchKernelGGL(k_l1_ssim_fused, grid, dim3(FTHREADS), 0, stream, H, W, img1, img2, (float)(-(double)lambda_dssim * inv_n),
-                       (float)((1.0 - (double)lambda_dssim) * inv_n), dloss_dimg1, (float*)scratch);
+    launch_l1_ssim_fused(stream, B * C, H, W, img1, img2, target_stats, (float)(-(double)lambda_dssim * inv_n),
+                         (float)((1.0 - (double)lambda_dssim) * inv_n), dloss_dimg1, (float*)scratch);
   }
   GS_CHECK_LAUNCH("l1_ssim_fused");
   GS_KRANGE("ssim_finish");
@@ -668,19 +771,23 @@
   return MI355GS_OK;
 }
 
-int mi355gs_l1_ssim_pair_forward(void* stream_, int B, int C, int H, int W, const float* img1, const float* img2, void* scratch,
+int mi355gs_l1_ssim_pair_forward(void* stream, int B, int C, int H, int W, const float* img1, const float* img2, void* scratch,
                                  float* dssim_dimg1) {
+  return mi355gs_l1_ssim_pair_forward_cached(stream, B, C, H, W, img1, img2, scratch, dssim_dimg1, nullptr);
+}
+
+int mi355gs_l1_ssim_pair_forward_cached(void* stream_, int B, int C, int H, int W, const float* img1, const float* img2, void* scratch,
+                                        float* dssim_dimg1, const void* target_stats) {
   GS_RANGE();
   hipStream_t stream = (hipStream_t)stream_;
   const int debug = 0;
   if (B <= 0 || C <= 0 || H <= 0 || W <= 0 || !img1 || !img2 || !scratch || !dssim_dimg1) return MI355GS_EINVAL;
   if ((size_t)B * C > 65535) return MI355GS_EINVAL;
   const double inv_n = 1.0 / ((double)B * C * H * W);
-  const dim3 grid((W + FT - 1) / FT, (H + FT - 1) / FT, B * C);
   {
     GsProfScope prof(3, stream);
     GS_KRANGE("l1_ssim_pair");
-    hipLaunchKernelGGL(k_l1_ssim_fused, grid, dim3(FTHREADS), 0, stream, H, W, img1, img2, (float)inv_n, 0.0f, dssim_dimg1, (float*)scratch);
+    launch_l1_ssim_fused(stream, B * C, H, W, img1, img2, target_stats, (float)inv_n, 0.0f, dssim_dimg1, (float*)scratch);
   }
   GS_CHECK_LAUNCH("l1_ssim_pair");
   return MI355GS_OK;
@@ -755,16 +862,15 @@
 
 }
 
-int gs_loss_fused(hipStream_t stream, int C, int H, int W, const float* img1, const float* img2, float lambda_dssim, float* dL_dimg1,
-                  void* scratch) {
+int gs_loss_fused(hipStream_t stream, int C, int H, int W, const float* img1, const float* img2, const void* target_stats,
+                  float lambda_dssim, float* dL_dimg1, void* scratch) {
   const int debug = 0;
   const double inv_n = 1.0 / ((double)C * H * W);
-  const dim3 grid((W + FT - 1) / FT, (H + FT - 1) / FT, C);
   {
     GsProfScope prof(3, stream);
     GS_KRANGE("l1_ssim_fused");
-    hipLaunchKernelGGL(k_l1_ssim_fused, grid, dim3(FTHREADS), 0, stream, H, W, img1, img2, (float)(-(double)lambda_dssim * inv_n),
-                       (float)((1.0 - (double)lambda_dssim) * inv_n), dL_dimg1, (float*)scratch);
+    launch_l1_ssim_fused(stream, C, H, W, img1, img2, target_stats, (float)(-(double)lambda_dssim * inv_n),
+                         (float)((1.0 - (double)lambda_dssim) * inv_n), dL_dimg1, (float*)scratch);
   }
   GS_CHECK_LAUNCH("l1_ssim_fused");
   return MI355GS_OK;
diff --git a/instantsplat_amd/csrc/trainer.hip b/instantsplat_amd/csrc/trainer.hip
--- a/instantsplat_amd/csrc/trainer.hip
+++ b/instantsplat_amd/csrc/trainer.hip
@@ -2,7 +2,7 @@
 #include <string.h>
 #include "common.h"
 
-int gs_loss_fused(hipStream_t, int, int, int, const float*, const float*, float, float*, void*);
+int gs_loss_fused(hipStream_t, int, int, int, const float*, const float*, const void*, float, float*, void*);
 int gs_loss_fused_nblocks(int, int, int);
 int gs_launch_pose_finish_partials(hipStream_t, const float*, const float*, int, float*, float*, const float*, int, double, float, float*, int,
                                    int);
@@ -26,6 +26,7 @@
   uint32_t adam_seq;
   bool consts_ready;
   int det;
+  const void** target_stats;
   int min_units;
 };
 
@@ -143,6 +144,8 @@
     t->m[k] = exp_avg[k]; t->v[k] = exp_avg_sq[k];
   }
   t->pplr = per_point_lr;
+  t->target_stats = (const void**)calloc((size_t)V, sizeof(void*));
+  if (!t->target_stats) { free(t); return nullptr; }
   t->min_units = gs_min_units();
   t->det = gs_deterministic();
   carve(*t, workspace);
@@ -150,12 +153,22 @@
   return t;
 }
 
-void mi355gs_trainer_destroy(void* handle) { free(handle); }
+void mi355gs_trainer_destroy(void* handle) {
+  if (handle) free(((Trainer*)handle)->target_stats);
+  free(handle);
+}
+
+int mi355gs_trainer_set_target_stats(void* handle, int view, const void* stats) {
+  Trainer* t = (Trainer*)handle;
+  if (!t || view < 0 || view >= t->V) return MI355GS_EINVAL;
+  t->target_stats[view] = stats;
+  return MI355GS_OK;
+}
 
 const float* mi355gs_trainer_grad(void* handle, int k) {
   Trainer* t = (Trainer*)handle;
-  if (!t || k < 0 || k > 6) return nullptr;
-  const float* g[7] = {t->g_xyz, t->g_fdc, t->g_frest, t->g_opacity, t->g_scaling, t->g_rot, t->g_poses};
+  if (!t || k < 0 || k > 8) return nullptr;
+  const float* g[9] = {t->g_xyz, t->g_fdc, t->g_frest, t->g_opacity, t->g_scaling, t->g_rot, t->g_poses, t->dL_dimg, (const float*)t->ssim_scratch};
   return g[k];
 }
 
@@ -208,7 +221,7 @@
                                               t->geom, t->tiles, num_rendered_out, nullptr, nullptr, 0)))
     return rc;
   if ((rc = mi355gs_raster_forward_render(stream, P, W, H, t->capacity, bg, t->geom, t->tiles, t->binning, t->image, 0))) return rc;
-  if ((rc = gs_loss_fused(stream, 3, H, W, t->image, gt_image, lambda_dssim, t->dL_dimg, t->ssim_scratch))) return rc;
+  if ((rc = gs_loss_fused(stream, 3, H, W, t->image, gt_image, t->target_stats[view], lambda_dssim, t->dL_dimg, t->ssim_scratch))) return rc;
   if ((rc = mi355gs_raster_backward(stream, P, D, M, W, H, bg, t->xyz, t->f_dc, rest, nullptr, t->opacity, t->scaling, 1.0f, t->rotation,
                                     nullptr, view_m, projmatrix, campos, tanfovx, tanfovy, t->geom, t->tiles, t->binning,
                                     t->capacity, t->radii, t->image, t->dL_dimg, t->grad_scratch, t->g_xyz, t->g_means2D, t->g_fdc,
diff --git a/instantsplat_amd/csrc_torch/binding.cpp b/instantsplat_amd/csrc_torch/binding.cpp
--- a/instantsplat_amd/csrc_torch/binding.cpp
+++ b/instantsplat_amd/csrc_torch/binding.cpp
@@ -3,9 +3,12 @@
 #include <c10/hip/HIPStream.h>
 
 #include <chrono>
+#include <cstdlib>
+#include <list>
 #include <optional>
 #include <map>
 #include <mutex>
+#include <tuple>
 
 #include "../../include/mi355gs.h"
 
@@ -29,11 +32,13 @@
   X(forward_render_only, mi355gs_raster_forward_render_only)           \
   X(posed_backward, mi355gs_posed_backward)                            \
   X(ssim_scratch_bytes, mi355gs_ssim_scratch_bytes)                    \
-  X(l1_ssim_loss_fused, mi355gs_l1_ssim_loss_fused)                    \
+  X(l1_ssim_loss_fused_cached, mi355gs_l1_ssim_loss_fused_cached)      \
+  X(target_stats_bytes, mi355gs_ssim_target_stats_bytes)               \
+  X(target_stats, mi355gs_ssim_target_stats)                           \
   X(l1_scratch_bytes, mi355gs_l1_scratch_bytes)                        \
   X(l1_loss_forward, mi355gs_l1_loss_forward)                          \
   X(l1_loss_backward, mi355gs_l1_loss_backward)                        \
-  X(pair_forward, mi355gs_l1_ssim_pair_forward)                        \
+  X(pair_forward_cached, mi355gs_l1_ssim_pair_forward_cached)          \
   X(pair_backward, mi355gs_l1_ssim_pair_backward)                      \
   X(program_eval, mi355gs_loss_program_eval)                           \
   X(program_eval_grad, mi355gs_loss_program_eval_grad)                 \
@@ -512,6 +517,83 @@
                             tanfovx, tanfovy, scale_modifier, D, prefiltered, capacity, count_hint, count_slot);
 }
 
+struct TargetStatsCache {
+  using Key = std::tuple<uintptr_t, int64_t, int, int, int, int, int>;
+  struct Entry {
+    c10::weak_intrusive_ptr<c10::StorageImpl> storage;
+    Tensor stats;
+    void* stream = nullptr;
+    std::list<Key>::iterator lru;
+    explicit Entry(c10::weak_intrusive_ptr<c10::StorageImpl> s) : storage(std::move(s)) {}
+  };
+  static constexpr size_t kMaxEntries = 256;
+  std::mutex mu;
+  std::map<Key, Entry> entries;
+  std::list<Key> lru;
+  int64_t bytes = 0, hits = 0, misses = 0, computed = 0, evictions = 0;
+
+  static int64_t max_bytes() {
+    const char* e = std::getenv("MI355GS_TARGET_STATS_MB");
+    if (!e || !*e) return (int64_t)512 << 20;
+    const double mb = std::atof(e);
+    return mb > 0 ? (int64_t)(mb * (double)(1 << 20)) : 0;
+  }
+  void drop(std::map<Key, Entry>::iterator it) {
+    if (it->second.stats.defined()) bytes -= it->second.stats.numel();
+    lru.erase(it->second.lru);
+    entries.erase(it);
+  }
+  void clear() {
+    std::lock_guard<std::mutex> lock(mu);
+    entries.clear(); lru.clear(); bytes = 0;
+  }
+  Tensor lookup(const Tensor& b, int B, int C, int H, int W, const DeviceScope& dev) {
+    const int64_t limit = max_bytes();
+    if (limit == 0 || b.is_inference()) return Tensor();
+    const Key key((uintptr_t)b.data_ptr(), (int64_t)b._version(), B, C, H, W, b.is_cuda() ? (int)b.device().index() : -1);
+    std::lock_guard<std::mutex> lock(mu);
+    auto it = entries.find(key);
+    if (it != entries.end() && it->second.storage.expired()) {
+      drop(it);
+      it = entries.end();
+    }
+    if (it == entries.end()) {
+      ++misses;
+      it = entries.emplace(key, Entry(c10::weak_intrusive_ptr<c10::StorageImpl>(b.storage().getWeakStorageImpl()))).first;
+      it->second.lru = lru.insert(lru.end(), key);
+      while (entries.size() > kMaxEntries) { drop(entries.find(lru.front())); ++evictions; }
+      return Tensor();
+    }
+    Entry& e = it->second;
+    lru.splice(lru.end(), lru, e.lru);
+    if (!e.stats.defined()) {
+      const int64_t n = (int64_t)g_abi.target_stats_bytes(B, C, H, W);
+      if (n > limit) return Tensor();
+      Tensor stats = empty_bytes((size_t)n, b);
+      check(g_abi.target_stats(dev.stream, B, C, H, W, fp(b), stats.data_ptr()), "ssim_target_stats");
+      e.stats = stats; e.stream = dev.stream;
+      bytes += n;
+      ++computed;
+      while (bytes > limit && lru.front() != key) { drop(entries.find(lru.front())); ++evictions; }
+    } else if (e.stream != dev.stream) {
+      return Tensor();
+    }
+    ++hits;
+    return e.stats;
+  }
+} g_target_stats;
+
+void target_stats_clear() { g_target_stats.clear(); }
+
+std::map<std::string, int64_t> target_stats_info() {
+  std::lock_guard<std::mutex> lock(g_target_stats.mu);
+  int64_t with_stats = 0;
+  for (const auto& kv : g_target_stats.entries) with_stats += kv.second.stats.defined() ? 1 : 0;
+  return {{"entries", (int64_t)g_target_stats.entries.size()}, {"with_stats", with_stats}, {"bytes", g_target_stats.bytes},
+          {"max_bytes", TargetStatsCache::max_bytes()}, {"hits", g_target_stats.hits}, {"misses", g_target_stats.misses},
+          {"computed", g_target_stats.computed}, {"evictions", g_target_stats.evictions}};
+}
+
 struct L1SsimLossFn : public torch::autograd::Function<L1SsimLossFn> {
   static variable_list forward(AutogradContext* ctx, Tensor img1, Tensor img2, double lambda_dssim) {
     TORCH_CHECK(g_abi.bound, "mi355gs torch binding: bind() has not been called");
@@ -524,8 +606,9 @@
     Tensor out = at::empty({2}, a.options());
     Tensor loss = at::empty({}, a.options());
     Tensor grad = at::empty_like(a);
-    check(g_abi.l1_ssim_loss_fused(dev.stream, B, C, H, W, fp(a), fp(b), scratch.data_ptr(), (float)lambda_dssim, fp(out), fp(out) + 1,
-                                   fp(loss), fp(grad)),
+    const Tensor stats = g_target_stats.lookup(b, B, C, H, W, dev);
+    check(g_abi.l1_ssim_loss_fused_cached(dev.stream, B, C, H, W, fp(a), fp(b), scratch.data_ptr(), (float)lambda_dssim, fp(out), fp(out) + 1,
+                                          fp(loss), fp(grad), stats.defined() ? stats.data_ptr() : nullptr),
           "l1_ssim_loss_fused");
     ctx->save_for_backward({grad});
     ctx->mark_non_differentiable({out});
@@ -579,7 +662,9 @@
   Tensor scratch = empty_bytes(g_abi.ssim_scratch_bytes(B, C, H, W), a);
   Tensor means = at::empty({2}, a.options());
   Tensor dmap = at::empty_like(a);
-  check(g_abi.pair_forward(dev.stream, B, C, H, W, fp(a), fp(b), scratch.data_ptr(), fp(dmap)), "l1_ssim_pair_forward");
+  const Tensor stats = g_target_stats.lookup(b, B, C, H, W, dev);
+  check(g_abi.pair_forward_cached(dev.stream, B, C, H, W, fp(a), fp(b), scratch.data_ptr(), fp(dmap), stats.defined() ? stats.data_ptr() : nullptr),
+        "l1_ssim_pair_forward");
   return {means, scratch, dmap, a, b};
 }
 
@@ -862,6 +947,8 @@
   m.def("pose_row", &pose_row, "GaussianModel.get_RT: row `index` of the [views, 7] pose table as a node the render node's backward cooperates with");
   m.def("rasterize", &rasterize);
   m.def("l1_ssim_loss", &l1_ssim_loss);
+  m.def("target_stats_clear", &target_stats_clear);
+  m.def("target_stats_info", &target_stats_info);
   m.def("loss_pair_forward", &loss_pair_forward, "-> [means (l1, ssim: filled by the first loss_affine), partial sums, d(ssim_mean)/dimg1, img1, img2 (contiguous)]: one launch, no autograd node");
   m.def("wait_for_loss", &wait_for_loss, "the value the program kernel stored to a pinned host slot under this ticket, or None (timeout / slot taken over)");
   m.def("loss_affine_backward", &loss_affine_backward, "loss_affine + the engine run of loss.backward() in one call (root gradient: a cached 1)");
diff --git a/instantsplat_amd/fused_ssim/__init__.py b/instantsplat_amd/fused_ssim/__init__.py
--- a/instantsplat_amd/fused_ssim/__init__.py
+++ b/instantsplat_amd/fused_ssim/__init__.py
@@ -4,6 +4,7 @@
 
 from .. import _lib
 from .. import lazy_loss
+from .. import target_stats
 
 
 def _run_forward(img1, img2, train, valid=False):
@@ -96,9 +97,10 @@
         loss = torch.empty((), dtype=torch.float32, device=dev)
         grad = torch.empty_like(a)
         p0 = out.data_ptr()
+        stats = target_stats.lookup(b, B, C, H, W, dev)
         with _lib.on_device(dev):
-            _lib.check(L.mi355gs_l1_ssim_loss_fused(_lib.stream_ptr(dev), B, C, H, W, _lib.ptr(a), _lib.ptr(b), _lib.ptr(scratch),
-                                                    float(lambda_dssim), p0, p0 + 4, _lib.ptr(loss), _lib.ptr(grad)),
+            _lib.check(L.mi355gs_l1_ssim_loss_fused_cached(_lib.stream_ptr(dev), B, C, H, W, _lib.ptr(a), _lib.ptr(b), _lib.ptr(scratch),
+                                                           float(lambda_dssim), p0, p0 + 4, _lib.ptr(loss), _lib.ptr(grad), _lib.ptr(stats)),
                        "l1_ssim_loss_fused")
         ctx.save_for_backward(grad)
         ctx.mark_non_differentiable(out)
diff --git a/instantsplat_amd/lazy_loss.py b/instantsplat_amd/lazy_loss.py
--- a/instantsplat_amd/lazy_loss.py
+++ b/instantsplat_amd/lazy_loss.py
@@ -7,7 +7,7 @@
 import numpy as np
 import torch
 
-from . import _lib
+from . import _lib, target_stats
 
 ENABLED = os.environ.get("MI355GS_LAZY_LOSS", "1") != "0"
 
@@ -79,6 +79,9 @@
 
 def forget():
     _LAST[0] = None
+    target_stats.clear()
+    if _lib._EXT is not None:
+        _lib._EXT.target_stats_clear()
 
 
 def _new(rec, prog):
@@ -347,9 +350,10 @@
     scratch = torch.empty(int(L.mi355gs_ssim_scratch_bytes(B, C, H, W)), dtype=torch.uint8, device=dev)
     means = torch.empty(2, dtype=torch.float32, device=dev)
     dmap = torch.empty_like(a)
+    stats = target_stats.lookup(b, B, C, H, W, dev)
     with _lib.on_device(dev):
-        _lib.check(L.mi355gs_l1_ssim_pair_forward(_lib.stream_ptr(dev), B, C, H, W, _lib.ptr(a), _lib.ptr(b), _lib.ptr(scratch),
-                                                  _lib.ptr(dmap)), "l1_ssim_pair_forward")
+        _lib.check(L.mi355gs_l1_ssim_pair_forward_cached(_lib.stream_ptr(dev), B, C, H, W, _lib.ptr(a), _lib.ptr(b), _lib.ptr(scratch),
+                                                         _lib.ptr(dmap), _lib.ptr(stats)), "l1_ssim_pair_forward")
     return means, scratch, dmap, a, b
 
 
diff --git a/instantsplat_amd/target_stats.py b/instantsplat_amd/target_stats.py
--- /dev/null
+++ b/instantsplat_amd/target_stats.py
@@ -0,0 +1,80 @@
+from __future__ import annotations
+
+import os
+from collections import OrderedDict
+
+import torch
+from torch.multiprocessing.reductions import StorageWeakRef
+
+from . import _lib
+
+MAX_ENTRIES = 256
+
+
+def _max_bytes():
+    try:
+        return max(0, int(float(os.environ.get("MI355GS_TARGET_STATS_MB", "512")) * (1 << 20)))
+    except ValueError:
+        return 512 << 20
+
+
+_ENTRIES = OrderedDict()
+_BYTES = [0]
+_COUNTERS = dict(hits=0, misses=0, computed=0, evictions=0)
+
+
+def _drop(key):
+    e = _ENTRIES.pop(key)
+    if e[1] is not None:
+        _BYTES[0] -= e[1].numel()
+
+
+def lookup(gt, B, C, H, W, dev):
+    limit = _max_bytes()
+    if limit == 0:
+        return None
+    key = (gt.data_ptr(), gt._version, B, C, H, W, str(dev))
+    stream = _lib.stream_ptr(dev)
+    e = _ENTRIES.get(key)
+    if e is not None and e[0].expired():
+        _drop(key)
+        e = None
+    if e is None:
+        _COUNTERS["misses"] += 1
+        _ENTRIES[key] = [StorageWeakRef(gt.untyped_storage()), None, stream]
+        while len(_ENTRIES) > MAX_ENTRIES:
+            _drop(next(iter(_ENTRIES)))
+            _COUNTERS["evictions"] += 1
+        return None
+    _ENTRIES.move_to_end(key)
+    if e[1] is None:
+        L = _lib.lib()
+        n = int(L.mi355gs_ssim_target_stats_bytes(B, C, H, W))
+        if n > limit:
+            return None
+        stats = torch.empty(n, dtype=torch.uint8, device=dev)
+        with _lib.on_device(dev):
+            _lib.check(L.mi355gs_ssim_target_stats(stream, B, C, H, W, _lib.ptr(gt), _lib.ptr(stats)), "ssim_target_stats")
+        e[1], e[2] = stats, stream
+        _BYTES[0] += n
+        _COUNTERS["computed"] += 1
+        while _BYTES[0] > limit:
+            oldest = next(iter(_ENTRIES))
+            if oldest == key:
+                break
+            _drop(oldest)
+            _COUNTERS["evictions"] += 1
+    elif e[2] != stream:
+        return None
+    _COUNTERS["hits"] += 1
+    return e[1]
+
+
+def clear():
+    _ENTRIES.clear()
+    _BYTES[0] = 0
+
+
+def info():
+    return dict(entries=len(_ENTRIES), with_stats=sum(1 for e in _ENTRIES.values() if e[1] is not None), bytes=_BYTES[0],
+                max_bytes=_max_bytes(), **_COUNTERS)
diff --git a/instantsplat_amd/train.py b/instantsplat_amd/train.py
--- a/instantsplat_amd/train.py
+++ b/instantsplat_amd/train.py
@@ -330,6 +330,18 @@
         if not self.handle:
             raise RuntimeError("mi355gs_trainer_create failed")
         self.num_rendered = torch.zeros(1, dtype=torch.int32, device=dev)
+        self._target_stats = {}
+        nstats = int(L.mi355gs_ssim_target_stats_bytes(1, 3, self.H, self.W))
+        with _lib.on_device(dev):
+            for cam in st.cameras:
+                uid = int(cam.uid)
+                if uid in self._target_stats or not 0 <= uid < V:
+                    continue
+                gt = st.gt_images[uid]
+                stats = torch.empty(nstats, dtype=torch.uint8, device=dev)
+                _lib.check(L.mi355gs_ssim_target_stats(_lib.stream_ptr(dev), 1, 3, self.H, self.W, _lib.ptr(gt), _lib.ptr(stats)), "ssim_target_stats")
+                _lib.check(L.mi355gs_trainer_set_target_stats(ctypes.c_void_p(self.handle), uid, _lib.ptr(stats)), "trainer_set_target_stats")
+                self._target_stats[uid] = (gt, gt._version, stats)
         self._count_ring = torch.zeros(self.COUNT_RING, dtype=torch.int32, pin_memory=(dev.type == "cuda"))
         self._count_next = 0
 
@@ -349,6 +361,22 @@
             assert addr and 0 <= off and off + nbytes <= self.workspace.numel(), (name, off)
             out[name] = self.workspace[off:off + nbytes].view(torch.float32).view(p.shape).clone()
         return out
+
+    def loss_pass_outputs(self):
+        L, base = _lib.lib(), self.workspace.data_ptr()
+        n = 3 * ((self.H + 31) // 32) * ((self.W + 31) // 32)
+        out = []
+        for k, shape in ((7, (3, self.H, self.W)), (8, (n, 2))):
+            addr = L.mi355gs_trainer_grad(ctypes.c_void_p(self.handle), k)
+            off, nbytes = int(addr) - base, 4 * math.prod(shape)
+            assert addr and 0 <= off and off + nbytes <= self.workspace.numel(), (k, off)
+            out.append(self.workspace[off:off + nbytes].view(torch.float32).view(shape).clone())
+        return tuple(out)
+
+    def withdraw_target_stats(self):
+        for uid in list(self._target_stats):
+            _lib.check(_lib.lib().mi355gs_trainer_set_target_stats(ctypes.c_void_p(self.handle), uid, None), "trainer_set_target_stats")
+            del self._target_stats[uid]
 
     __del__ = close
 
@@ -378,9 +406,14 @@
 
     def launch(self, a, loss_slot: torch.Tensor, count_out: torch.Tensor, defer_optimizer: bool = False):
         cam = a["cam"]
+        gt = self.st.gt_images[cam.uid]
+        kept = self._target_stats.get(int(cam.uid))
+        if kept is not None and (kept[0] is not gt or kept[1] != gt._version):
+            _lib.check(_lib.lib().mi355gs_trainer_set_target_stats(ctypes.c_void_p(self.handle), int(cam.uid), None), "trainer_set_target_stats")
+            del self._target_stats[int(cam.uid)]
         with _lib.on_device(self.dev):
             _lib.check(_lib.lib().mi355gs_trainer_step(
-                ctypes.c_void_p(self.handle), _lib.stream_ptr(self.dev), int(cam.uid), a["sh"], _lib.ptr(self.st.gt_images[cam.uid]),
+                ctypes.c_void_p(self.handle), _lib.stream_ptr(self.dev), int(cam.uid), a["sh"], _lib.ptr(gt),
                 _lib.ptr(cam.projection_matrix), math.tan(cam.FoVx * 0.5), math.tan(cam.FoVy * 0.5), _lib.ptr(a["bg"]),
                 a["lr"], a["steps"], a["b1"], a["b2"], a["eps"], a["lam"],
                 1 if (a["do_opt"] and not defer_optimizer) else 0, _lib.ptr(loss_slot), _lib.ptr(count_out)), "trainer_step")
```
